# hmetaxa/MVTopicModel

Measured on AMD Instinct MI355X. Metric: gibbs_tokens_per_sec, higher is better.
Workload: dtype f64

## Files before the change

include/mvhdp.h:

```cpp
#ifndef MVHDP_H
#define MVHDP_H

#include <stddef.h>
#include <stdint.h>

#ifdef __cplusplus
extern "C" {
#endif

#define MVHDP_MAX_MODALITIES 8
#define MVHDP_MAX_TOPICS     2048
#define MVHDP_UNASSIGNED_TOPIC (-1)

typedef enum {
    MVHDP_OK = 0,
    MVHDP_ERR_INVALID_ARG   = -1,
    MVHDP_ERR_STATE         = -2,
    MVHDP_ERR_HIP           = -3,
    MVHDP_ERR_NO_DEVICE     = -4,
    MVHDP_ERR_NEGATIVE_COUNT= -5,
    MVHDP_ERR_UNSUPPORTED   = -6
} mvhdp_status;

typedef struct mvhdp_ctx* mvhdp_handle;
// ... 95 lines not shown
int mvhdp_build_counts(mvhdp_handle h);
int mvhdp_build_trees(mvhdp_handle h);
int mvhdp_build_inference_trees(mvhdp_handle h);
int mvhdp_init_assignments_from_trees(mvhdp_handle h, uint64_t seed);
int mvhdp_get_counts(mvhdp_handle h, int32_t m, int32_t* n_wk , int32_t* n_k );
int mvhdp_set_counts(mvhdp_handle h, int32_t m, const int32_t* n_wk, const int32_t* n_k);
int mvhdp_get_tree(mvhdp_handle h, int32_t m, int32_t type, double* tree );
int mvhdp_get_doc_topic_hist(mvhdp_handle h, int32_t m, int32_t* hist , int32_t hist_len,
                             int32_t* doc_len_counts , int32_t len_len);

int mvhdp_get_count_histogram(mvhdp_handle h, int32_t m, int32_t* hist, int32_t len);
int mvhdp_view_overlap_sums(mvhdp_handle h, double* sums );
int mvhdp_model_log_likelihood(mvhdp_handle h, double* log_likelihood );
int mvhdp_gamma_doc_statistics(mvhdp_handle h, int32_t m, double gamma_m, uint64_t seed, uint32_t round, double* qs, double* qw);
int mvhdp_dp_table_statistics(mvhdp_handle h, int32_t m, const int32_t* hist , int32_t hist_len, const double* conc ,
                              uint64_t seed, uint32_t round, double* mk , uint8_t* active );
int mvhdp_antoniak_draws(mvhdp_handle h, int32_t n, const int32_t* items , const double* conc , uint64_t seed, uint32_t round, int32_t* tables );
int mvhdp_doc_topic_proportions(mvhdp_handle h, const double* view_weights , int64_t d0, int64_t d1, double* out );

#define MVHDP_DIAG_MAX_TOP_WORDS 64
#define MVHDP_DIAG_PROPORTIONS   7
#define MVHDP_DIAG_TOKENS             0
#define MVHDP_DIAG_DOCUMENT_ENTROPY   1
#define MVHDP_DIAG_WORD_LENGTH        2
#define MVHDP_DIAG_COHERENCE          3
#define MVHDP_DIAG_NORM_DISCR_WEIGHT  4
#define MVHDP_DIAG_DISCR_WEIGHT       5
#define MVHDP_DIAG_UNIFORM_DIST       6
#define MVHDP_DIAG_CORPUS_DIST        7
#define MVHDP_DIAG_EFF_NUM_WORDS      8
#define MVHDP_DIAG_TOKEN_DOC_DIFF     9
#define MVHDP_DIAG_RANK_1_DOCS       10
#define MVHDP_DIAG_ALLOCATION_RATIO  11
#define MVHDP_DIAG_ALLOCATION_COUNT  12
#define MVHDP_DIAG_ROWS              13
typedef struct {
    int32_t num_top_words;
    const int32_t* word_length;
} mvhdp_diag_args;
typedef struct {
    double*  scores;
    double*  word_scores;
    int32_t* codoc;
    int32_t* top_types;
    int32_t* top_counts;
    int32_t* nonzero;
    int32_t* num_rank1_docs;
    int32_t* num_nonzero_docs;
    int32_t* num_docs_at_proportions;
    double*  sum_count_log_count;
    int32_t* word_type_counts;
    int64_t* num_tokens;
    double*  discr_weight_per_view;
} mvhdp_diag_out;
int mvhdp_top_words(mvhdp_handle h, int32_t m, int32_t n, int32_t* types , int32_t* counts , int32_t* nonzero );
int mvhdp_discr_weights(mvhdp_handle h, double* per_view , int32_t m, double* type_weight );
int mvhdp_diagnostics(mvhdp_handle h, const mvhdp_diag_args* args, mvhdp_diag_out* out);

int mvhdp_sweep(mvhdp_handle h, uint32_t sweep_idx, uint64_t seed, uint32_t flags,
                const double* p_override, const mvhdp_debug* dbg, mvhdp_sweep_stats* stats);
int mvhdp_sweep_many(mvhdp_handle h, uint32_t first_idx, int32_t n, uint64_t seed, uint32_t flags, mvhdp_sweep_stats* stats );
int mvhdp_apply_delta(mvhdp_handle h, int32_t activated_topic, int32_t activated_modality);
int mvhdp_apply_delta_begin(mvhdp_handle h);
int mvhdp_apply_delta_rows(mvhdp_handle h, int64_t row_begin, int64_t row_end);
int mvhdp_apply_delta_end(mvhdp_handle h, int32_t activated_topic, int32_t activated_modality);
int mvhdp_get_birth_keys(mvhdp_handle h, int64_t* keys );
int mvhdp_activate_births(mvhdp_handle h, const int64_t* keys );
int mvhdp_trees_current(mvhdp_handle h);
int mvhdp_get_view_weights(mvhdp_handle h, double* p );

typedef struct {
    int32_t force_primary;
    int32_t narrow;
    int32_t walk_fixed;
    int32_t single_stream;
    int32_t live16;
    int32_t single_wave;
    double  walk_theta[MVHDP_MAX_MODALITIES];
    double  primary_min_share;
    int32_t learnt_walk_step[4];
    double  tree_branch_share[MVHDP_MAX_MODALITIES];
    int32_t live_overlap;
    int32_t live_rows;
} mvhdp_tuning;
int mvhdp_get_tuning(mvhdp_handle h, mvhdp_tuning* t);
int mvhdp_set_tuning(mvhdp_handle h, const mvhdp_tuning* t);

typedef struct {
    int32_t num_topics, num_modalities;
    int64_t num_entities;
    int64_t max_entity_tokens;
    int64_t entities_longer_than[5];
    uint64_t tokens_by_list_rounds[17];
    uint64_t entities_by_class[8];
    uint32_t flags;
    int32_t debug, batch, trees_current;
    int32_t num_cus;
    int32_t kernel_registers[6][3];
    int32_t inactive_topics;
} mvhdp_plan_input;
typedef struct {
    int32_t status;
    int32_t segments, primary_class, register_resident, need_full_trees, dominant_class;
    int64_t routed_prefix;
    int32_t class_used[6], class_map[6], class_stream[6], class_grid[6], class_walk[6], class_narrow[6], class_register_resident[6];
    int64_t class_lds_bytes[6];
    double  class_theta0[6];
    int32_t delta16, live_rows;
} mvhdp_plan_output;
int mvhdp_plan_probe(const mvhdp_plan_input* in, const mvhdp_tuning* tuning , mvhdp_plan_output* out);
int mvhdp_tuner_probe(int32_t num_modalities, const double* tree_branch_share , const double* u1_hist ,
                      const double* ns_by_step , int32_t n_sweeps, int32_t group, int32_t* steps_out );

typedef struct mvhdp_group_ctx* mvhdp_group;
#define MVHDP_UNIQUE_ID_BYTES 128
typedef struct {
    int32_t local_members;
    int32_t local_devices;
    int32_t ranks, first_rank;
    int32_t rccl;
    int32_t rccl_version;
    int32_t exchange_chunks;
    int32_t exchange_packed;
    double  last_exchange_ms;
    int64_t last_exchange_bytes;
} mvhdp_group_info;
int mvhdp_group_create(int32_t n, const mvhdp_handle* members, mvhdp_group* out);
int mvhdp_group_unique_id(uint8_t* id );
int mvhdp_group_create_rank(mvhdp_handle member, const uint8_t* id , int32_t rank, int32_t nranks, mvhdp_group* out);
int mvhdp_group_destroy(mvhdp_group g);
const char* mvhdp_group_last_error(mvhdp_group g);
int mvhdp_group_get_info(mvhdp_group g, mvhdp_group_info* info);
int mvhdp_group_set_exchange_chunks(mvhdp_group g, int32_t chunks );
int mvhdp_group_build_counts(mvhdp_group g);
int mvhdp_group_sweep(mvhdp_group g, uint32_t sweep_idx, uint64_t seed, uint32_t flags, mvhdp_sweep_stats* stats);
#define MVHDP_SWEEP_ASYNC_EXCHANGE 0x100u
int mvhdp_group_drain(mvhdp_group g);
int mvhdp_group_abort(mvhdp_group g);

int mvhdp_group_set_hyper(mvhdp_group g, const mvhdp_hyper* hy);
int mvhdp_group_log_likelihood(mvhdp_group g, double* log_likelihood );
int mvhdp_group_doc_topic_hist(mvhdp_group g, int32_t m, int32_t* hist , int32_t hist_len,
                               int32_t* doc_len_counts , int32_t len_len);
int mvhdp_group_count_histogram(mvhdp_group g, int32_t m, int32_t* hist, int32_t len);
int mvhdp_group_view_overlap_sums(mvhdp_group g, double* sums );
int mvhdp_group_gamma_doc_statistics(mvhdp_group g, int32_t m, double gamma_m, uint64_t seed, uint32_t round, double* qs, double* qw);
int mvhdp_group_diagnostics(mvhdp_group g, const mvhdp_diag_args* args, mvhdp_diag_out* out);

int mvhdp_device_buffer(mvhdp_handle h, mvhdp_buffer which, void** dev_ptr, size_t* bytes);
int mvhdp_counts_written(mvhdp_handle h);
int mvhdp_set_stream(mvhdp_handle h, void* hip_stream );
int mvhdp_synchronize(mvhdp_handle h);

#ifdef __cplusplus
}
#endif
#endif
```

mvtopicmodel_amd/_lib.py:

```python
import ctypes as C
import os

_HERE = os.path.dirname(os.path.abspath(__file__))
LIB_PATH = os.path.join(_HERE, "lib", "libmvhdp.so")

MAX_M = 8

ABI_SYMBOLS = [
    "mvhdp_create", "mvhdp_destroy", "mvhdp_last_error", "mvhdp_version",
    "mvhdp_set_corpus", "mvhdp_set_assignments", "mvhdp_set_view_presence", "mvhdp_get_assignments",
    "mvhdp_set_hyper", "mvhdp_get_alpha", "mvhdp_build_counts", "mvhdp_build_trees",
    "mvhdp_build_inference_trees", "mvhdp_init_assignments_from_trees",
    "mvhdp_get_counts", "mvhdp_set_counts", "mvhdp_get_tree", "mvhdp_get_doc_topic_hist",
    "mvhdp_get_count_histogram", "mvhdp_view_overlap_sums", "mvhdp_model_log_likelihood", "mvhdp_doc_topic_proportions",
    "mvhdp_gamma_doc_statistics", "mvhdp_dp_table_statistics", "mvhdp_antoniak_draws",
    "mvhdp_top_words", "mvhdp_discr_weights", "mvhdp_diagnostics",
    "mvhdp_sweep", "mvhdp_sweep_many", "mvhdp_get_tuning", "mvhdp_set_tuning", "mvhdp_plan_probe", "mvhdp_tuner_probe",
    "mvhdp_apply_delta", "mvhdp_apply_delta_begin", "mvhdp_apply_delta_rows", "mvhdp_apply_delta_end",
    "mvhdp_get_birth_keys", "mvhdp_activate_births",
    "mvhdp_trees_current", "mvhdp_get_view_weights",
    "mvhdp_device_buffer", "mvhdp_counts_written", "mvhdp_set_stream", "mvhdp_synchronize",
    "mvhdp_group_create", "mvhdp_group_unique_id", "mvhdp_group_create_rank", "mvhdp_group_destroy", "mvhdp_group_last_error",
    "mvhdp_group_get_info", "mvhdp_group_set_exchange_chunks", "mvhdp_group_build_counts", "mvhdp_group_sweep", "mvhdp_group_abort", "mvhdp_group_drain",
    "mvhdp_group_set_hyper", "mvhdp_group_log_likelihood", "mvhdp_group_doc_topic_hist", "mvhdp_group_count_histogram",
    "mvhdp_group_view_overlap_sums", "mvhdp_group_gamma_doc_statistics", "mvhdp_group_diagnostics",
]

UNIQUE_ID_BYTES = 128


class MvhdpError(RuntimeError):
    def __init__(self, code, msg):
        super().__init__(f"mvhdp error {code}: {msg}")
        self.code = code


class Config(C.Structure):
    _fields_ = [("num_topics", C.c_int32), ("num_modalities", C.c_int32),
                ("num_types", C.c_int32 * MAX_M), ("device", C.c_int32),
                ("doc_id_base", C.c_int64), ("flags", C.c_uint32)]


class HyperC(C.Structure):
    _fields_ = [("alpha", C.c_void_p),
                ("alpha_sum", C.c_double * MAX_M), ("beta", C.c_double * MAX_M),
                ("beta_sum", C.c_double * MAX_M), ("gamma", C.c_double * MAX_M),
                ("p_a", (C.c_double * MAX_M) * MAX_M), ("p_b", (C.c_double * MAX_M) * MAX_M),
                ("inactive", C.c_void_p)]


class SweepStatsC(C.Structure):
    _fields_ = [("tokens", C.c_int64), ("changed", C.c_int64), ("new_mass_cnt", C.c_int64),
                ("topic_doc_mass_cnt", C.c_int64), ("word_ftree_mass_cnt", C.c_int64),
                ("oov_skipped", C.c_int64), ("aborted_docs", C.c_int64), ("exact_fallbacks", C.c_int64),
                ("activated_topic", C.c_int32), ("activated_modality", C.c_int32),
                ("activation_key", C.c_int64), ("sweep_kernel_ms", C.c_double), ("total_ms", C.c_double),
                ("activations", C.c_int32), ("reserved", C.c_int32)]


class DebugC(C.Structure):
    _fields_ = [("tok_dbg", C.c_void_p * MAX_M), ("n_trace", C.c_int32),
                ("trace_doc", C.c_void_p), ("trace_view", C.c_void_p), ("trace_pos", C.c_void_p),
                ("trace_out", C.c_void_p)]


class TuningC(C.Structure):
    _fields_ = [("force_primary", C.c_int32), ("narrow", C.c_int32), ("walk_fixed", C.c_int32), ("single_stream", C.c_int32),
                ("live16", C.c_int32), ("single_wave", C.c_int32),
                ("walk_theta", C.c_double * MAX_M), ("primary_min_share", C.c_double),
                ("learnt_walk_step", C.c_int32 * 4), ("tree_branch_share", C.c_double * MAX_M),
                ("live_overlap", C.c_int32), ("live_rows", C.c_int32)]


class GroupInfoC(C.Structure):
    _fields_ = [("local_members", C.c_int32), ("local_devices", C.c_int32), ("ranks", C.c_int32), ("first_rank", C.c_int32),
                ("rccl", C.c_int32), ("rccl_version", C.c_int32), ("exchange_chunks", C.c_int32), ("exchange_packed", C.c_int32),
                ("last_exchange_ms", C.c_double), ("last_exchange_bytes", C.c_int64)]


class PlanInputC(C.Structure):
    _fields_ = [("num_topics", C.c_int32), ("num_modalities", C.c_int32), ("num_entities", C.c_int64),
                ("max_entity_tokens", C.c_int64), ("entities_longer_than", C.c_int64 * 5),
                ("tokens_by_list_rounds", C.c_uint64 * 17), ("entities_by_class", C.c_uint64 * 8),
                ("flags", C.c_uint32), ("debug", C.c_int32), ("batch", C.c_int32), ("trees_current", C.c_int32),
                ("num_cus", C.c_int32), ("kernel_registers", (C.c_int32 * 3) * 6), ("inactive_topics", C.c_int32)]


class PlanOutputC(C.Structure):
    _fields_ = [("status", C.c_int32), ("segments", C.c_int32), ("primary_class", C.c_int32), ("register_resident", C.c_int32),
                ("need_full_trees", C.c_int32), ("dominant_class", C.c_int32), ("routed_prefix", C.c_int64),
                ("class_used", C.c_int32 * 6), ("class_map", C.c_int32 * 6), ("class_stream", C.c_int32 * 6),
                ("class_grid", C.c_int32 * 6), ("class_walk", C.c_int32 * 6), ("class_narrow", C.c_int32 * 6),
                ("class_register_resident", C.c_int32 * 6), ("class_lds_bytes", C.c_int64 * 6), ("class_theta0", C.c_double * 6),
                ("delta16", C.c_int32), ("live_rows", C.c_int32)]


DIAG_MAX_TOP_WORDS = 64
DIAG_PROPORTIONS = 7
DIAG_ROWS = ["tokens", "document_entropy", "word-length", "coherence", "normDiscrWeight", "discrWeight", "uniform_dist",
             "corpus_dist", "eff_num_words", "token-doc-diff", "rank_1_docs", "allocation_ratio", "allocation_count"]


class DiagArgsC(C.Structure):
    _fields_ = [("num_top_words", C.c_int32), ("word_length", C.c_void_p)]


class DiagOutC(C.Structure):
    _fields_ = [("scores", C.c_void_p), ("word_scores", C.c_void_p), ("codoc", C.c_void_p), ("top_types", C.c_void_p),
                ("top_counts", C.c_void_p), ("nonzero", C.c_void_p), ("num_rank1_docs", C.c_void_p), ("num_nonzero_docs", C.c_void_p),
                ("num_docs_at_proportions", C.c_void_p), ("sum_count_log_count", C.c_void_p), ("word_type_counts", C.c_void_p),
                ("num_tokens", C.c_void_p), ("discr_weight_per_view", C.c_void_p)]


_lib = None
_preloaded = []


def _torch_lib_dir():
    import importlib.util
    try:
        spec = importlib.util.find_spec("torch")
    except (ImportError, ValueError):
        return None
    if spec is None or not spec.submodule_search_locations:
        return None
    d = os.path.join(list(spec.submodule_search_locations)[0], "lib")
    return d if os.path.isdir(d) else None


def mapped_runtime_libraries():
    found = {"libamdhip64": set(), "libhsa-runtime64": set(), "librccl": set()}
    try:
        with open("/proc/self/maps") as f:
            for line in f:
                path = line.rsplit(None, 1)[-1] if "/" in line else ""
                base = os.path.basename(path)
                for name in found:
                    if base.startswith(name + ".so"):
                        found[name].add(os.path.realpath(path))
    except OSError:
        pass
    return {k: sorted(v) for k, v in found.items()}


def _preload_one_hip_runtime():
    d = _torch_lib_dir()
    if d is None:
        return False
    already = mapped_runtime_libraries()
    if already["libamdhip64"] or already["libhsa-runtime64"]:
        return False
    path = os.path.join(d, "libamdhip64.so")
    if not os.path.exists(path):
        return False
# ... 96 lines not shown
```

mvtopicmodel_amd/csrc/mvhdp_api.hip:

```cpp
#include "mvhdp_ctx.h"

static thread_local std::string g_create_error;

static std::mutex g_reg_mutex;
static std::set<mvhdp_ctx*>* g_live = nullptr;
static bool g_exiting = false, g_atexit_registered = false;
static void release_device_resources(mvhdp_ctx* h);

static void mvhdp_at_exit()
{
    std::lock_guard<std::mutex> lk(g_reg_mutex);
    g_exiting = true;
    if (g_live) for (mvhdp_ctx* h : *g_live) release_device_resources(h);
}

static void register_handle(mvhdp_ctx* h)
{
    std::lock_guard<std::mutex> lk(g_reg_mutex);
    if (!g_live) g_live = new std::set<mvhdp_ctx*>();
    g_live->insert(h);
    if (!g_atexit_registered) { atexit(mvhdp_at_exit); g_atexit_registered = true; }
}

bool mvhdp_is_live(mvhdp_ctx* h)
{
    std::lock_guard<std::mutex> lk(g_reg_mutex);
    return g_live && g_live->count(h) != 0;
}

static void read_environment(mvhdp_ctx* h)
{
    if (const char* f = getenv("MVHDP_FORCE_RMAX")) { const int v = atoi(f); if (v == 1 || v == 2 || v == 4 || v == 8 || v == 16 || v == 32) h->tu.force_primary = v; }
    if (const char* f = getenv("MVHDP_NARROW")) h->tu.narrow = atoi(f) != 0 ? -1 : 0;
    if (const char* f = getenv("MVHDP_SINGLE_STREAM")) h->tu.single_stream = atoi(f) != 0;
    if (const char* f = getenv("MVHDP_SIDE_PRIORITY")) h->side_priority = atoi(f);
    if (const char* f = getenv("MVHDP_LIVE16")) h->tu.live16 = atoi(f);
    if (const char* f = getenv("MVHDP_LIVE_OVERLAP")) h->tu.live_overlap = atoi(f);
    if (const char* f = getenv("MVHDP_LIVE_ROWS")) h->tu.live_rows = atoi(f);
    if (const char* f = getenv("MVHDP_LIVE_ROWS_THETA")) h->tu.live_rows_theta = atof(f);
    if (const char* f = getenv("MVHDP_COEF_LDS_KB")) h->tu.coef_lds_max_bytes = std::max(0, std::min(64, atoi(f))) * 1024;
    if (const char* f = getenv("MVHDP_LIVE_ROWS_SEGMENTS")) h->tu.live_rows_segments = std::max(1, std::min(255, atoi(f)));
    if (const char* f = getenv("MVHDP_WIDEST_ON_MAIN")) h->tu.widest_on_main = atoi(f) != 0;
    if (const char* f = getenv("MVHDP_NARROW_WIDE")) h->tu.narrow_wide = atoi(f) != 0;
    if (const char* f = getenv("MVHDP_LIVE_TREE_EVERY")) h->live_tree_every = std::max(1, atoi(f));
    if (const char* f = getenv("MVHDP_GATE_PCT")) { const int v = atoi(f); if (v >= 5 && v <= 95) h->gate_pct = v; }
    if (const char* f = getenv("MVHDP_FOUR_ROUND_ON_C")) h->tu.four_round_on_c = atoi(f);
    if (const char* f = getenv("MVHDP_DELTA16")) h->tu.delta16 = atoi(f) != 0;
    if (const char* f = getenv("MVHDP_FORK_DELAY_US")) h->tu.fork_delay_us = std::max(0, std::min(1000, atoi(f)));
    if (const char* f = getenv("MVHDP_FORCE_MODE")) { if (!strcmp(f, "serial")) h->tu.single_stream = 1; }
    if (const char* f = getenv("MVHDP_PRIMARY_MIN_SHARE")) { const double v = atof(f); if (v > 0.0 && v <= 1.0) h->tu.primary_min_share = v; }
    if (const char* t = getenv("MVHDP_WALK_THETA")) {
        int m = 0;
        for (const char* q = t; *q && m < MVHDP_MAXM; m++) {
            h->tu.walk_theta[m] = atof(q);
            while (*q && *q != ',') q++;
            if (*q == ',') q++;
        }
        for (; m < MVHDP_MAXM; m++) h->tu.walk_theta[m] = 0.0;
        h->tu.walk_fixed = 1;
    }
    h->dbg_env = getenv("MVHDP_DEBUG") != nullptr;
}

extern "C" const char* mvhdp_version(void) { return "mvhdp 0.1 (gfx950)"; }

extern "C" const char* mvhdp_last_error(mvhdp_handle h) { return (h && mvhdp_is_live(h)) ? h->err.c_str() : g_create_error.c_str(); }

extern "C" int mvhdp_create(const mvhdp_config* cfg, mvhdp_handle* out)
{
    if (!cfg || !out) { g_create_error = "null argument"; return MVHDP_ERR_INVALID_ARG; }
    *out = nullptr;
    const int K = cfg->num_topics, M = cfg->num_modalities;
    if (K < 1 || K > MVHDP_MAX_TOPICS || M < 1 || M > MVHDP_MAX_MODALITIES) {
        g_create_error = "num_topics must be in [1,2048] and num_modalities in [1,8]";
        return MVHDP_ERR_INVALID_ARG;
    }
    for (int m = 0; m < M; m++) if (cfg->num_types[m] < 1) { g_create_error = "num_types[m] must be >= 1"; return MVHDP_ERR_INVALID_ARG; }
    for (int m = 0; m < M; m++) if (cfg->num_types[m] >= (1 << 29)) { g_create_error = "num_types[m] must be below 2^29"; return MVHDP_ERR_INVALID_ARG; }
    if (cfg->doc_id_base < 0 || cfg->doc_id_base >= (1LL << 29)) { g_create_error = "doc_id_base out of range"; return MVHDP_ERR_INVALID_ARG; }
    int ndev = 0;
    if (hipGetDeviceCount(&ndev) != hipSuccess || ndev <= 0 || cfg->device < 0 || cfg->device >= ndev) {
        g_create_error = "no usable HIP device (the sweep has no CPU fallback)";
        return MVHDP_ERR_NO_DEVICE;
    }
    hipDeviceProp_t prop;
    if (hipGetDeviceProperties(&prop, cfg->device) != hipSuccess) { g_create_error = "hipGetDeviceProperties failed"; return MVHDP_ERR_HIP; }
    if (strncmp(prop.gcnArchName, "gfx950", 6) != 0) {
        g_create_error = std::string("device is ") + prop.gcnArchName + ", this library is built for gfx950 only";
        return MVHDP_ERR_NO_DEVICE;
    }
    mvhdp_ctx* h = new mvhdp_ctx();
    register_handle(h);
    h->cfg = *cfg;
    h->device = cfg->device;
    h->num_cus = prop.multiProcessorCount;
    h->max_lds = 160 * 1024;
    MvModel& mm = h->mm;
    mm.K = K; mm.M = M;
    mm.rowbase[0] = 0;
    for (int m = 0; m < M; m++) { mm.V[m] = cfg->num_types[m]; mm.rowbase[m + 1] = mm.rowbase[m] + cfg->num_types[m]; }
    mm.doc_id_base = cfg->doc_id_base;
    mm.first_inactive = -1;
    mm.D = -1;
#define CREATE_HIP(call) do { hipError_t e_ = (call); if (e_ != hipSuccess) { \
    g_create_error = std::string(#call) + ": " + hipGetErrorString(e_); mvhdp_destroy(h); return MVHDP_ERR_HIP; } } while (0)
    CREATE_HIP(hipSetDevice(h->device));
    CREATE_HIP(hipStreamCreateWithFlags(&h->stream, hipStreamNonBlocking));
    h->own_stream = true;
    for (auto& e : h->ev) CREATE_HIP(hipEventCreate(&e));
    const int64_t nrows = mm.rowbase[M];
    const size_t cbytes = (size_t)(nrows * K + (int64_t)M * K + MVHDP_TAIL_WORDS) * sizeof(int32_t);
    CREATE_HIP(hipMalloc(&mm.counts, cbytes));
    CREATE_HIP(hipMalloc(&mm.delta, cbytes));
    CREATE_HIP(hipMemset(mm.counts, 0, cbytes));
    CREATE_HIP(hipMalloc(&mm.counts16, (size_t)nrows * K * sizeof(uint16_t) + 64));
    CREATE_HIP(hipMemset(mm.counts16, 0, (size_t)nrows * K * sizeof(uint16_t)));
    CREATE_HIP(hipMalloc(&mm.delta16, (size_t)(nrows * K + 2) * sizeof(uint16_t)));
    CREATE_HIP(hipMemsetD16(mm.delta16, (unsigned short)0x8000, (size_t)(nrows * K + 2)));
    CREATE_HIP(hipMalloc(&mm.heavy, (size_t)nrows));
    CREATE_HIP(hipMemset(mm.heavy, 1, (size_t)nrows));
    CREATE_HIP(hipMemset(mm.delta, 0, cbytes));
    CREATE_HIP(hipMalloc(&mm.trees, (size_t)nrows * 2 * K * sizeof(double)));
    CREATE_HIP(hipMalloc(&mm.root, (size_t)nrows * sizeof(double)));
    CREATE_HIP(hipMalloc(&mm.mass0, (size_t)nrows * sizeof(float)));
    CREATE_HIP(hipMemset(mm.mass0, 0, (size_t)nrows * sizeof(float)));
    CREATE_HIP(hipMalloc(&mm.coef, (size_t)M * (((K + 7) & ~7) + K + 8) * sizeof(float)));
    {
        const int nlev = (K > 1) ? (32 - __builtin_clz((unsigned)(K - 1))) : 0;
        mm.dt_f = nlev ? ((nlev - 1) % 3) + 1 : 0;
        mm.dt_nbd = 1; mm.dt_base[0] = 0; mm.dt_depth[0] = 0;
        int nblk = 1;
        for (int dep = mm.dt_f; nlev && dep < nlev; dep += 3) {
            mm.dt_base[mm.dt_nbd] = nblk; mm.dt_depth[mm.dt_nbd] = dep; mm.dt_nbd++;
            nblk += 1 << dep;
        }
        mm.dt_nblk = nblk;
        CREATE_HIP(hipMalloc(&mm.dtab, (size_t)nrows * nblk * 8 * sizeof(double)));
    }
    CREATE_HIP(hipMalloc(&h->d_alpha, (size_t)M * (K + 1) * sizeof(double)));
    CREATE_HIP(hipMalloc(&h->d_inactive, (size_t)K));
    CREATE_HIP(hipMemset(h->d_inactive, 0, (size_t)K));
    CREATE_HIP(hipMalloc(&h->d_births, (size_t)(2 + 2 * K) * sizeof(int32_t)));
    CREATE_HIP(hipMemset(h->d_births, 0, (size_t)(2 + 2 * K) * sizeof(int32_t)));
    CREATE_HIP(hipMalloc(&h->d_birth_keys, (size_t)K * sizeof(long long)));
    CREATE_HIP(hipMalloc(&h->d_birth_table, (size_t)K * sizeof(long long)));
    {
        const std::vector<long long> none((size_t)K, LLONG_MAX);
        CREATE_HIP(hipMemcpy(h->d_birth_table, none.data(), (size_t)K * sizeof(long long), hipMemcpyHostToDevice));
    }
    CREATE_HIP(hipMalloc(&h->d_ctl, CTL_WORDS * sizeof(unsigned long long)));
    CREATE_HIP(hipMemset(h->d_ctl, 0, CTL_WORDS * sizeof(unsigned long long)));
    h->d_stats = h->d_ctl;
    h->d_act_key = (long long*)(h->d_ctl + ST_COUNT);
    h->d_ovf_meta = (unsigned int*)(h->d_ctl + ST_COUNT + 1);
    h->d_doc_counter = h->d_ctl + ST_COUNT + 1 + META_WORDS64;
    CREATE_HIP(hipHostMalloc((void**)&h->h_ctl, CTL_WORDS * sizeof(unsigned long long), hipHostMallocDefault));
    for (int c = 0; c < MVHDP_N_CLASSES; c++)
        for (int f = 0; f < 3; f++) h->regs.regs[c][f] = mvhdp_sweep_kernel_regs(c, f);
    read_environment(h);
    mm.alpha = h->d_alpha;
    mm.inactive = h->d_inactive;
    h->h_alpha.assign((size_t)M * (K + 1), 0.0);
    h->h_inactive.assign((size_t)K, 0);
    h->wt.init_defaults(K);
    *out = h;
    return MVHDP_OK;
}

static void release_device_resources(mvhdp_ctx* h)
{
    if (h->device_released) return;
    h->device_released = true;
    hipSetDevice(h->device);
    if (h->stream) hipStreamSynchronize(h->stream);
    auto fr = [](auto*& p) { if (p) { hipFree((void*)p); p = nullptr; } };
    for (int m = 0; m < MVHDP_MAXM; m++) { fr(h->d_doc_off[m]); fr(h->d_tok[m]); fr(h->d_z[m]); fr(h->d_carry[m]); fr(h->d_present[m]); }
    fr(h->mm.counts); fr(h->mm.delta16); fr(h->mm.counts16); fr(h->mm.heavy); fr(h->mm.delta); fr(h->mm.trees); fr(h->mm.root); fr(h->mm.coef); fr(h->mm.mass0); fr(h->d_births); fr(h->d_birth_keys); fr(h->d_birth_table); fr(h->mm.dtab); fr(h->mm.p);
    fr(h->d_alpha); fr(h->d_inactive); fr(h->d_ctl);
    if (h->h_ctl) { hipHostFree(h->h_ctl); h->h_ctl = nullptr; }
    h->d_stats = nullptr; h->d_act_key = nullptr; h->d_doc_counter = nullptr; h->d_ovf_meta = nullptr;
    fr(h->d_doc_order); fr(h->d_lists); fr(h->d_nslots); fr(h->d_stats_many); fr(h->d_heavy_list); fr(h->d_heavy_ctl);
    if (h->ev_rf_go) { hipEventDestroy(h->ev_rf_go); h->ev_rf_go = nullptr; }
    if (h->ev_rf_done) { hipEventDestroy(h->ev_rf_done); h->ev_rf_done = nullptr; }
    if (h->rf_stream) { hipStreamDestroy(h->rf_stream); h->rf_stream = nullptr; }
    fr(h->ov.counts2); fr(h->ov.counts16_2); fr(h->ov.dtab2); fr(h->ov.root2); fr(h->ov.trees2); fr(h->ov.delta2); fr(h->ov.delta3); fr(h->ov.ctl2); fr(h->ov.lists2);
    for (auto& e : h->ov.ev_seg) if (e) { hipEventDestroy(e); e = nullptr; }
    if (h->ov.ev_start) { hipEventDestroy(h->ov.ev_start); h->ov.ev_start = nullptr; }
    if (h->ov.x1) { hipStreamDestroy(h->ov.x1); h->ov.x1 = nullptr; }
    if (h->ov.xa) { hipStreamDestroy(h->ov.xa); h->ov.xa = nullptr; }
    for (auto& e : h->ev_many) if (e) { hipEventDestroy(e); e = nullptr; }
    for (auto& e : h->ev) if (e) { hipEventDestroy(e); e = nullptr; }
    if (h->ev_fork) { hipEventDestroy(h->ev_fork); h->ev_fork = nullptr; }
    for (auto& e : h->ev_join) if (e) { hipEventDestroy(e); e = nullptr; }
    for (auto& st : h->side) if (st) { hipStreamDestroy(st); st = nullptr; }
    if (h->own_stream && h->stream) hipStreamDestroy(h->stream);
    h->stream = nullptr;
}

extern "C" int mvhdp_destroy(mvhdp_handle h)
{
    if (!h) return MVHDP_OK;
    bool exiting;
    {
        std::lock_guard<std::mutex> lk(g_reg_mutex);
        if (!g_live || g_live->erase(h) == 0) return MVHDP_ERR_INVALID_ARG;
        exiting = g_exiting;
    }
    if (!exiting) release_device_resources(h);
    delete h;
    return MVHDP_OK;
}

extern "C" int mvhdp_set_stream(mvhdp_handle h, void* hip_stream)
{
    CHECK_H(h);
    HIPC(h, hipSetDevice(h->device));
    HIPC(h, hipStreamSynchronize(h->stream));
    if (h->own_stream) { hipStreamDestroy(h->stream); h->own_stream = false; }
    if (hip_stream) h->stream = (hipStream_t)hip_stream;
    else { HIPC(h, hipStreamCreateWithFlags(&h->stream, hipStreamNonBlocking)); h->own_stream = true; }
    return MVHDP_OK;
}

extern "C" int mvhdp_synchronize(mvhdp_handle h)
{
    CHECK_H(h);
    HIPC(h, hipSetDevice(h->device));
    HIPC(h, hipStreamSynchronize(h->stream));
    return MVHDP_OK;
}

extern "C" int mvhdp_set_corpus(mvhdp_handle h, int32_t m, int64_t D, const int64_t* doc_off, const int32_t* tokens)
{
    CHECK_H(h);
    MvModel& mm = h->mm;
    if (m < 0 || m >= mm.M || D < 0 || !doc_off) FAIL(h, MVHDP_ERR_INVALID_ARG, "set_corpus: bad view, num_docs or doc_off");
    if (mm.D >= 0 && D != mm.D) {
        bool any_other = false;
        for (int j = 0; j < mm.M; j++) if (j != m && h->have_corpus[j]) any_other = true;
        if (any_other) FAIL(h, MVHDP_ERR_INVALID_ARG, "set_corpus: every view must list the same entities (empty span = view absent)");
    }
    if (mm.doc_id_base + D >= (1LL << 29)) FAIL(h, MVHDP_ERR_INVALID_ARG, "set_corpus: too many entities");
    if (doc_off[0] != 0) FAIL(h, MVHDP_ERR_INVALID_ARG, "set_corpus: doc_off[0] must be 0");
    for (int64_t d = 0; d < D; d++) {
        int64_t len = doc_off[d + 1] - doc_off[d];
        if (len < 0) FAIL(h, MVHDP_ERR_INVALID_ARG, "set_corpus: doc_off must be non-decreasing");
        if (len >= (1 << 20)) FAIL(h, MVHDP_ERR_INVALID_ARG, "set_corpus: a view of one entity is limited to 2^20-1 tokens");
    }
    const int64_t N = doc_off[D];
    if (N > 0 && !tokens) FAIL(h, MVHDP_ERR_INVALID_ARG, "set_corpus: tokens is null");
    HIPC(h, hipSetDevice(h->device));
    HIPC(h, hipStreamSynchronize(h->stream));
    if (h->d_doc_off[m]) { hipFree(h->d_doc_off[m]); h->d_doc_off[m] = nullptr; }
    if (h->d_tok[m]) { hipFree(h->d_tok[m]); h->d_tok[m] = nullptr; }
    if (h->d_z[m]) { hipFree(h->d_z[m]); h->d_z[m] = nullptr; }
    if (h->d_present[m]) { hipFree(h->d_present[m]); h->d_present[m] = nullptr; }
    h->h_present[m].clear(); mm.present[m] = nullptr;
    HIPC(h, hipMalloc(&h->d_doc_off[m], (size_t)(D + 1) * sizeof(int64_t)));
    HIPC(h, hipMemcpy(h->d_doc_off[m], doc_off, (size_t)(D + 1) * sizeof(int64_t), hipMemcpyHostToDevice));
    const size_t nb = (size_t)std::max<int64_t>(N, 1) * sizeof(int32_t);
// ... 746 lines not shown
        MvModel mk;
        if (p.seg_apply) {
            mk = B[seg == 0 ? 0 : (seg - 1) & 1];
            mk.delta = D3[seg % 3];
        } else {
            mk = mm;
            mk.delta = mm.counts;
            mk.dtab = B[seg & 1].dtab; mk.root = B[seg & 1].root; mk.trees = B[seg & 1].trees;
            if (seg >= 1 && !(flags & MVHDP_SWEEP_REUSE_TREES)) {
                step(hipStreamWaitEvent(xs, ev_reset(seg - 1), 0));
                const int64_t n_prev = share_of(seg - 1, mm.D), H_prev = p.route ? share_of(seg - 1, p.H) : 0;
                const unsigned long long thr = (unsigned long long)((n_prev - H_prev) * h->gate_pct / 100);
                step(mvhdp_launch_gate(ctl[(seg - 1) & 1].qheads + p.pc, thr, xs));
                MvModel tm = mm;
                tm.dtab = mk.dtab; tm.root = mk.root; tm.trees = mk.trees;
                if (p.live16) step(mvhdp_launch_build_trees_from_mirror(tm, p.need_full, xs, true));
                else step(mvhdp_launch_build_trees(tm, false, p.need_full, xs, true));
            } else if (seg >= 1) {
                mk.dtab = mm.dtab; mk.root = mm.root; mk.trees = mm.trees;
            }
        }
        step(mvhdp_launch_ctl_reset(nullptr, 0, nullptr, nullptr, 0, cs.class_counts, cs.qheads, xs));
        step(hipEventRecord(ev_reset(seg), xs));
        step(launch_segment_kernels(h, p, mk, sl, seg, xs, cs, d_stats));
        step(hipEventRecord(ev_done(seg), xs));
        if (p.seg_apply) {
            if (seg >= 1) step(hipStreamWaitEvent(xs, ev_applied(seg - 1), 0));
            const MvModel& dst = B[(seg + 1) & 1];
            step(mvhdp_launch_apply2_counts(dst, D3[seg % 3], seg >= 1 ? D3[(seg - 1) % 3] : nullptr, use_mirror, d_stats + ST_NEGATIVE, xs));
            step(hipEventRecord(ev_applied(seg), xs));
        }
    }
    if (mm.D > 0 && e == hipSuccess) {
        if (p.seg_apply) {
            step(hipStreamWaitEvent(X[0], ev_applied(nseg - 1), 0));
            if (nseg >= 2) step(hipStreamWaitEvent(X[0], ev_done(nseg - 2), 0));
            const MvModel& last = B[(nseg + 1) & 1];
            step(mvhdp_launch_apply_sparse(last, D3[(nseg - 1) % 3], use_mirror, X[0]));
            h->have_trees = false;
        } else {
            step(hipStreamWaitEvent(X[0], ev_done(nseg - 1), 0));
            if (nseg >= 2) step(hipStreamWaitEvent(X[0], ev_done(nseg - 2), 0));
        }
    }
    if (p.live) {
        if (p.live16 && mm.D > 0) { step(mvhdp_launch_widen_mirror(mm, X[0])); h->have_trees = false; }
        if (flags & MVHDP_SWEEP_NO_APPLY) {
            step(mvhdp_launch_live_helper(mm, 1, d_stats, X[0]));
            if (!(flags & MVHDP_SWEEP_REUSE_TREES)) h->have_trees = false;
        } else step(mvhdp_launch_live_helper(mm, 2, d_stats, X[0]));
        if (!(flags & MVHDP_SWEEP_REUSE_TREES)) h->have_trees = false;
    }
    step(hipEventRecord(ev_k1, X[0]));
    if (e != hipSuccess) HIPC(h, e);
    return MVHDP_OK;
}

static int enqueue_sweep(mvhdp_ctx* h, const SweepPlan& p, uint32_t sweep_idx, uint64_t seed, const double* p_override,
                         const DebugBufs* db, unsigned long long* d_stats, hipEvent_t ev_k0, hipEvent_t ev_k1, SweepOutcome& oc)
{
    if (p.overlap) return enqueue_overlapped(h, p, sweep_idx, seed, p_override, d_stats, ev_k0, ev_k1);
    MvModel& mm = h->mm;
    const int M = mm.M;
    const uint32_t flags = p.flags;
    const int nseg = p.nseg;
    hipStream_t s = h->stream;
    hipError_t e = hipSuccess;
    auto step = [&](hipError_t r) { if (e == hipSuccess) e = r; };

    SweepLaunch sl{};
    sl.sweep_idx = sweep_idx; sl.seed_lo = (uint32_t)seed; sl.seed_hi = (uint32_t)(seed >> 32);
    sl.flags = flags & 0x7fffu; sl.S_cap = p.S_cap;
    if (h->tu.single_wave && p.live) sl.flags |= MVHDP_SL_STRICT_LIVE;
    if (p.live_rows && getenv("MVHDP_NO_ROW_SAMPLE")) sl.flags |= 0x2000u;
#ifdef MVHDP_PROBE
    if (const char* f = getenv("MVHDP_ATOMIC_PROBE")) sl.flags |= ((unsigned)atoi(f) & 7u) << 16;
#endif
    sl.q_order_stride = 1;
    sl.nk_global = p.nk_global; sl.block_shared_bytes = p.block_shared_bytes;
    sl.live16 = p.live16 ? 1 : 0;
    sl.live_rows = p.live_rows ? 1 : 0;
    sl.coef_lds = p.coef_lds ? 1 : 0;
    sl.delta16 = p.delta16 ? 1 : 0;
    sl.stats = d_stats;
    sl.act_key = h->d_act_key;
    const bool births = sweep_births(p, flags, mm);
    if (births) { sl.births = h->d_births; sl.birth_keys = h->d_birth_keys; }
    sl.slot_hist = (unsigned long long*)h->d_ovf_meta + META_HIST;
    if (db) {
        for (int m = 0; m < M; m++) sl.tok_dbg[m] = db->tok_dbg[m];
        sl.n_trace = db->n_trace; sl.trace_doc = db->trace_doc; sl.trace_view = db->trace_view; sl.trace_pos = db->trace_pos; sl.trace_out = db->trace_out;
    }
    unsigned int* class_counts = h->d_ovf_meta + META_CLASS_COUNTS;

    if (M > 1) {
        if (!mm.p && mm.D > 0) step(hipMalloc(&mm.p, (size_t)mm.D * M * M * sizeof(double)));
        if (e == hipSuccess) {
            if (p_override) step(hipMemcpyAsync(mm.p, p_override, (size_t)mm.D * M * M * sizeof(double), hipMemcpyHostToDevice, s));
            else step(mvhdp_launch_draw_p(mm, sweep_idx, sl.seed_lo, sl.seed_hi, s));
        }
    }
    h->last_need_full = p.need_full;
    const bool dummy_poll = getenv("MVHDP_DUMMY_POLL") != nullptr;
    const bool refresher = ((p.live_rows && p.live16) || dummy_poll) && !h->tu.single_wave && !getenv("MVHDP_NO_HEAVY_REFRESH");
    auto live_rows_prepare = [&](bool from_mirror) -> hipError_t {
        if ((p.live16 || dummy_poll) && !h->d_heavy_list) {
            hipError_t e1 = hipMalloc(&h->d_heavy_list, (size_t)MVHDP_HEAVY_CAP * sizeof(int32_t));
            if (e1 == hipSuccess) e1 = hipMalloc(&h->d_heavy_ctl, 2 * sizeof(unsigned int));
            if (e1 != hipSuccess) return e1;
        }
        if (refresher && !h->rf_stream) {
            int least = 0, greatest = 0;
            if (hipDeviceGetStreamPriorityRange(&least, &greatest) != hipSuccess || greatest >= least ||
                hipStreamCreateWithPriority(&h->rf_stream, hipStreamNonBlocking, greatest) != hipSuccess) {
                (void)hipGetLastError(); h->rf_stream = nullptr;
                hipError_t e1 = hipStreamCreateWithFlags(&h->rf_stream, hipStreamNonBlocking); if (e1 != hipSuccess) return e1;
            }
            hipError_t e1 = hipEventCreateWithFlags(&h->ev_rf_go, hipEventDisableTiming);
            if (e1 == hipSuccess) e1 = hipEventCreateWithFlags(&h->ev_rf_done, hipEventDisableTiming);
            if (e1 != hipSuccess) return e1;
        }
        return mvhdp_launch_live_rows_prepare(mm, from_mirror, p.live16, p.live16 ? h->d_heavy_list : nullptr, p.live16 ? h->d_heavy_ctl : nullptr, MVHDP_HEAVY_CAP,
                                              p.live16 ? 512 : 256 , s);
    };
    auto rebuild_trees = [&]() {
        step(mvhdp_launch_build_trees(mm, false, p.need_full, s));
        h->have_trees = true; h->full_trees = p.need_full; h->trees_inference = false;
    };
    if (p.live_rows) {
        step(live_rows_prepare(false));
        h->have_trees = false; h->full_trees = false;
    } else if (!(flags & MVHDP_SWEEP_REUSE_TREES)) rebuild_trees();
    if (dummy_poll && !p.live_rows) {
        if (!h->d_heavy_list) { step(hipMalloc(&h->d_heavy_list, (size_t)MVHDP_HEAVY_CAP * sizeof(int32_t))); step(hipMalloc(&h->d_heavy_ctl, 2 * sizeof(unsigned int))); }
        if (!h->rf_stream) { step(hipStreamCreateWithFlags(&h->rf_stream, hipStreamNonBlocking)); step(hipEventCreateWithFlags(&h->ev_rf_go, hipEventDisableTiming)); step(hipEventCreateWithFlags(&h->ev_rf_done, hipEventDisableTiming)); }
        step(hipMemsetAsync(h->d_heavy_ctl, 0, 2 * sizeof(unsigned int), s));
    }
    else if (p.need_full && !h->full_trees) {
        step(mvhdp_launch_build_trees(mm, h->trees_inference, true, s));
        h->full_trees = true;
    }
    MvModel mk = mm;
    if (p.live) {
        mk.delta = mm.counts;
        if (flags & MVHDP_SWEEP_NO_APPLY) { step(mvhdp_launch_live_helper(mm, 0, d_stats, s)); h->delta_clean = false; }
    } else if (!p.frozen) {
        if (!h->delta_clean) {
            step(hipMemsetAsync(mm.delta, 0, (size_t)counts_len(h) * sizeof(int32_t), s));
            if (h->delta16_used) step(hipMemsetD16Async(mm.delta16, (unsigned short)0x8000, (size_t)(mm.rowbase[M] * mm.K), s));
            h->delta16_used = false;
        }
        h->delta_clean = false;
        if (p.delta16) h->delta16_used = true;
    }
    step(mvhdp_launch_ctl_reset(d_stats, ST_COUNT, h->d_act_key, (unsigned long long*)h->d_ovf_meta, META_WORDS64, nullptr, h->d_doc_counter, s));
    if (births) step(births_begin(h, s));
    step(hipEventRecord(ev_k0, s));

    const int seg_lo = p.only_seg >= 0 ? p.only_seg : 0, seg_hi = p.only_seg >= 0 ? p.only_seg + 1 : nseg;
    for (int seg = seg_lo; seg < seg_hi && e == hipSuccess && mm.D > 0; seg++) {
        if (seg > seg_lo) {
            if (births && !(flags & MVHDP_SWEEP_NO_APPLY) && e == hipSuccess) {
                const int rc = births_end(h, s, oc);
                if (rc != MVHDP_OK) return rc;
                mk.first_inactive = mm.first_inactive;
                step(births_begin(h, s));
// ... 261 lines not shown
    CHECK_H(h);
    if (n < 0) FAIL(h, MVHDP_ERR_INVALID_ARG, "sweep_many: n < 0");
    if (n == 0) return MVHDP_OK;
    MvModel& mm = h->mm;
    const bool frozen = (flags & MVHDP_SWEEP_FROZEN) != 0;
    if (n == 1 || mm.first_inactive >= 0 || ((flags & MVHDP_SWEEP_NO_APPLY) && !frozen) || ((flags & MVHDP_SWEEP_REUSE_TREES) && !frozen) || n > 4096) {
        for (int i = 0; i < n; i++) {
            const int rc = mvhdp_sweep(h, first_idx + (uint32_t)i, seed, flags, nullptr, nullptr, stats ? stats + i : nullptr);
            if (rc) return rc;
        }
        return MVHDP_OK;
    }
    int rc = sweep_preconditions(h, flags); if (rc) return rc;
    HIPC(h, hipSetDevice(h->device));
    hipStream_t s = h->stream;
    rc = ensure_slot_counts(h); if (rc) return rc;
    PlanIn in; fill_plan_in(h, flags, false, true, in);
    SweepPlan p;
    plan_sweep(in, h->tu, h->wt, p);
    if (p.err) FAIL(h, p.err, p.msg);
    rc = set_generic_lds(h, p); if (rc) return rc;
    if (h->dbg_env) debug_print_plan(h, p, first_idx);
    if (h->stats_many_cap < n) {
        if (h->d_stats_many) { hipFree(h->d_stats_many); h->d_stats_many = nullptr; h->stats_many_cap = 0; }
        HIPC(h, hipMalloc(&h->d_stats_many, (size_t)n * ST_COUNT * sizeof(unsigned long long)));
        h->stats_many_cap = n;
    }
    while ((int)h->ev_many.size() < 2 * n) { hipEvent_t ev; HIPC(h, hipEventCreate(&ev)); h->ev_many.push_back(ev); }
    HIPC(h, hipEventRecord(h->ev[0], s));
    for (int i = 0; i < n; i++) {
        SweepOutcome oc;
        unsigned long long* d_st = h->d_stats_many + (size_t)i * ST_COUNT;
        rc = enqueue_sweep(h, p, first_idx + (uint32_t)i, seed, nullptr, nullptr, d_st, h->ev_many[2 * i], h->ev_many[2 * i + 1], oc);
        if (rc) return rc;
        if (!p.frozen && !p.live && !p.seg_apply) {
            HIPC(h, mvhdp_launch_apply_delta(mm, d_st, s, h->delta16_used));
            h->delta16_used = false;
            h->have_trees = false; h->delta_clean = true;
        } else if (p.live || p.seg_apply) {
            h->have_trees = false;
            if (p.seg_apply) h->delta_clean = true;
        }
    }
    HIPC(h, hipEventRecord(h->ev[3], s));
    std::vector<unsigned long long> hs((size_t)n * ST_COUNT);
    unsigned long long meta[META_WORDS64] = {0};
    HIPC(h, hipMemcpyAsync(hs.data(), h->d_stats_many, hs.size() * sizeof(unsigned long long), hipMemcpyDeviceToHost, s));
    HIPC(h, hipMemcpyAsync(meta, h->d_ovf_meta, sizeof meta, hipMemcpyDeviceToHost, s));
    HIPC(h, hipStreamSynchronize(s));
    if (p.seg_apply && p.overlap) h->ov.deltas_dirty = false;
    float ms_t = 0;
    hipEventElapsedTime(&ms_t, h->ev[0], h->ev[3]);
    int ret = MVHDP_OK;
    double ms_sum = 0;
    for (int i = 0; i < n; i++) {
        const unsigned long long* hi = hs.data() + (size_t)i * ST_COUNT;
        mvhdp_sweep_stats st;
        stats_from_counters(hi, LLONG_MAX, st);
        float ms_k = 0;
        hipEventElapsedTime(&ms_k, h->ev_many[2 * i], h->ev_many[2 * i + 1]);
        st.sweep_kernel_ms = ms_k; st.total_ms = ms_t / n;
        ms_sum += ms_k;
        if (stats) stats[i] = st;
        if (hi[ST_MISCLASS]) { h->nslots_valid = false; FAIL(h, MVHDP_ERR_HIP, "internal: an entity reached a sweep kernel variant that cannot hold its topic list"); }
        if (hi[ST_NEGATIVE] && ret == MVHDP_OK) { h->err = "a topic count went below zero (UPD:202-215)"; ret = MVHDP_ERR_NEGATIVE_COUNT; }
    }
    if (meta[META_MISROUTED]) { h->nslots_valid = false; FAIL(h, MVHDP_ERR_HIP, "internal: an entity could not be routed to a sweep kernel"); }
    std::vector<unsigned long long> acc(ST_COUNT, 0);
    for (int i = 0; i < n; i++) for (int k = 0; k < ST_COUNT; k++) acc[k] += hs[(size_t)i * ST_COUNT + k];
    const bool comparable = p.fast && !h->tu.walk_fixed && !(flags & (MVHDP_SWEEP_FROZEN | MVHDP_SWEEP_EXACT_CHAIN));
    learn_from_sweep(h, p, acc.data(), meta + META_HIST, ms_sum, comparable);
    if (!p.frozen && acc[ST_ABORT] == 0) for (int m = 0; m < mm.M; m++) h->unassigned[m] = false;
    return ret;
}

extern "C" int mvhdp_get_tuning(mvhdp_handle h, mvhdp_tuning* t)
{
    CHECK_H(h);
    if (!t) FAIL(h, MVHDP_ERR_INVALID_ARG, "get_tuning: null");
    memset(t, 0, sizeof *t);
    t->force_primary = h->tu.force_primary; t->narrow = h->tu.narrow; t->walk_fixed = h->tu.walk_fixed;
    t->single_stream = h->tu.single_stream; t->primary_min_share = h->tu.primary_min_share; t->live16 = h->tu.live16;
    t->single_wave = h->tu.single_wave; t->live_overlap = h->tu.live_overlap; t->live_rows = h->tu.live_rows;
    for (int m = 0; m < MVHDP_MAX_MODALITIES; m++) { t->walk_theta[m] = h->tu.walk_theta[m]; t->tree_branch_share[m] = h->wt.walk_f[m]; }
    for (int g = 0; g < WALK_GROUPS; g++) t->learnt_walk_step[g] = g == h->wt.walk_cls ? h->wt.walk_i : h->wt.walk_i_by[g];
    t->learnt_walk_step[3] = -1;
    return MVHDP_OK;
}

extern "C" int mvhdp_set_tuning(mvhdp_handle h, const mvhdp_tuning* t)
{
    CHECK_H(h);
    if (!t) FAIL(h, MVHDP_ERR_INVALID_ARG, "set_tuning: null");
    const int fp = t->force_primary;
    if (!(fp == 0 || fp == 1 || fp == 2 || fp == 4 || fp == 8 || fp == 16 || fp == 32)) FAIL(h, MVHDP_ERR_INVALID_ARG, "set_tuning: force_primary must be 0, 1, 2, 4, 8, 16 or 32");
    if (t->primary_min_share < 0.0 || t->primary_min_share > 1.0) FAIL(h, MVHDP_ERR_INVALID_ARG, "set_tuning: primary_min_share outside [0, 1]");
    for (int g = 0; g < WALK_GROUPS; g++) if (t->learnt_walk_step[g] < -1 || t->learnt_walk_step[g] > MVHDP_WALK_BINS) FAIL(h, MVHDP_ERR_INVALID_ARG, "set_tuning: learnt_walk_step outside [-1, 20]");
    h->tu.force_primary = fp; h->tu.narrow = t->narrow; h->tu.walk_fixed = t->walk_fixed ? 1 : 0;
    h->tu.single_stream = t->single_stream ? 1 : 0;
    h->tu.live16 = t->live16 < 0 ? -1 : (t->live16 ? 1 : 0);
    h->tu.single_wave = t->single_wave ? 1 : 0;
    h->tu.live_overlap = t->live_overlap < 0 ? -1 : (t->live_overlap ? 1 : 0);
    h->tu.live_rows = t->live_rows < 0 ? -1 : (t->live_rows ? 1 : 0);
    h->tu.primary_min_share = t->primary_min_share > 0.0 ? t->primary_min_share : 0.10;
    for (int m = 0; m < MVHDP_MAX_MODALITIES; m++) h->tu.walk_theta[m] = t->walk_theta[m];
    if (t->learnt_walk_step[0] >= 0 || t->learnt_walk_step[1] >= 0 || t->learnt_walk_step[2] >= 0) h->wt.restore(t->learnt_walk_step, t->tree_branch_share, h->mm.M);
    return MVHDP_OK;
}

extern "C" int mvhdp_plan_probe(const mvhdp_plan_input* pi, const mvhdp_tuning* t, mvhdp_plan_output* po)
{
    if (!pi || !po) return MVHDP_ERR_INVALID_ARG;
    PlanIn in;
    in.K = pi->num_topics; in.M = pi->num_modalities; in.D = pi->num_entities; in.mdt = pi->max_entity_tokens;
    if (in.K < 1 || in.K > MVHDP_MAX_TOPICS || in.M < 1 || in.M > MVHDP_MAX_MODALITIES || in.D < 0) return MVHDP_ERR_INVALID_ARG;
    in.have_order = true;
    for (int c = 0; c < 5; c++) in.n_longer[c] = pi->entities_longer_than[c];
    for (int b = 0; b < MVHDP_HIST_BINS; b++) in.tok_hist[b] = pi->tokens_by_list_rounds[b];
    for (int b = 0; b < MVHDP_ENT_BINS; b++) in.ent_hist[b] = pi->entities_by_class[b];
    in.flags = pi->flags; in.debug = pi->debug != 0; in.batch = pi->batch != 0; in.trees_current = pi->trees_current != 0;
    in.first_inactive = pi->inactive_topics ? 0 : -1;
    in.num_cus = pi->num_cus > 0 ? pi->num_cus : 256;
    for (int c = 0; c < MVHDP_N_CLASSES; c++) for (int f = 0; f < 3; f++) in.regs.regs[c][f] = pi->kernel_registers[c][f];
    PlanTuning tu;
    WalkTuner wt;
    wt.init_defaults(in.K);
    if (t) {
        tu.force_primary = t->force_primary; tu.narrow = t->narrow; tu.walk_fixed = t->walk_fixed; tu.single_stream = t->single_stream;
        tu.live16 = t->live16; tu.single_wave = t->single_wave ? 1 : 0; tu.live_overlap = t->live_overlap; tu.live_rows = t->live_rows;
        if (t->primary_min_share > 0) tu.primary_min_share = t->primary_min_share;
        for (int m = 0; m < MVHDP_MAX_MODALITIES; m++) tu.walk_theta[m] = t->walk_theta[m];
        if (t->learnt_walk_step[0] >= 0 || t->learnt_walk_step[1] >= 0 || t->learnt_walk_step[2] >= 0) wt.restore(t->learnt_walk_step, t->tree_branch_share, in.M);
    }
    SweepPlan p;
    plan_sweep(in, tu, wt, p);
    memset(po, 0, sizeof *po);
    po->status = p.err;
    if (p.err) return MVHDP_OK;
    po->segments = p.nseg; po->primary_class = p.pc; po->routed_prefix = p.H; po->register_resident = p.fast ? 1 : 0;
    po->need_full_trees = p.need_full ? 1 : 0; po->dominant_class = p.dominant;
    for (int c = 0; c < MVHDP_N_CLASSES; c++) {
        po->class_used[c] = p.cls[c].used ? 1 : 0; po->class_map[c] = p.class_map[c];
        po->class_stream[c] = p.cls[c].stream; po->class_grid[c] = p.cls[c].grid; po->class_lds_bytes[c] = (int64_t)p.cls[c].lds;
        po->class_walk[c] = p.cls[c].walk; po->class_narrow[c] = p.cls[c].narrow; po->class_register_resident[c] = p.cls[c].fast ? 1 : 0;
        po->class_theta0[c] = p.cls[c].theta[0];
    }
    po->delta16 = p.delta16 ? 1 : 0;
    po->live_rows = p.live_rows ? 1 : 0;
    return MVHDP_OK;
}

extern "C" int mvhdp_tuner_probe(int32_t num_modalities, const double* tree_branch_share, const double* u1_hist, const double* ns_by_step ,
                                 int32_t n_sweeps, int32_t group, int32_t* steps_out )
{
    if (!tree_branch_share || !ns_by_step || !steps_out || num_modalities < 1 || num_modalities > MVHDP_MAX_MODALITIES || n_sweeps < 0) return MVHDP_ERR_INVALID_ARG;
    WalkTuner wt;
    if (group < 0 || group >= WALK_GROUPS) return MVHDP_ERR_INVALID_ARG;
    for (int m = 0; m < num_modalities; m++) wt.walk_f[m] = tree_branch_share[m];
    for (int b = 0; b < MVHDP_WALK_BINS; b++) wt.walk_hist[b] = u1_hist ? u1_hist[b] : 0.0;
    for (int i = 0; i < n_sweeps; i++) {
        double theta[WALK_GROUPS][MVHDP_MAXM]; bool measure;
        wt.propose(group, num_modalities, theta, &measure);
        steps_out[i] = wt.walk_probe_i;
        wt.observe(true, 1, num_modalities, ns_by_step[std::max(0, std::min(MVHDP_WALK_BINS, wt.walk_probe_i))]);
    }
    return MVHDP_OK;
}

extern "C" int mvhdp_get_view_weights(mvhdp_handle h, double* p)
{
    CHECK_H(h);
    MvModel& mm = h->mm;
    if (!p) FAIL(h, MVHDP_ERR_INVALID_ARG, "get_view_weights: null");
    if (mm.M == 1) { for (int64_t d = 0; d < mm.D; d++) p[d] = 1.0; return MVHDP_OK; }
    if (!mm.p) FAIL(h, MVHDP_ERR_STATE, "get_view_weights before the first sweep");
    HIPC(h, hipSetDevice(h->device));
    HIPC(h, hipStreamSynchronize(h->stream));
    HIPC(h, hipMemcpy(p, mm.p, (size_t)mm.D * mm.M * mm.M * sizeof(double), hipMemcpyDeviceToHost));
    return MVHDP_OK;
}

extern "C" int mvhdp_device_buffer(mvhdp_handle h, mvhdp_buffer which, void** dev_ptr, size_t* bytes)
{
    CHECK_H(h);
    if (!dev_ptr || !bytes) FAIL(h, MVHDP_ERR_INVALID_ARG, "device_buffer: null");
    size_t b = (size_t)counts_len(h) * sizeof(int32_t);
    if (which == MVHDP_BUF_COUNTS) { *dev_ptr = h->mm.counts; *bytes = b; return MVHDP_OK; }
    if (which == MVHDP_BUF_DELTA) { *dev_ptr = h->mm.delta; *bytes = b; return MVHDP_OK; }
    if (which == MVHDP_BUF_BIRTH_KEYS) { *dev_ptr = h->d_birth_table; *bytes = (size_t)h->mm.K * sizeof(long long); return MVHDP_OK; }
    FAIL(h, MVHDP_ERR_INVALID_ARG, "device_buffer: unknown buffer");
}

extern "C" int mvhdp_counts_written(mvhdp_handle h)
{
    CHECK_H(h);
    h->have_counts = true; h->have_trees = false; h->counts_stale = false;
    return MVHDP_OK;
}

static double log_gamma_stirling_host(double z)
{
    const double HALF_LOG_TWO_PI = std::log(6.283185307179586) / 2.0;
    int shift = 0;
    while (z < 2.0) { z = z + 1; shift++; }
    double result = HALF_LOG_TWO_PI + (z - 0.5) * std::log(z) - z + 1 / (12.0 * z) - 1 / (360.0 * z * z * z)
                    + 1 / (1260.0 * z * z * z * z * z);
    while (shift > 0) { shift--; z = z - 1; result = result - std::log(z); }
    return result;
}

extern "C" int mvhdp_get_count_histogram(mvhdp_handle h, int32_t m, int32_t* hist, int32_t len)
{
// ... 237 lines not shown
```

mvtopicmodel_amd/csrc/mvhdp_device.h:

```cpp
#pragma once
#include <hip/hip_runtime.h>
#include <stdint.h>

#define MVHDP_MAXM 8
#define MVHDP_WALK_BINS 20
#define MVHDP_VIEW_STATS (2 + MVHDP_WALK_BINS)

struct MvModel {
    int32_t K, M;
    int32_t V[MVHDP_MAXM];
    int64_t rowbase[MVHDP_MAXM + 1];
    int64_t D;
    int64_t doc_id_base;
    const int64_t* doc_off[MVHDP_MAXM];
    const int32_t* tok[MVHDP_MAXM];
    int32_t* z[MVHDP_MAXM];
    const uint8_t* present[MVHDP_MAXM];
    uint16_t* nslots;
    int32_t* counts;
    uint16_t* delta16;
    uint16_t* counts16;
    uint8_t* heavy;
    int32_t* delta;
    double* trees;
    double* root;
    float* coef;
    float* mass0;
    double* dtab;
    int32_t dt_nblk, dt_nbd, dt_f;
    int32_t dt_base[6], dt_depth[6];
    const double* alpha;
    const uint8_t* inactive;
    double alpha_sum[MVHDP_MAXM], beta[MVHDP_MAXM], beta_sum[MVHDP_MAXM], gamma[MVHDP_MAXM];
    double p_a[MVHDP_MAXM][MVHDP_MAXM], p_b[MVHDP_MAXM][MVHDP_MAXM];
    double* p;
    int32_t first_inactive;
};

#define MVHDP_SL_STRICT_LIVE 0x8000u
#define MVHDP_ROW_HEAVY 1
#define MVHDP_ROW_BIG 2

struct SweepLaunch {
    uint32_t sweep_idx;
    uint32_t seed_lo, seed_hi;
    uint32_t flags;
    int32_t  S_cap;
    int32_t  waves_per_block;
    uint32_t block_shared_bytes;
    int32_t  nk_global;
    uint32_t wave_bytes;
    unsigned long long* stats;
    long long* act_key;
    int32_t* births;
    long long* birth_keys;
    unsigned long long* doc_counter;
    const int32_t* q_list;
    const unsigned int* q_list_count;
    const int32_t* q_order;
    int64_t q_order_start, q_order_count, q_order_stride;
    double walk_theta[MVHDP_MAXM];
    int32_t walk;
    int32_t narrow;
    int32_t delta16;
    int32_t live16;
    int32_t live_rows;
    int32_t coef_lds;
    unsigned long long* slot_hist;
    double* tok_dbg[MVHDP_MAXM];
    int32_t n_trace;
    const int64_t* trace_doc; const int32_t* trace_view; const int32_t* trace_pos;
    double* trace_out;
};

enum {
    ST_TOKENS = 0, ST_CHANGED, ST_NEW, ST_DOC, ST_TREE, ST_OOV, ST_ABORT, ST_FALLBACK, ST_NEGATIVE, ST_MISCLASS, ST_ONDEMAND,
    ST_VIEW_BASE, ST_VIEW_LAST = ST_VIEW_BASE + MVHDP_VIEW_STATS * MVHDP_MAXM - 1,
    ST_T_QUEUE, ST_T_PROLOGUE, ST_T_VIEW, ST_T_CHUNK_HEAD, ST_T_TOKENS, ST_T_CHUNK_END, ST_T_TOTAL,
    ST_T_ENT0, ST_T_ENT1, ST_T_ENT2, ST_N_ENT0, ST_N_ENT1, ST_N_ENT2, ST_T_INIT, ST_T_FLUSH, ST_N_WAVES, ST_T_ROWS, ST_T_ROWS_WAIT,
    ST_COUNT
};

size_t mvhdp_sweep_wave_bytes(int M, int S_cap);

hipError_t mvhdp_launch_build_counts(const MvModel& mm, const int64_t* n_tokens_per_view, hipStream_t s);
hipError_t mvhdp_launch_build_trees(const MvModel& mm, bool inference_leaves, bool write_full, hipStream_t s, bool beside_samplers = false);
hipError_t mvhdp_launch_build_trees_rows(const MvModel& mm, bool inference_leaves, bool write_full, int64_t row_begin, int64_t row_end,
                                         bool apply_first, unsigned long long* negatives, hipStream_t s);
hipError_t mvhdp_launch_build_trees_from_mirror(const MvModel& mm, bool write_full, hipStream_t s, bool beside_samplers = false);
hipError_t mvhdp_launch_widen_mirror(const MvModel& mm, hipStream_t s);
hipError_t mvhdp_launch_live_rows_prepare(const MvModel& mm, bool from_mirror, bool with_heavy_trees, int32_t* heavy_list, unsigned int* heavy_ctl, int heavy_cap, int batch_cells, hipStream_t s);
hipError_t mvhdp_launch_heavy_refresh(const MvModel& mm, const int32_t* heavy_list, const unsigned int* ctl, int heavy_cap, int blocks, hipStream_t s);
hipError_t mvhdp_launch_set_u32(unsigned int* p, unsigned int v, hipStream_t s);
hipError_t mvhdp_launch_apply_nk(const MvModel& mm, unsigned long long* negatives, hipStream_t s);
hipError_t mvhdp_launch_apply2_counts(const MvModel& dst, const int32_t* dA, int32_t* dB, bool use_mirror, unsigned long long* negatives, hipStream_t s);
hipError_t mvhdp_launch_apply_sparse(const MvModel& dst, int32_t* d, bool use_mirror, hipStream_t s);
hipError_t mvhdp_launch_gate(const unsigned long long* qhead, unsigned long long threshold, hipStream_t s);
hipError_t mvhdp_launch_init_from_trees(const MvModel& mm, uint32_t seed_lo, uint32_t seed_hi, hipStream_t s);
hipError_t mvhdp_launch_draw_p(const MvModel& mm, uint32_t sweep_idx, uint32_t seed_lo, uint32_t seed_hi, hipStream_t s);
hipError_t mvhdp_launch_sweep(const MvModel& mm, const SweepLaunch& sl, int grid_blocks, bool debug, hipStream_t s);
hipError_t mvhdp_launch_apply_delta(const MvModel& mm, unsigned long long* stats, hipStream_t s, bool with_delta16 = false);
hipError_t mvhdp_launch_delay(int microseconds, hipStream_t s);
hipError_t mvhdp_launch_ctl_reset(unsigned long long* stats, int n_stats, long long* act_key, unsigned long long* meta, int n_meta,
                                  unsigned int* class_counts, unsigned long long* qheads, hipStream_t s);
hipError_t mvhdp_launch_birth_table(const int32_t* births, const long long* birth_keys, const long long* act_key, int K, long long* keys, hipStream_t s);
hipError_t mvhdp_launch_live_helper(const MvModel& mm, int which, unsigned long long* stats, hipStream_t s);
hipError_t mvhdp_launch_doc_topic_hist(const MvModel& mm, int m, int32_t* hist, int32_t hist_len,
                                       int32_t* doc_len_counts, int32_t len_len, hipStream_t s);
hipError_t mvhdp_sweep_set_max_lds(size_t bytes);
hipError_t mvhdp_launch_count_hist(const MvModel& mm, int m, int32_t* hist, int32_t len, hipStream_t s);
hipError_t mvhdp_launch_view_overlap(const MvModel& mm, double* out, hipStream_t s);
hipError_t mvhdp_launch_loglik_doc(const MvModel& mm, int m, double* doc_out, hipStream_t s);
hipError_t mvhdp_launch_loglik_topic(const MvModel& mm, int m, double* partial, int n_partial, unsigned long long* nonzero, hipStream_t s);
hipError_t mvhdp_launch_gamma_doc_stats(const MvModel& mm, int m, double gamma_m, uint32_t seed_lo, uint32_t seed_hi, uint32_t round,
                                        double* partial, int n_blocks, hipStream_t s);
hipError_t mvhdp_launch_dp_tables(const int32_t* hist, int hist_len, int K, int m, const double* conc, uint32_t seed_lo, uint32_t seed_hi, uint32_t round,
                                  double* mk, uint8_t* active, hipStream_t s);
hipError_t mvhdp_launch_antoniak_draws(int n, const int32_t* items, const double* conc, uint32_t seed_lo, uint32_t seed_hi, uint32_t round, int32_t* tables, hipStream_t s);
hipError_t mvhdp_launch_slot_hist(const MvModel& mm, unsigned long long* hist, hipStream_t s);
struct DocTopicCarry { const int64_t* src[MVHDP_MAXM]; };
hipError_t mvhdp_launch_doc_topic_prop(const MvModel& mm, const DocTopicCarry& carry, const double* w_dev, int64_t d0, int64_t d1, double* out_dev, hipStream_t s);
#define MVHDP_N_CLASSES 6
struct ClassifyArgs {
    const int32_t* order;
    int64_t n, start, stride;
    int32_t class_map[MVHDP_N_CLASSES];
    int32_t check_views;
    int32_t* lists[MVHDP_N_CLASSES];
    unsigned int* counts;
    unsigned long long* misrouted;
};
hipError_t mvhdp_launch_classify(const MvModel& mm, const ClassifyArgs& ca, hipStream_t s);
size_t mvhdp_sweep_fast_wave_bytes(int M, int S_cap, int rmax);
hipError_t mvhdp_launch_sweep_fast(const MvModel& mm, const SweepLaunch& sl, int rmax, int grid_blocks, bool debug, hipStream_t s);
int mvhdp_sweep_fast_occupancy(int rmax, bool debug, bool walk, int block_threads, size_t lds_bytes);
int mvhdp_sweep_generic_occupancy(bool debug, int block_threads, size_t lds_bytes);
int mvhdp_sweep_kernel_regs(int cls, int flavour);
int mvhdp_sweep_generic_regs(bool debug);

#define MVHDP_DOC_BATCH 2
#define MVHDP_HIST_BINS 17
#define MVHDP_ENT_BINS 8
#define MVHDP_NSLOTS_UNKNOWN 0xFFFFu

__host__ __device__ __forceinline__ int mvhdp_class_of(int n, bool view_beyond_16_bits)
{
    int c = (n <= 64) ? 0 : (n <= 128) ? 1 : (n <= 256) ? 2 : (n <= 512) ? 3 : (n <= 1024) ? 4 : 5;
// ... 66 lines not shown
```

mvtopicmodel_amd/csrc/mvhdp_group.hip:

```cpp
#include "mvhdp_ctx.h"

#include <dlfcn.h>
#include <rccl/rccl.h>

#include <map>

namespace {

struct Rccl {
    void* lib = nullptr;
    std::string path, why;
    ncclResult_t (*GetVersion)(int*) = nullptr;
    ncclResult_t (*GetUniqueId)(ncclUniqueId*) = nullptr;
    ncclResult_t (*CommInitRank)(ncclComm_t*, int, ncclUniqueId, int) = nullptr;
    ncclResult_t (*CommInitAll)(ncclComm_t*, int, const int*) = nullptr;
    ncclResult_t (*CommDestroy)(ncclComm_t) = nullptr;
    ncclResult_t (*AllReduce)(const void*, void*, size_t, ncclDataType_t, ncclRedOp_t, ncclComm_t, hipStream_t) = nullptr;
    ncclResult_t (*GroupStart)() = nullptr;
    ncclResult_t (*GroupEnd)() = nullptr;
    const char* (*GetErrorString)(ncclResult_t) = nullptr;
};

std::mutex g_rccl_mutex;
Rccl g_rccl;
// ... 363 lines not shown
    info->exchange_packed = g->pack_on ? 1 : 0;
    return MVHDP_OK;
}

extern "C" int mvhdp_group_set_exchange_chunks(mvhdp_group g, int32_t chunks)
{
    CHECK_G(g);
    if (chunks < 1 || chunks > 64) GFAIL(g, MVHDP_ERR_INVALID_ARG, "group_set_exchange_chunks: 1..64");
    g->chunks = chunks;
    return MVHDP_OK;
}

struct XErr {
    mvhdp_group_ctx* g;
    int rc = MVHDP_OK;
    void hip(hipError_t e, const char* what) { if (e != hipSuccess && rc == MVHDP_OK) { rc = MVHDP_ERR_HIP; g->err = std::string(what) + ": " + hipGetErrorString(e); } }
    void nccl(ncclResult_t r, const char* what) { if (r != ncclSuccess && rc == MVHDP_OK) { rc = MVHDP_ERR_HIP; g->err = std::string(what) + ": " + (g_rccl.GetErrorString ? g_rccl.GetErrorString(r) : "RCCL error"); } }
};

static int reduce_local(mvhdp_group_ctx* g, bool counts)
{
    XErr x{g};
    const int n = (int)g->members.size();
    for (int i = 0; i < n; i++) {
        const int li = g->leader_of[i];
        if (li == i) continue;
        mvhdp_ctx *h = g->members[i], *L = g->members[li];
        x.hip(hipSetDevice(L->device), "hipSetDevice");
        x.hip(hipStreamWaitEvent(L->stream, g->ev_swept[i], 0), "hipStreamWaitEvent");
        x.hip(launch_add_into(counts ? L->mm.counts : L->mm.delta, counts ? h->mm.counts : h->mm.delta, counts_len_of(L), L->stream), "add_into_kernel");
    }
    return x.rc;
}

static int allreduce_range(mvhdp_group_ctx* g, bool counts, int64_t e0, int64_t e1)
{
    if (e1 <= e0 || g->comms.empty()) return MVHDP_OK;
    Rccl* r = &g_rccl;
    XErr x{g};
    if (g->comms.size() > 1) x.nccl(r->GroupStart(), "ncclGroupStart");
    for (size_t l = 0; l < g->leaders.size(); l++) {
        mvhdp_ctx* L = g->members[g->leaders[l]];
        x.hip(hipSetDevice(L->device), "hipSetDevice");
        int32_t* buf = (counts ? L->mm.counts : L->mm.delta) + e0;
        x.nccl(r->AllReduce(buf, buf, (size_t)(e1 - e0), ncclInt32, ncclSum, g->comms[l], L->stream), "ncclAllReduce");
    }
    if (g->comms.size() > 1) x.nccl(r->GroupEnd(), "ncclGroupEnd");
    return x.rc;
}

static int fan_out_range(mvhdp_group_ctx* g, bool counts, int64_t e0, int64_t e1)
{
    if (e1 <= e0 || g->members.size() == g->leaders.size()) return MVHDP_OK;
    XErr x{g};
    for (size_t l = 0; l < g->leaders.size(); l++) {
        mvhdp_ctx* L = g->members[g->leaders[l]];
        x.hip(hipSetDevice(L->device), "hipSetDevice");
        x.hip(hipEventRecord(g->ev_reduced[l], L->stream), "hipEventRecord");
        for (size_t i = 0; i < g->members.size(); i++) {
            if (g->leader_of[i] != g->leaders[l] || (int)i == g->leaders[l]) continue;
            mvhdp_ctx* h = g->members[i];
            x.hip(hipStreamWaitEvent(h->stream, g->ev_reduced[l], 0), "hipStreamWaitEvent");
            const int32_t* src = (counts ? L->mm.counts : L->mm.delta) + e0;
            int32_t* dst = (counts ? h->mm.counts : h->mm.delta) + e0;
            x.hip(hipMemcpyAsync(dst, src, (size_t)(e1 - e0) * sizeof(int32_t), hipMemcpyDeviceToDevice, h->stream), "hipMemcpyAsync");
            x.hip(hipEventRecord(g->ev_swept[i], h->stream), "hipEventRecord");
            x.hip(hipStreamWaitEvent(L->stream, g->ev_swept[i], 0), "hipStreamWaitEvent");
        }
    }
    return x.rc;
}

static int pack_prepare(mvhdp_group_ctx* g)
{
    if (g->pack_ready || !g->pack_allowed) return MVHDP_OK;
    for (mvhdp_ctx* h : g->members) for (int m = 0; m < h->mm.M; m++) if (h->unassigned[m]) return MVHDP_OK;
    mvhdp_ctx* L0 = g->members[g->leaders[0]];
    const int64_t rows = L0->mm.rowbase[L0->mm.M];
    const int K = L0->mm.K;
    if (rows <= 0) return MVHDP_OK;
    std::vector<uint8_t> cls((size_t)rows);
    GHIP(g, hipSetDevice(L0->device));
    GHIP(g, hipMemcpy(cls.data(), L0->mm.heavy, (size_t)rows, hipMemcpyDeviceToHost));
    g->woff.assign((size_t)rows + 1, 0);
    for (int64_t r = 0; r < rows; r++) g->woff[(size_t)r + 1] = g->woff[(size_t)r] + (cls[(size_t)r] == 0 ? (K + 1) / 2 : K);
    if (g->d_woff.empty()) { g->d_woff.assign(g->leaders.size(), nullptr); g->d_cls.assign(g->leaders.size(), nullptr); g->xpack.assign(g->leaders.size(), nullptr); }
    for (size_t l = 0; l < g->leaders.size(); l++) {
        mvhdp_ctx* L = g->members[g->leaders[l]];
        GHIP(g, hipSetDevice(L->device));
        if (!g->d_woff[l]) GHIP(g, hipMalloc(&g->d_woff[l], (size_t)(rows + 1) * sizeof(int64_t)));
        if (!g->d_cls[l]) GHIP(g, hipMalloc(&g->d_cls[l], (size_t)rows));
        if (!g->xpack[l]) GHIP(g, hipMalloc(&g->xpack[l], (size_t)rows * K * sizeof(int32_t)));
        GHIP(g, hipMemcpy(g->d_woff[l], g->woff.data(), (size_t)(rows + 1) * sizeof(int64_t), hipMemcpyHostToDevice));
        GHIP(g, hipMemcpy(g->d_cls[l], cls.data(), (size_t)rows, hipMemcpyHostToDevice));
    }
    g->pack_hash = (int32_t)(g->woff[(size_t)rows] % 4091) + 1;
    g->pack_ready = true;
    return MVHDP_OK;
}

static void pack_reset(mvhdp_group_ctx* g) { g->pack_on = false; g->pack_ready = false; g->pack_hash = 0; g->sweeps_since_counts = 0; }

static int allreduce_rows_packed(mvhdp_group_ctx* g, int64_t r0, int64_t r1)
{
    XErr x{g};
    Rccl* r = &g_rccl;
    const int64_t w0 = g->woff[(size_t)r0], w1 = g->woff[(size_t)r1];
    const int K = g->members[0]->mm.K;
    const int grid = (int)std::min<int64_t>((r1 - r0 + 3) / 4, 8192);
    for (size_t l = 0; l < g->leaders.size(); l++) {
        mvhdp_ctx* L = g->members[g->leaders[l]];
        x.hip(hipSetDevice(L->device), "hipSetDevice");
        hipLaunchKernelGGL(pack_rows_kernel, dim3(std::max(grid, 1)), dim3(256), 0, L->stream, L->mm.delta, g->d_cls[l], g->d_woff[l], g->xpack[l], r0, r1, K);
        x.hip(hipGetLastError(), "pack_rows_kernel");
    }
    if (!g->comms.empty() && w1 > w0) {
        if (g->comms.size() > 1) x.nccl(r->GroupStart(), "ncclGroupStart");
        for (size_t l = 0; l < g->leaders.size(); l++) {
            mvhdp_ctx* L = g->members[g->leaders[l]];
            x.hip(hipSetDevice(L->device), "hipSetDevice");
            x.nccl(r->AllReduce(g->xpack[l] + w0, g->xpack[l] + w0, (size_t)(w1 - w0), ncclInt32, ncclSum, g->comms[l], L->stream), "ncclAllReduce");
        }
        if (g->comms.size() > 1) x.nccl(r->GroupEnd(), "ncclGroupEnd");
    }
    for (size_t l = 0; l < g->leaders.size(); l++) {
        mvhdp_ctx* L = g->members[g->leaders[l]];
        x.hip(hipSetDevice(L->device), "hipSetDevice");
        hipLaunchKernelGGL(unpack_rows_kernel, dim3(std::max(grid, 1)), dim3(256), 0, L->stream, L->mm.delta, g->d_cls[l], g->d_woff[l], g->xpack[l], r0, r1, K);
        x.hip(hipGetLastError(), "unpack_rows_kernel");
    }
    g->last_exchange_bytes += (w1 - w0) * (long long)sizeof(int32_t);
    return x.rc;
}

extern "C" int mvhdp_group_build_counts(mvhdp_group g)
{
    CHECK_G(g);
    DeviceGuard dg;
    if (g->async_pending) {
        for (size_t l = 0; l < g->leaders.size(); l++) { hipSetDevice(g->members[g->leaders[l]]->device); hipStreamSynchronize(g->comm[l]); }
        g->async_pending = false;
    }
    const int n = (int)g->members.size();
    const int64_t len = counts_len_of(g->members[0]);
    int local_err = MVHDP_OK;
    auto note = [&](int rc, const std::string& what) { if (rc != MVHDP_OK && local_err == MVHDP_OK) { local_err = rc; g->err = what; } };
    XErr x{g};
    pack_reset(g);
    for (int i = 0; i < n; i++) {
        mvhdp_ctx* h = g->members[i];
        const int rc = mvhdp_build_counts(h);
        if (rc != MVHDP_OK) note(rc, "member " + std::to_string(i) + ": " + h->err);
        if (!h->delta_clean) { x.hip(hipSetDevice(h->device), "hipSetDevice"); x.hip(hipMemsetAsync(h->mm.delta, 0, (size_t)(len + MVHDP_TAIL_WORDS) * sizeof(int32_t), h->stream), "hipMemsetAsync"); h->delta_clean = true; h->delta_pending = false; }
    }
    if (local_err != MVHDP_OK)
        for (int i = 0; i < n; i++) { mvhdp_ctx* h = g->members[i]; x.hip(hipSetDevice(h->device), "hipSetDevice"); x.hip(hipMemsetAsync(h->mm.counts, 0, (size_t)len * sizeof(int32_t), h->stream), "hipMemsetAsync"); }
    for (int i = 0; i < n; i++) { x.hip(hipSetDevice(g->members[i]->device), "hipSetDevice"); x.hip(hipEventRecord(g->ev_swept[i], g->members[i]->stream), "hipEventRecord"); }
    note(reduce_local(g, true), g->err);
    note(x.rc, g->err);
    for (size_t l = 0; l < g->leaders.size(); l++) {
        mvhdp_ctx* L = g->members[g->leaders[l]];
        x.hip(hipSetDevice(L->device), "hipSetDevice");
        hipLaunchKernelGGL(set_word_kernel, dim3(1), dim3(1), 0, L->stream, L->mm.counts + len, local_err != MVHDP_OK ? 1 : 0);
    }
    note(allreduce_range(g, true, 0, len + 1), g->err);
    note(fan_out_range(g, true, 0, len + 1), g->err);
// ... 661 lines not shown
```

mvtopicmodel_amd/csrc/mvhdp_kernels.hip:

```cpp
#include "mvhdp_device.h"
#include "../../include/mvhdp.h"

#include "mvhdp_wave.h"
#include <algorithm>

__global__ __launch_bounds__(256) void build_counts_kernel(MvModel mm, int m, int64_t n_tokens)
{
    extern __shared__ int nk_local[];
    const int K = mm.K;
    for (int i = threadIdx.x; i < K; i += blockDim.x) nk_local[i] = 0;
    __syncthreads();
    int32_t* nwk = mm.counts;
    const int64_t stride = (int64_t)gridDim.x * blockDim.x;
    for (int64_t i = (int64_t)blockIdx.x * blockDim.x + threadIdx.x; i < n_tokens; i += stride) {
        int topic = mm.z[m][i];
        if (topic == MVHDP_UNASSIGNED_TOPIC) continue;
        int type = mm.tok[m][i];
        if (type < 0 || type >= mm.V[m] || topic < 0 || topic >= K) continue;
        atomicAdd(&nk_local[topic], 1);
        atomicAdd(&nwk[(mm.rowbase[m] + type) * K + topic], 1);
    }
    __syncthreads();
    int32_t* nk = mm.counts + mm.rowbase[mm.M] * K + (int64_t)m * K;
    for (int i = threadIdx.x; i < K; i += blockDim.x)
        if (nk_local[i]) atomicAdd(&nk[i], nk_local[i]);
}

hipError_t mvhdp_launch_build_counts(const MvModel& mm, const int64_t* n_tokens, hipStream_t s)
{
    const int K = mm.K;
    size_t total = (size_t)(mm.rowbase[mm.M] * K + (int64_t)mm.M * K) * sizeof(int32_t);
    hipError_t e = hipMemsetAsync(mm.counts, 0, total, s);
    if (e != hipSuccess) return e;
    for (int m = 0; m < mm.M; m++) {
        if (n_tokens[m] <= 0) continue;
        int64_t blocks = (n_tokens[m] + 255) / 256;
        int grid = (int)(blocks < 2048 ? blocks : 2048);
        hipLaunchKernelGGL(build_counts_kernel, dim3(grid), dim3(256), (size_t)K * sizeof(int), s, mm, m, n_tokens[m]);
        e = hipGetLastError();
        if (e != hipSuccess) return e;
    }
    return hipSuccess;
}

template <bool COHERENT = false>
__device__ __forceinline__ void tree_from_leaves(const MvModel& mm, int64_t row, double* t, int lane, bool write_full)
{
    const int K = mm.K;
    if (lane == 0) t[0] = 0.0;
    __syncthreads();
    if (K > 1) {
        int dmax = 31 - __clz(K - 1);
        for (int d = dmax; d >= 0; d--) {
            int lo = 1 << d, hi = min(2 << d, K);
            for (int i = lo + lane; i < hi; i += WAVE) t[i] = t[2 * i] + t[2 * i + 1];
            __syncthreads();
        }
    }
    if (write_full) {
        double* out = mm.trees + row * 2 * K;
        for (int i = lane; i < 2 * K; i += WAVE) out[i] = t[i];
    }
    if (lane == 0) { if (COHERENT) __hip_atomic_store(&mm.root[row], t[1], __ATOMIC_RELAXED, __HIP_MEMORY_SCOPE_AGENT); else mm.root[row] = t[1]; }
    double* dt = mm.dtab + row * (int64_t)mm.dt_nblk * 8;
    double2* o = (double2*)dt;
    for (int u = lane; u < mm.dt_nblk * 4; u += WAVE) {
        const int x = u >> 2, j = u & 3;
        int base = 0, dep = 0;
        if (x >= 1) {
            base = 1; dep = mm.dt_f;
            while (x >= base + (1 << dep)) { base += 1 << dep; dep += 3; }
        }
        const int b = (1 << dep) + (x - base);
        double v2[2];
#pragma unroll
        for (int h = 0; h < 2; h++) {
            const int q = 2 * j + h;
            const int node = (q == 0) ? b : (q < 3) ? 2 * b + (q - 1) : 4 * b + (q - 3);
            v2[h] = (q == 7) ? ((x == 0) ? t[1] : 0.0) : ((node < K) ? t[2 * node] : 0.0);
        }
        if (COHERENT) {
            __hip_atomic_store(&dt[2 * u], v2[0], __ATOMIC_RELAXED, __HIP_MEMORY_SCOPE_AGENT);
            __hip_atomic_store(&dt[2 * u + 1], v2[1], __ATOMIC_RELAXED, __HIP_MEMORY_SCOPE_AGENT);
        } else o[u] = make_double2(v2[0], v2[1]);
    }
    __syncthreads();
}

template <int TB>
__global__ __launch_bounds__(64) void build_trees_kernel(MvModel mm, bool inference_leaves, bool write_full, int64_t row_begin, int64_t row_end,
                                                         bool apply_first, unsigned long long* negatives, bool from_mirror, bool only_heavy = false)
{
    extern __shared__ double t[];
    const int K = mm.K, lane = threadIdx.x;
    const int64_t nrows = mm.rowbase[mm.M];
    const int32_t* nk_all = mm.counts + nrows * K;
    int neg = 0;
    __builtin_amdgcn_s_setprio(3);
    for (int64_t row = row_begin + blockIdx.x; row < row_end; row += gridDim.x) {
        if (only_heavy && mm.heavy[row] != MVHDP_ROW_HEAVY) continue;
        int m = 0;
        while (m + 1 < mm.M && row >= mm.rowbase[m + 1]) m++;
        int32_t* cnt = mm.counts + row * K;
        int32_t* dl = mm.delta + row * K;
        const int32_t* nk = nk_all + (int64_t)m * K;
        const double* al = mm.alpha + (int64_t)m * (K + 1);
        const double beta = mm.beta[m], beta_sum = mm.beta_sum[m], gamma = mm.gamma[m];
        uint16_t* c16 = mm.counts16 + row * K;
        const bool light_src = from_mirror && mm.heavy[row] != MVHDP_ROW_HEAVY;
        bool hv = false;
        if (!from_mirror) {
            long long sum = 0;
            for (int k0 = 0; k0 < K; k0 += WAVE * TB) {
                int cv[TB], dv[TB];
#pragma unroll
                for (int u = 0; u < TB; u++) {
                    const int k = k0 + u * WAVE + lane;
                    cv[u] = (k < K) ? cnt[k] : 0;
                    dv[u] = (apply_first && k < K) ? dl[k] : 0;
                }
#pragma unroll
                for (int u = 0; u < TB; u++) {
                    const int k = k0 + u * WAVE + lane;
                    if (k < K) {
                        int c = cv[u];
                        if (apply_first) {
                            const int d = dv[u];
                            if (d) { c += d; cnt[k] = c; dl[k] = 0; neg += c < 0; }
                        }
                        sum += c < 0 ? 70000 : c;
                    }
                }
            }
#pragma unroll
            for (int sft = 32; sft >= 1; sft >>= 1) sum += __shfl_xor(sum, sft, WAVE);
            hv = sum > 65534;
            if (lane == 0) mm.heavy[row] = hv ? MVHDP_ROW_HEAVY : (sum > 32767 ? MVHDP_ROW_BIG : 0);
        }
        for (int k0 = 0; k0 < K; k0 += WAVE * TB) {
            int cv[TB], nkv[TB];
            double alv[TB];
            bool inact[TB];
#pragma unroll
            for (int u = 0; u < TB; u++) {
                const int k = k0 + u * WAVE + lane;
                const bool in = k < K;
                cv[u] = in ? (light_src ? (int)c16[k] : cnt[k]) : 0;
                nkv[u] = in ? nk[k] : 0;
                alv[u] = (in && !inference_leaves) ? al[k] : 0.0;
                inact[u] = in && !inference_leaves && mm.inactive[k];
            }
#pragma unroll
            for (int u = 0; u < TB; u++) {
                const int k = k0 + u * WAVE + lane;
                if (k < K) {
                    const int c = cv[u];
                    if (light_src) cnt[k] = c;
                    else if (!from_mirror) c16[k] = hv ? (uint16_t)65535 : (uint16_t)c;
                    double leaf;
                    if (inference_leaves) {
                        leaf = ((double)c + beta) / ((double)nkv[u] + beta_sum);
                    } else if (inact[u]) {
                        leaf = 0.0;
                    } else {
                        double p_wt = ((double)c + beta) / ((double)nkv[u] + beta_sum);
                        leaf = gamma * alv[u] * p_wt;
                    }
                    t[K + k] = leaf;
                }
            }
        }
        tree_from_leaves(mm, row, t, lane, write_full);
    }
    if (apply_first && negatives) {
#pragma unroll
        for (int sft = 32; sft >= 1; sft >>= 1) neg += __shfl_xor(neg, sft, WAVE);
        if (lane == 0 && neg) atomicAdd(negatives, (unsigned long long)neg);
    }
}

hipError_t mvhdp_launch_build_trees(const MvModel& mm, bool inference_leaves, bool write_full, hipStream_t s, bool beside_samplers)
{
    if (!beside_samplers) return mvhdp_launch_build_trees_rows(mm, inference_leaves, write_full, 0, mm.rowbase[mm.M], false, nullptr, s);
    const int64_t nrows = mm.rowbase[mm.M];
    if (nrows <= 0) return hipSuccess;
    int grid = (int)(nrows < 65536 ? nrows : 65536);
    hipLaunchKernelGGL(build_trees_kernel<1>, dim3(grid), dim3(64), (size_t)2 * mm.K * sizeof(double), s, mm, inference_leaves, write_full,
                       (int64_t)0, nrows, false, (unsigned long long*)nullptr, false);
    return hipGetLastError();
}

hipError_t mvhdp_launch_build_trees_rows(const MvModel& mm, bool inference_leaves, bool write_full, int64_t row_begin, int64_t row_end,
                                         bool apply_first, unsigned long long* negatives, hipStream_t s)
{
    int64_t nrows = row_end - row_begin;
    if (nrows <= 0) return hipSuccess;
    int grid = (int)(nrows < 65536 ? nrows : 65536);
    if (mm.K > 512)
        hipLaunchKernelGGL(build_trees_kernel<8>, dim3(grid), dim3(64), (size_t)2 * mm.K * sizeof(double), s, mm, inference_leaves, write_full,
                           row_begin, row_end, apply_first, negatives, false);
    else
        hipLaunchKernelGGL(build_trees_kernel<4>, dim3(grid), dim3(64), (size_t)2 * mm.K * sizeof(double), s, mm, inference_leaves, write_full,
                           row_begin, row_end, apply_first, negatives, false);
    return hipGetLastError();
}

hipError_t mvhdp_launch_build_trees_from_mirror(const MvModel& mm, bool write_full, hipStream_t s, bool beside_samplers)
{
    const int64_t nrows = mm.rowbase[mm.M];
    if (nrows <= 0) return hipSuccess;
    int grid = (int)(nrows < 65536 ? nrows : 65536);
    if (beside_samplers)
        hipLaunchKernelGGL(build_trees_kernel<1>, dim3(grid), dim3(64), (size_t)2 * mm.K * sizeof(double), s, mm, false, write_full,
                           (int64_t)0, nrows, false, (unsigned long long*)nullptr, true);
    else if (mm.K > 512)
        hipLaunchKernelGGL(build_trees_kernel<8>, dim3(grid), dim3(64), (size_t)2 * mm.K * sizeof(double), s, mm, false, write_full,
                           (int64_t)0, nrows, false, (unsigned long long*)nullptr, true);
    else
        hipLaunchKernelGGL(build_trees_kernel<4>, dim3(grid), dim3(64), (size_t)2 * mm.K * sizeof(double), s, mm, false, write_full,
                           (int64_t)0, nrows, false, (unsigned long long*)nullptr, true);
    return hipGetLastError();
}

__global__ __launch_bounds__(256) void apply2_nk_kernel(int32_t* nk_dst, const int32_t* __restrict__ dA, int32_t* __restrict__ dB, int n, unsigned long long* negatives)
{
    const int i = blockIdx.x * blockDim.x + threadIdx.x;
    if (i >= n) return;
    int d = dA[i];
    if (dB) { const int d2 = dB[i]; if (d2) { d += d2; dB[i] = 0; } }
    if (d) { const int c = nk_dst[i] + d; nk_dst[i] = c; if (c < 0 && negatives) atomicAdd(negatives, 1ull); }
}

__global__ __launch_bounds__(256) void apply2_counts_kernel(MvModel mm, const int32_t* __restrict__ dA, int32_t* __restrict__ dB, bool use_mirror,
                                                           int64_t n_cells, int64_t n_all, unsigned long long* negatives)
{
    const int64_t stride = (int64_t)gridDim.x * blockDim.x;
    unsigned int* m32 = (unsigned int*)mm.counts16;
    const int K = mm.K;
    int neg = 0;
    __builtin_amdgcn_s_setprio(3);
    for (int64_t i = (int64_t)blockIdx.x * blockDim.x + threadIdx.x; i < n_all; i += stride) {
        int d = dA[i];
        if (dB) { const int d2 = dB[i]; if (d2) { d += d2; dB[i] = 0; } }
        if (!d) continue;
        const int old = __hip_atomic_fetch_add(&mm.counts[i], d, __ATOMIC_RELAXED, __HIP_MEMORY_SCOPE_AGENT);
        neg += old + d < 0;
        if (use_mirror && i < n_cells && mm.heavy[i / K] != MVHDP_ROW_HEAVY) __hip_atomic_fetch_add(&m32[i >> 1], (unsigned int)d << ((i & 1) * 16), __ATOMIC_RELAXED, __HIP_MEMORY_SCOPE_AGENT);
    }
    if (neg && negatives) atomicAdd(negatives, (unsigned long long)neg);
}

hipError_t mvhdp_launch_apply2_counts(const MvModel& dst, const int32_t* dA, int32_t* dB, bool use_mirror, unsigned long long* negatives, hipStream_t s)
{
    const int64_t cells = dst.rowbase[dst.M] * dst.K, all = cells + (int64_t)dst.M * dst.K;
    int grid = (int)std::min<int64_t>((all + 255) / 256, 4096);
    if (grid < 1) grid = 1;
    hipLaunchKernelGGL(apply2_counts_kernel, dim3(grid), dim3(256), 0, s, dst, dA, dB, use_mirror, cells, all, negatives);
    return hipGetLastError();
}

__global__ __launch_bounds__(256) void apply_sparse_kernel(MvModel mm, int32_t* __restrict__ d, bool use_mirror, int64_t n_cells, int64_t n_all)
{
    const int64_t stride = (int64_t)gridDim.x * blockDim.x;
    unsigned int* m32 = (unsigned int*)mm.counts16;
    const int K = mm.K;
    for (int64_t i = (int64_t)blockIdx.x * blockDim.x + threadIdx.x; i < n_all; i += stride) {
        const int dl = d[i];
        if (!dl) continue;
        mm.counts[i] += dl;
        d[i] = 0;
        if (use_mirror && i < n_cells && mm.heavy[i / K] != MVHDP_ROW_HEAVY) __hip_atomic_fetch_add(&m32[i >> 1], (unsigned int)dl << ((i & 1) * 16), __ATOMIC_RELAXED, __HIP_MEMORY_SCOPE_AGENT);
    }
}

hipError_t mvhdp_launch_apply_sparse(const MvModel& dst, int32_t* d, bool use_mirror, hipStream_t s)
{
    const int64_t cells = dst.rowbase[dst.M] * dst.K, all = cells + (int64_t)dst.M * dst.K;
    int grid = (int)std::min<int64_t>((all + 255) / 256, 8192);
    if (grid < 1) grid = 1;
    hipLaunchKernelGGL(apply_sparse_kernel, dim3(grid), dim3(256), 0, s, dst, d, use_mirror, cells, all);
    return hipGetLastError();
}

__global__ __launch_bounds__(64) void gate_kernel(const unsigned long long* qhead, unsigned long long threshold)
{
    const unsigned long long t0 = __builtin_amdgcn_s_memrealtime();
    for (int i = 0; i < 4000000; i++) {
        const unsigned long long v = __hip_atomic_load(qhead, __ATOMIC_RELAXED, __HIP_MEMORY_SCOPE_AGENT);
        if (v >= threshold) break;
        if (__builtin_amdgcn_s_memrealtime() - t0 > 200000000ull) break;
        __builtin_amdgcn_s_sleep(32);
    }
}

hipError_t mvhdp_launch_gate(const unsigned long long* qhead, unsigned long long threshold, hipStream_t s)
{
    hipLaunchKernelGGL(gate_kernel, dim3(1), dim3(64), 0, s, qhead, threshold);
    return hipGetLastError();
}

__global__ __launch_bounds__(256) void widen_mirror_kernel(MvModel mm)
{
    const int K = mm.K;
    const int64_t nrows = mm.rowbase[mm.M];
    const int lane = threadIdx.x & 63;
    const int64_t wstride = (int64_t)gridDim.x * (blockDim.x >> 6);
    for (int64_t row = (int64_t)blockIdx.x * (blockDim.x >> 6) + (threadIdx.x >> 6); row < nrows; row += wstride) {
        if (mm.heavy[row] == MVHDP_ROW_HEAVY) continue;
        const uint16_t* c16 = mm.counts16 + row * K;
        int32_t* cnt = mm.counts + row * K;
        for (int k = lane; k < K; k += WAVE) cnt[k] = (int)c16[k];
    }
}

hipError_t mvhdp_launch_widen_mirror(const MvModel& mm, hipStream_t s)
{
    const int64_t nrows = mm.rowbase[mm.M];
    if (nrows <= 0) return hipSuccess;
    int64_t blocks = (nrows + 3) / 4;
    hipLaunchKernelGGL(widen_mirror_kernel, dim3((unsigned int)(blocks < 16384 ? blocks : 16384)), dim3(256), 0, s, mm);
    return hipGetLastError();
}

__global__ __launch_bounds__(64) void live_coef_kernel(MvModel mm)
{
    const int K = mm.K, Kp = (K + 7) & ~7, m = blockIdx.x;
    const int32_t* nk = mm.counts + mm.rowbase[mm.M] * K + (int64_t)m * K;
    float* cf = mm.coef + (int64_t)m * Kp;
    float* smp = mm.coef + (int64_t)mm.M * Kp + (int64_t)m * K;
    for (int k = threadIdx.x; k < Kp; k += blockDim.x)
        cf[k] = (k >= K || mm.inactive[k]) ? 0.0f : (float)(mm.gamma[m] * mm.alpha[(int64_t)m * (K + 1) + k] / ((double)nk[k] + mm.beta_sum[m]));
    __syncthreads();
    if (threadIdx.x == 0) {
        const float beta32 = (float)mm.beta[m];
        float run = 0.0f;
        for (int k = 0; k < K; k++) { run += cf[k] * beta32; smp[k] = run; }
    }
}

template <int TB>
__global__ __launch_bounds__(64) void live_rows_prepare_kernel(MvModel mm, bool from_mirror, int32_t* heavy_list, unsigned int* heavy_n, int heavy_cap, int batch_cells)
{
    const int K = mm.K, lane = threadIdx.x;
    const int64_t nrows = mm.rowbase[mm.M];
    for (int64_t row = blockIdx.x; row < nrows; row += gridDim.x) {
        int m = 0;
        while (m + 1 < mm.M && row >= mm.rowbase[m + 1]) m++;
        const int32_t* cnt = mm.counts + row * K;
        uint16_t* c16 = mm.counts16 + row * K;
        const int Kp = (K + 7) & ~7;
        const float* cf = mm.coef + (int64_t)m * Kp;
        const float smp_total = mm.coef[(int64_t)mm.M * Kp + (int64_t)m * K + K - 1];
        const bool light_src = from_mirror && mm.heavy[row] != MVHDP_ROW_HEAVY;
        bool hv = false;
        if (!from_mirror) {
            long long sum = 0;
            for (int k0 = 0; k0 < K; k0 += WAVE * TB) {
                int cv[TB];
#pragma unroll
                for (int u = 0; u < TB; u++) { const int k = k0 + u * WAVE + lane; cv[u] = (k < K) ? cnt[k] : 0; }
#pragma unroll
                for (int u = 0; u < TB; u++) sum += cv[u] < 0 ? 70000 : cv[u];
            }
#pragma unroll
            for (int sft = 32; sft >= 1; sft >>= 1) sum += __shfl_xor(sum, sft, WAVE);
            hv = sum > 65534;
            if (lane == 0) mm.heavy[row] = hv ? MVHDP_ROW_HEAVY : (sum > 32767 ? MVHDP_ROW_BIG : 0);
        }
        double acc = 0.0, acc0 = 0.0;
        for (int k0 = 0; k0 < K; k0 += WAVE * TB) {
            int cv[TB];
            float fv[TB];
#pragma unroll
            for (int u = 0; u < TB; u++) {
                const int k = k0 + u * WAVE + lane;
                const bool in = k < K;
                cv[u] = in ? (light_src ? (int)c16[k] : cnt[k]) : 0;
                fv[u] = in ? cf[k] : 0.0f;
            }
#pragma unroll
            for (int u = 0; u < TB; u++) {
                const int k = k0 + u * WAVE + lane;
                if (k < K) {
                    if (!from_mirror) c16[k] = hv ? (uint16_t)65535 : (uint16_t)cv[u];
                    const double t = (double)fv[u] * (double)cv[u];
                    acc += t;
                    if (k < batch_cells) acc0 += t;
                }
            }
        }
#pragma unroll
        for (int sft = 32; sft >= 1; sft >>= 1) { acc += __shfl_xor(acc, sft, WAVE); acc0 += __shfl_xor(acc0, sft, WAVE); }
        if (lane == 0) { mm.root[row] = (double)smp_total + acc; mm.mass0[row] = (float)acc0; }
        if (lane == 0 && heavy_list && mm.heavy[row] == MVHDP_ROW_HEAVY) {
            const unsigned int i = atomicAdd(heavy_n, 1u);
            if ((int)i < heavy_cap) heavy_list[i] = (int32_t)row;
        }
    }
}

__global__ __launch_bounds__(64) void heavy_refresh_kernel(MvModel mm, const int32_t* heavy_list, const unsigned int* ctl , int heavy_cap, bool write_full)
{
    extern __shared__ double t[];
    const int K = mm.K, lane = threadIdx.x;
    const int64_t nrows = mm.rowbase[mm.M];
    const int32_t* nk_all = mm.counts + nrows * K;
    const unsigned long long t0 = __builtin_amdgcn_s_memrealtime();
    const int n = min((int)__hip_atomic_load(&ctl[0], __ATOMIC_RELAXED, __HIP_MEMORY_SCOPE_AGENT), heavy_cap);
#ifdef MVHDP_REFRESH_PRINT
    if (blockIdx.x == 0 && lane == 0) printf("[refresher] %d heavy rows\n", n);
#endif
    for (int pass = 0; pass < 1000000; pass++) {
        for (int i = blockIdx.x; i < n; i += gridDim.x) {
            const int64_t row = heavy_list[i];
            int m = 0;
            while (m + 1 < mm.M && row >= mm.rowbase[m + 1]) m++;
            const int32_t* cnt = mm.counts + row * K;
            const int32_t* nk = nk_all + (int64_t)m * K;
            const double* al = mm.alpha + (int64_t)m * (K + 1);
            const double beta = mm.beta[m], beta_sum = mm.beta_sum[m], gamma = mm.gamma[m];
            for (int k = lane; k < K; k += WAVE) {
                const int c = __hip_atomic_load(&cnt[k], __ATOMIC_RELAXED, __HIP_MEMORY_SCOPE_AGENT);
                t[K + k] = mm.inactive[k] ? 0.0 : gamma * al[k] * (((double)c + beta) / ((double)nk[k] + beta_sum));
            }
            tree_from_leaves<true>(mm, row, t, lane, write_full);
        }
#ifdef MVHDP_REFRESH_SLEEP_ONLY
        if (__builtin_amdgcn_s_memrealtime() - t0 > 300000ull) break;
        __builtin_amdgcn_s_sleep(127);
        continue;
#endif
        if (n <= (int)blockIdx.x) break;
        if (__hip_atomic_load(&ctl[1], __ATOMIC_RELAXED, __HIP_MEMORY_SCOPE_AGENT) != 0u) break;
        if (__builtin_amdgcn_s_memrealtime() - t0 > 200000000ull) break;
    }
}

hipError_t mvhdp_launch_heavy_refresh(const MvModel& mm, const int32_t* heavy_list, const unsigned int* ctl, int heavy_cap, int blocks, hipStream_t s)
{
    hipLaunchKernelGGL(heavy_refresh_kernel, dim3(blocks), dim3(64), (size_t)2 * mm.K * sizeof(double), s, mm, heavy_list, ctl, heavy_cap, getenv("MVHDP_REFRESH_FULL") != nullptr);
    return hipGetLastError();
}

__global__ void set_u32_kernel(unsigned int* p, unsigned int v) { __hip_atomic_store(p, v, __ATOMIC_RELAXED, __HIP_MEMORY_SCOPE_AGENT); }
hipError_t mvhdp_launch_set_u32(unsigned int* p, unsigned int v, hipStream_t s)
{
    hipLaunchKernelGGL(set_u32_kernel, dim3(1), dim3(1), 0, s, p, v);
    return hipGetLastError();
}

hipError_t mvhdp_launch_live_rows_prepare(const MvModel& mm, bool from_mirror, bool with_heavy_trees, int32_t* heavy_list, unsigned int* heavy_ctl, int heavy_cap, int batch_cells, hipStream_t s)
{
    const int64_t nrows = mm.rowbase[mm.M];
    hipLaunchKernelGGL(live_coef_kernel, dim3(mm.M), dim3(64), 0, s, mm);
    if (nrows <= 0) return hipGetLastError();
    const int grid = (int)(nrows < 65536 ? nrows : 65536);
    if (heavy_ctl) { hipError_t e = hipMemsetAsync(heavy_ctl, 0, 2 * sizeof(unsigned int), s); if (e != hipSuccess) return e; }
    if (mm.K > 512) hipLaunchKernelGGL(live_rows_prepare_kernel<8>, dim3(grid), dim3(64), 0, s, mm, from_mirror, heavy_list, heavy_ctl, heavy_cap, batch_cells);
    else hipLaunchKernelGGL(live_rows_prepare_kernel<4>, dim3(grid), dim3(64), 0, s, mm, from_mirror, heavy_list, heavy_ctl, heavy_cap, batch_cells);
    if (with_heavy_trees)
        hipLaunchKernelGGL(build_trees_kernel<4>, dim3(grid), dim3(64), (size_t)2 * mm.K * sizeof(double), s, mm, false, false, (int64_t)0, nrows, false,
                           (unsigned long long*)nullptr, true, true);
    return hipGetLastError();
}

__global__ __launch_bounds__(256) void apply_nk_kernel(int32_t* counts_nk, int32_t* delta_nk, int n, unsigned long long* negatives)
{
    const int i = blockIdx.x * blockDim.x + threadIdx.x;
    if (i >= n) return;
    const int d = delta_nk[i];
    if (d) { const int c = counts_nk[i] + d; counts_nk[i] = c; delta_nk[i] = 0; if (c < 0 && negatives) atomicAdd(negatives, 1ull); }
}

hipError_t mvhdp_launch_apply_nk(const MvModel& mm, unsigned long long* negatives, hipStream_t s)
{
    const int n = mm.M * mm.K;
    const int64_t off = mm.rowbase[mm.M] * mm.K;
// ... 833 lines not shown
```

mvtopicmodel_amd/csrc/mvhdp_plan.h:

```cpp
#pragma once
#include <stdint.h>
#include <stddef.h>
#include <algorithm>
#include <cmath>
#include <cstring>

#include "mvhdp_device.h"
#include "../../include/mvhdp.h"

enum { PLAN_STREAM_MAIN = 0, PLAN_STREAM_A = 1, PLAN_STREAM_B = 2, PLAN_STREAM_C = 3, PLAN_STREAM_D = 4, PLAN_N_STREAMS = 5 };

struct PlanRegs { int regs[MVHDP_N_CLASSES][3]; };

struct PlanIn {
    int K = 0, M = 0;
    int64_t D = 0;
    int64_t mdt = 0;
    int64_t n_longer[5] = {0, 0, 0, 0, 0};
    bool have_order = false;
    unsigned long long tok_hist[MVHDP_HIST_BINS] = {0};
    unsigned long long ent_hist[MVHDP_ENT_BINS] = {0};
    uint32_t flags = 0;
    bool debug = false;
    bool batch = false;
    bool trees_current = false;
    bool unassigned = false;
    int first_inactive = -1;
    int num_cus = 256;
    size_t max_lds = 160 * 1024;
    PlanRegs regs{};
};

struct ClassLaunch {
    bool used = false;
    bool fast = false;
    int r = 0;
    int S_cap = 0;
    uint32_t wave_bytes = 0;
    int wpb = 0;
    size_t lds = 0;
    int grid = 0;
    int stream = PLAN_STREAM_MAIN;
    int walk = 0, narrow = 0;
    double theta[MVHDP_MAXM] = {0};
};

struct SweepPlan {
    int err = 0;
    const char* msg = "";
    uint32_t flags = 0;
    bool live = false, seg_apply = false, frozen = false, debug = false;
    bool overlap = false;
    int nseg = 1;
    int only_seg = -1;
    int S_cap = 0;
    bool fast = false;
    int pc = 0;
    bool route = false;
    int64_t H = 0;
    ClassLaunch cls[MVHDP_N_CLASSES];
    int class_map[MVHDP_N_CLASSES] = {0, 1, 2, 3, 4, 5};
    bool need_full = false;
    int nk_global = 0;
    uint32_t block_shared_bytes = 0;
    bool delta16 = false;
    bool live16 = false;
    bool live_rows = false;
    bool coef_lds = false;
    int dominant = 0;
    int walk_cfg = 0;
};

static inline double plan_class_tokens(const unsigned long long* tok_hist, int c)
{
    double t = 0;
    for (int b = 0; b < MVHDP_HIST_BINS; b++) {
        const int rounds = b + 1;
        int cb = 0;
        while (cb < 5 && rounds > (1 << cb)) cb++;
        if (b == MVHDP_HIST_BINS - 1) cb = 5;
        if (cb == c) t += (double)tok_hist[b];
    }
    return t;
}

static inline int plan_blocks_per_cu(int regs, int threads, size_t lds)
{
    int r = (regs + 7) / 8 * 8;
    int waves_simd = r > 0 ? 512 / r : 8;
    waves_simd = std::max(1, std::min(8, waves_simd));
    const int wpb = threads / 64;
    int b = waves_simd * 4 / wpb;
    b = std::min(b, (int)((160 * 1024) / (lds > 0 ? lds : 1)));
    b = std::min(b, 32 / wpb);
    return std::max(1, b);
}

size_t mvhdp_sweep_wave_bytes(int M, int S_cap);
size_t mvhdp_sweep_fast_wave_bytes(int M, int S_cap, int rmax);

struct PlanTuning {
    int force_primary = 0;
    int narrow = -1;
    int walk_fixed = 0;
    double walk_theta[MVHDP_MAXM] = {0};
    double primary_min_share = 0.10;
    int single_stream = 0;
    int four_round_on_c = -1;
    int delta16 = 1;
    int narrow_wide = 1;
    int fork_delay_us = 0;
    int widest_on_main = 0;
    int live_overlap = -1;
    int single_wave = 0;
    int live16 = -1;
    int live_rows = -1;
    int live_rows_segments = 1;
    int coef_lds_max_bytes = 12 * 1024;
    double live_rows_theta = 0.3;
};

enum { WALK_GROUPS = 3 };
struct WalkTuner {
    int walk_i = 0, walk_probe_i = 0, walk_b_i = 0, walk_phase = 0, walk_dir = 1, walk_fails = 0, walk_wait = 4, walk_cfg = -1, walk_maxj = 6;
    bool walk_far = false;
    double walk_ns_a1 = 0.0, walk_ns_b = 0.0;
    int walk_cls = 2, walk_i_by[WALK_GROUPS] = {-1, -1, -1};
    int walk_default[WALK_GROUPS] = {0, 0, 0};

    void init_defaults(int K)
    {
        if (K >= 256) { walk_default[0] = 6; walk_default[1] = MVHDP_WALK_BINS; walk_default[2] = 9; }
        walk_i = walk_default[walk_cls];
    }
    int stored(int g) const { return walk_i_by[g] >= 0 ? walk_i_by[g] : walk_default[g]; }
    double walk_cap = 0.004;
    long long walk_idle_until = 0, walk_refresh_at = 0, sweeps_done = 0;
    double walk_f[MVHDP_MAXM] = {-1, -1, -1, -1, -1, -1, -1, -1};
    double walk_hist[MVHDP_WALK_BINS] = {0};

    bool controlled(int m) const { return walk_f[m] >= 0.0 && walk_f[m] < 0.35; }
    bool any_controlled(int M) const { for (int m = 0; m < M; m++) if (controlled(m)) return true; return false; }
    bool any_unknown(int M) const { for (int m = 0; m < M; m++) if (walk_f[m] < 0.0) return true; return false; }

    void propose(int grp, int M, double theta[WALK_GROUPS][MVHDP_MAXM], bool* measure)
    {
        if (grp != walk_cls) {
            walk_i_by[walk_cls] = walk_i;
            walk_i = stored(grp);
            walk_cls = grp;
            walk_phase = 0; walk_far = false;
        }
        const bool any = any_controlled(M);
        const int top = MVHDP_WALK_BINS;
        walk_probe_i = walk_i;
        if (walk_phase == 1 && any) {
            if (walk_far && walk_i < 4) walk_far = false;
            if (walk_far) walk_dir = -1;
            if (walk_dir > 0 && walk_i >= top) walk_dir = -1;
            if (walk_dir < 0 && walk_i <= 0) walk_dir = 1;
            if (walk_dir > 0) {
                int j = 1;
                double extra = walk_hist[walk_i];
                while (walk_i + j < top && j < walk_maxj && extra + walk_hist[walk_i + j] <= walk_cap) { extra += walk_hist[walk_i + j]; j++; }
                walk_probe_i = walk_i + j;
            } else walk_probe_i = walk_far ? walk_i / 2 : walk_i - 1;
        }
        for (int m = 0; m < MVHDP_MAXM; m++) {
            const bool c = m < M && controlled(m);
            for (int g = 0; g < WALK_GROUPS; g++) theta[g][m] = c ? (double)(g == grp ? walk_probe_i : stored(g)) / MVHDP_WALK_BINS : 0.0;
        }
        *measure = false;
        if (!any && sweeps_done >= walk_refresh_at) { *measure = true; walk_refresh_at = sweeps_done + 16; }
        if (any_unknown(M)) *measure = true;
    }

    void measured(int M, int nseg, const unsigned long long* view_stats )
    {
        double all = 0.0;
        for (int m = 0; m < M; m++) {
            const double n = (double)view_stats[m * MVHDP_VIEW_STATS];
            all += n;
            if (n >= 64) walk_f[m] = (double)view_stats[m * MVHDP_VIEW_STATS + 1] / n;
            else if (nseg == 1) walk_f[m] = 1.0;
        }
        for (int b = 0; b < MVHDP_WALK_BINS; b++) {
            double c = 0.0;
            for (int m = 0; m < M; m++)
                if (controlled(m)) c += (double)view_stats[m * MVHDP_VIEW_STATS + 2 + b];
            walk_hist[b] = all > 0 ? c / all : 0.0;
        }
    }
// ... 143 lines not shown
    auto geometry = [&](bool is_fast, int c, int walk, ClassLaunch& g) -> bool {
        const int r = 1 << c;
        g.fast = is_fast; g.r = is_fast ? r : 0;
        g.S_cap = is_fast ? std::min(S_cap, 64 * r) : S_cap;
        g.wave_bytes = (uint32_t)(is_fast ? mvhdp_sweep_fast_wave_bytes(M, g.S_cap, r) : mvhdp_sweep_wave_bytes(M, S_cap));
        g.wpb = 4;
        while (g.wpb > 1 && p.block_shared_bytes + (size_t)g.wpb * g.wave_bytes > in.max_lds) g.wpb >>= 1;
        g.lds = p.block_shared_bytes + (size_t)g.wpb * g.wave_bytes;
        if (g.lds > in.max_lds) return false;
        const int regs = is_fast ? in.regs.regs[c][in.debug ? 2 : (walk ? 1 : 0)] : in.regs.regs[5][in.debug ? 2 : 0];
        const int bpc = plan_blocks_per_cu(regs, 64 * g.wpb, g.lds);
        const int64_t need = (in.D + (int64_t)g.wpb * MVHDP_DOC_BATCH - 1) / ((int64_t)g.wpb * MVHDP_DOC_BATCH);
        g.grid = (int)std::max<int64_t>(1, std::min<int64_t>(need, (int64_t)in.num_cus * ((p.overlap && bpc > 1) ? bpc - 1 : bpc)));
        if (tu.single_wave) { g.wpb = 1; g.lds = p.block_shared_bytes + g.wave_bytes; g.grid = 1; }
        return true;
    };

    const bool mirror_ok = fast && !in.debug && tu.narrow != 0 && (!(flags & MVHDP_SWEEP_REUSE_TREES) || in.trees_current) &&
                           !((flags & MVHDP_SWEEP_SEGMENT_OVERLAP) && in.unassigned);
    const bool want_live16 = mirror_ok && p.live && !p.frozen && !in.unassigned && (tu.live16 > 0 || (tu.live16 < 0 && K >= 256));
    auto group_of = [&](int c) { return c != 0 ? 2 : ((mirror_ok && (!p.live || want_live16)) ? 0 : 1); };
    double theta[WALK_GROUPS][MVHDP_MAXM] = {{0}};
    bool measure = false;
    if (tu.walk_fixed) {
        for (int g = 0; g < WALK_GROUPS; g++) for (int m = 0; m < MVHDP_MAXM; m++) theta[g][m] = tu.walk_theta[m];
        measure = true;
    } else wt.propose(fast ? group_of(p.dominant) : 2, M, theta, &measure);
    const bool mirror_pays = mirror_ok && !p.live && K >= 256;
    auto walk_of = [&](int c) { const int g = group_of(c); bool w = measure || in.debug || mirror_pays; for (int m = 0; m < M; m++) w = w || theta[g][m] > 0.0; return w ? 1 : 0; };

    ClassLaunch gen;
    if (!geometry(false, 5, 0, gen)) return fail(MVHDP_ERR_UNSUPPORTED, "per-entity LDS state exceeds 160 KiB (K * modalities too large)");
    gen.used = false;
    if (fast) {
        ClassLaunch pg;
        if (!geometry(true, pc, walk_of(pc), pg)) fast = false;
    }
    p.fast = fast;
    p.pc = fast ? pc : 5;
    const bool four_on_c = tu.four_round_on_c > 0 || (tu.four_round_on_c < 0 && !unknown && tok[2] < 0.03 * tot);
    const int stream_of[MVHDP_N_CLASSES] = {PLAN_STREAM_C, PLAN_STREAM_C, four_on_c ? PLAN_STREAM_C : PLAN_STREAM_D, PLAN_STREAM_B, PLAN_STREAM_A, PLAN_STREAM_A};
    if (!fast) {
        p.cls[5] = gen; p.cls[5].used = true; p.cls[5].stream = PLAN_STREAM_MAIN;
        for (int c = 0; c < MVHDP_N_CLASSES; c++) p.class_map[c] = 5;
        p.route = false; p.H = 0;
        p.need_full = true;
    } else {
        p.H = (S_cap > (64 << pc)) ? (in.have_order ? in.n_longer[pc] : in.D) : 0;
        if (view_16 && pc >= 3) p.H = in.have_order ? std::max<int64_t>(p.H, in.n_longer[4]) : in.D;
        p.route = p.H > 0;
        for (int c = pc; c < MVHDP_N_CLASSES; c++) {
            const bool reachable = c == pc || (p.route && (c <= c_max || (c == 5 && view_16)));
            const bool populated = c == pc || unknown || in.ent_hist[c] != 0 || (c == 5 && view_16);
            if (!(reachable && populated)) continue;
            ClassLaunch g;
            const int w = walk_of(c);
            if (c < 5 && geometry(true, c, w, g)) { g.walk = w; }
            else { g = gen; g.walk = 0; }
            g.used = true;
            g.stream = (c == pc || tu.single_stream || tu.single_wave) ? PLAN_STREAM_MAIN : stream_of[c];
            for (int m = 0; m < MVHDP_MAXM; m++) g.theta[m] = theta[group_of(c)][m];
            p.cls[c] = g;
        }
        if (!tu.single_stream && !tu.single_wave && tu.widest_on_main) {
            int next = PLAN_STREAM_MAIN;
            for (int c = MVHDP_N_CLASSES - 1; c >= pc; c--) if (p.cls[c].used) { p.cls[c].stream = next; next = std::min(next + 1, (int)PLAN_STREAM_D); }
        }
        for (int c = 0; c < MVHDP_N_CLASSES; c++) {
            int t = std::max(c, pc);
            while (t < MVHDP_N_CLASSES && !p.cls[t].used) t++;
            p.class_map[c] = t < MVHDP_N_CLASSES ? t : -1;
        }
        p.need_full = in.debug;
        for (int c = pc; c < MVHDP_N_CLASSES; c++) if (p.cls[c].used && !p.cls[c].fast) p.need_full = true;
        if (p.route && p.class_map[5] < 0 && (c_max == 5 || view_16)) {
            p.cls[5] = gen; p.cls[5].used = true; p.cls[5].stream = tu.single_stream ? PLAN_STREAM_MAIN : PLAN_STREAM_A; p.class_map[5] = 5; p.need_full = true;
        }
    }
    if (mirror_ok && !p.live && p.cls[0].used && p.cls[0].fast && p.cls[0].walk) p.cls[0].narrow = 1;
    if (mirror_ok && !p.live && tu.narrow_wide && tu.narrow != 1)
        for (int c = 1; c < 5; c++) if (p.cls[c].used && p.cls[c].fast && p.cls[c].walk) p.cls[c].narrow = 1;
    p.delta16 = tu.delta16 != 0 && mirror_ok && !p.live && !p.frozen && !p.seg_apply && nseg == 1 && p.only_seg < 0 &&
                !(flags & MVHDP_SWEEP_NO_APPLY) && !in.unassigned;
    if (want_live16) {
        bool all_fast = true;
        for (int c = 0; c < MVHDP_N_CLASSES; c++) if (p.cls[c].used && !p.cls[c].fast) all_fast = false;
        if (all_fast) {
            p.live16 = true;
            for (int c = 0; c < MVHDP_N_CLASSES; c++) if (p.cls[c].used) { p.cls[c].walk = 1; p.cls[c].narrow = 1; }
        }
    }
    if (want_rows) {
        bool all_fast = p.fast;
        for (int c = 0; c < MVHDP_N_CLASSES; c++) if (p.cls[c].used && !p.cls[c].fast) all_fast = false;
        if (all_fast) {
            p.live_rows = true;
            p.need_full = false;
            for (int c = 0; c < MVHDP_N_CLASSES; c++)
                if (p.cls[c].used) {
                    p.cls[c].walk = 1;
                    for (int m = 0; m < MVHDP_MAXM; m++) p.cls[c].theta[m] = (m < M && wt.controlled(m)) ? tu.live_rows_theta : 0.0;
                }
        } else p.coef_lds = false;
    } else p.coef_lds = false;
    p.walk_cfg = (p.live_rows ? 1 << 20 : 0) + (p.fast ? (1 << p.dominant) : 32) * 2 + (p.route ? 1 : 0) + 64 * nseg + (p.live ? 1 << 16 : 0) + (p.seg_apply ? 1 << 17 : 0) + (p.live16 ? 1 << 18 : 0) + (p.overlap ? 1 << 19 : 0);
}
```

mvtopicmodel_amd/csrc/mvhdp_sweep_fast.hip:

```cpp
#include "mvhdp_device.h"
#include "../../include/mvhdp.h"
#include "mvhdp_wave.h"

size_t mvhdp_sweep_fast_wave_bytes(int M, int S_cap, int rmax)
{
    size_t counts = (size_t)M * S_cap * (rmax >= 8 ? 2 : 4);
    size_t b = (size_t)(64 + 64 + 64 + 16 + S_cap) * 4 + counts;
    b += (size_t)M * M * 12;
    return (b + 15) & ~(size_t)15;
}

#ifndef MVHDP_LB1
#define MVHDP_LB1 1
#endif
#ifndef MVHDP_LB1W
#define MVHDP_LB1W 7
#endif
#ifndef MVHDP_LB2
#define MVHDP_LB2 7
#endif
#ifndef MVHDP_LB2_ROOMY
#define MVHDP_LB2_ROOMY 6
#endif
#ifndef MVHDP_LB4
#define MVHDP_LB4 4
#endif
#ifndef MVHDP_NB2_FROM
#define MVHDP_NB2_FROM 4
#endif
#ifndef MVHDP_LB16
#define MVHDP_LB16 1
#endif
#ifndef MVHDP_LB_ROWS
#define MVHDP_LB_ROWS 7
#endif
#ifndef MVHDP_LB8
#define MVHDP_LB8 1
#endif
#ifndef MVHDP_GATHER_SC
#define MVHDP_GATHER_SC 0
#endif
template <typename T>
__device__ __forceinline__ int gather_cell(gptr_t p)
{
    const __attribute__((address_space(1))) T* q = (const __attribute__((address_space(1))) T*)p;
#if MVHDP_GATHER_SC == 1
    return (int)__hip_atomic_load(q, __ATOMIC_RELAXED, __HIP_MEMORY_SCOPE_AGENT);
#elif MVHDP_GATHER_SC == 3
    return (int)__hip_atomic_load(q, __ATOMIC_RELAXED, __HIP_MEMORY_SCOPE_SYSTEM);
#elif MVHDP_GATHER_SC == 4
    return (int)__builtin_nontemporal_load(q);
#else
    return (int)*q;
#endif
}
#define W_HEAVY 0x40000000
#define W_BIG   0x20000000
#define W_ROW(w) ((w) & 0x1fffffff)
typedef unsigned int rowq_t __attribute__((ext_vector_type(4), aligned(4)));
typedef float coefq_t __attribute__((ext_vector_type(4)));

__device__ __forceinline__ int smoothing_sample_live(const float* __restrict__ smp, int K, float t, int lane)
{
    for (int k0 = 0; k0 < K; k0 += WAVE) {
        const int k = k0 + lane;
        const float p = (k < K) ? smp[k] : 3.0e38f;
        const unsigned long long hit = __builtin_amdgcn_ballot_w64(p > t && k < K);
        if (hit) return k0 + (int)__builtin_ctzll(hit);
    }
    return K - 1;
}

template <bool CELL16>
__device__ __forceinline__ rowq_t row_batch_load(gptr_t rowp, int K, int b, int lane)
{
    constexpr int CPL = CELL16 ? 8 : 4;
    const int k = (b * WAVE + lane) * CPL;
    rowq_t q = {0u, 0u, 0u, 0u};
    if (k < K) q = *(const __attribute__((address_space(1))) rowq_t*)(rowp + (unsigned int)k * (CELL16 ? 2u : 4u));
    return q;
}

typedef float f2_t __attribute__((ext_vector_type(2)));
template <bool CELL16>
__device__ __forceinline__ int row_batch_pick(rowq_t q, coefq_t c0, coefq_t c1, int kb, float base, float target, bool force, float& tot, bool& any)
{
    constexpr int CPL = CELL16 ? 8 : 4, NS = CPL / 2;
    f2_t n2[NS], k2[NS], A[NS];
    if (CELL16) {
        n2[0] = f2_t{(float)(q.x & 0xffffu), (float)(q.x >> 16)}; n2[1] = f2_t{(float)(q.y & 0xffffu), (float)(q.y >> 16)};
        n2[NS - 2] = f2_t{(float)(q.z & 0xffffu), (float)(q.z >> 16)}; n2[NS - 1] = f2_t{(float)(q.w & 0xffffu), (float)(q.w >> 16)};
        k2[0] = f2_t{c0.x, c0.y}; k2[1] = f2_t{c0.z, c0.w}; k2[NS - 2] = f2_t{c1.x, c1.y}; k2[NS - 1] = f2_t{c1.z, c1.w};
    } else {
        n2[0] = f2_t{(float)(int)q.x, (float)(int)q.y}; n2[NS - 1] = f2_t{(float)(int)q.z, (float)(int)q.w};
        k2[0] = f2_t{c0.x, c0.y}; k2[NS - 1] = f2_t{c0.z, c0.w};
    }
    A[0] = n2[0] * k2[0];
#pragma unroll
    for (int s = 1; s < NS; s++) A[s] = __builtin_elementwise_fma(n2[s], k2[s], A[s - 1]);
    const float ev = A[NS - 1].x;
    const float acc = ev + A[NS - 1].y;
    const float incl = wave_incl_scan_f_dpp(acc);
    tot = bcast_f(incl, 63);
    const unsigned long long pos = __builtin_amdgcn_ballot_w64(acc > 0.0f);
    any = pos != 0;
    if (!pos || !(force || base + tot > target)) return -1;
    const unsigned long long hit = force ? 0ull : (__builtin_amdgcn_ballot_w64(base + incl > target) & pos);
    const int hl = hit ? (int)__builtin_ctzll(hit) : 63 - (int)__builtin_clzll(pos);
    const float thr = target - (base + (hl > 0 ? bcast_f(incl, hl - 1) : 0.0f));
    int cnt = 0;
#pragma unroll
    for (int s = 0; s < NS; s++) cnt += (A[s].x <= thr) ? 1 : 0;
#pragma unroll
    for (int s = 0; s < NS; s++) cnt += (ev + A[s].y <= thr) ? 1 : 0;
    int p = force ? CPL : bcast_i(cnt, hl);
    if (p >= CPL) {
        int lp = 0;
#pragma unroll
        for (int s = 0; s < NS; s++) if (n2[s].x > 0.0f && k2[s].x > 0.0f) lp = s;
#pragma unroll
        for (int s = 0; s < NS; s++) if (n2[s].y > 0.0f && k2[s].y > 0.0f) lp = NS + s;
        p = bcast_i(lp, hl);
    }
    return kb + hl * CPL + (p < NS ? 2 * p : 2 * (p - NS) + 1);
}

template <bool CELL16, bool TWOB>
__device__ __forceinline__ int row_sample_live(rowq_t q0, bool have_q0, bool in_lds, const __attribute__((address_space(3))) float* cf_lds, const float* __restrict__ cf_g, const float* __restrict__ smp, float S,
                                                gptr_t rowp, int K, float u2f, float rootf, int bq, float mass0, int lane, unsigned long long* t_after_wait)
{
    constexpr int CPL = CELL16 ? 8 : 4;
    (void)t_after_wait;
    float target = u2f * rootf;
    if (target < S) return smoothing_sample_live(smp, K, target, lane);
    target -= S;
    float base = 0.0f;
    int lastb = -1;
    const int nb = (K + WAVE * CPL - 1) / (WAVE * CPL);
    if (!TWOB || nb != 2) bq = 0;
    const float bbase = bq ? mass0 : 0.0f;
    if (have_q0 && in_lds) {
// ... 226 lines not shown
            const double pmj = pd ? pd[lane] : 1.0;
            qsh[lane] = pmj * (mm.gamma[pj] * mm.alpha[(int64_t)pj * (K + 1) + K]) / dd;
            wsh[lane] = (pj != pm && wlen[pj] != 0) ? (float)(pmj / dd) : 0.0f;
        }
        LDS_FENCE();
        MVHDP_TMAIN(tp, tt, te);
        bool aborted = false;

        for (int m = 0; m < M && !aborted; m++) {
            const int lenm = uniform_i(wlen[m]);
            if (lenm == 0) continue;
            const double beta_m = mm.beta[m];
            const double scale_m = (double)lenm + mm.gamma[m] * mm.alpha_sum[m];
            const double p_mm = pd ? pd[m * M + m] : 1.0;
            const int32_t* nk = nk_all + (int64_t)m * K;

            int cn[RMAX];
            double oth[RMAX], den[RMAX];
            unsigned int onz = 0;
            auto slot_consts = [&](int r, double& o, double& dn) {
                o = 0.0; dn = 1.0;
                const int i = lane * R_eff + r;
                if (r < R_eff && i < S_used) {
                    const int k = koff[r] >> 2;
                    double acc = 0.0;
                    for (int j = 0; j < M; j++) {
                        if (j == m) continue;
                        const int cj = sn_get(j * S + i);
                        const int lj = wlen[j];
                        if (lj != 0)
                            acc += pd[m * M + j] * ((double)cj + mm.gamma[j] * mm.alpha[(int64_t)j * (K + 1) + k])
                                   / ((double)lj + mm.gamma[j] * mm.alpha_sum[j]);
                    }
                    o = acc * scale_m;
                    dn = (double)nk[k] + mm.beta_sum[m];
                }
            };
            float rden32[RMAX], brden32[RMAX], oth32[RMAX];
            const float beta32 = (float)beta_m, scale32 = (float)scale_m;
            const float* const smp_m = mm.coef + (int64_t)M * Kp + (int64_t)m * K;
            const float smS = LIVEROWS ? uniform_f(smp_m[K - 1]) : 0.0f;
#pragma unroll
            for (int r = 0; r < RMAX; r++) {
                cn[r] = 0;
                const int i = lane * R_eff + r;
                const bool used = r < R_eff && i < S_used;
                if (SCREEN) {
                    float acc = 0.0f;
                    double dn = 1.0;
                    if (used) {
                        const int k = koff[r] >> 2;
                        cn[r] = sn_get(m * S + i);
                        for (int j = 0; j < M; j++) {
                            if (j == m) continue;
                            const int cj = sn_get(j * S + i);
                            if (cj != 0) onz |= 1u << r;
                            acc = __builtin_fmaf(wsh[m * M + j], (float)cj + (float)(mm.gamma[j] * mm.alpha[(int64_t)j * (K + 1) + k]), acc);
                        }
                        dn = (double)nk[k] + mm.beta_sum[m];
                    }
                    oth[r] = 0.0; den[r] = 1.0;
                    rden32[r] = __builtin_amdgcn_rcpf((float)dn);
                    brden32[r] = beta32 * rden32[r];
                    oth32[r] = acc * scale32;
                } else {
                    if (used) {
                        cn[r] = sn_get(m * S + i);
                        for (int j = 0; j < M; j++) if (j != m && sn_get(j * S + i) != 0) onz |= 1u << r;
                    }
                    slot_consts(r, oth[r], den[r]);
                    rden32[r] = 0.0f; brden32[r] = 0.0f; oth32[r] = 0.0f;
                }
            }
            double newAll = 0.0;
            for (int j = 0; j < M; j++) newAll += qsh[m * M + j];
            newAll = newAll * scale_m;
            const double newMass = (mm.first_inactive < 0) ? 0.0 : newAll / (double)K;
            const float pmm32 = uniform_f((float)p_mm), newMass32 = uniform_f((float)newMass);

            const int64_t base = mm.doc_off[m][d];
            const int64_t row0 = mm.rowbase[m];
            const char* nwk_v = (const char*)(nwk + row0 * K);
            const char* nwk16_v = (const char*)(nwk16 + row0 * K);
            int koffh[RMAX];
#pragma unroll
            for (int r = 0; r < RMAX; r++) koffh[r] = koff[r] >> 1;
            const int Vm = mm.V[m];
            const double walk_theta = sl.walk_theta[m];
            const unsigned int v_tok0 = n_tok, v_tree0 = c_tree;
            unsigned int whist_l = 0;

            MVHDP_TMAIN(tv, te, te);
            for (int c0 = 0; c0 < lenm && !aborted; c0 += WAVE) {
                const int ti = c0 + lane;
                const bool tvalid = ti < lenm;
                int w_l = tvalid ? mm.tok[m][base + ti] : -1;
                int z_l = tvalid ? mm.z[m][base + ti] : -1;
                int so_l = -1;
                if (z_l >= 0) {
                    uint32_t w = bitmap[z_l >> 5];
                    so_l = prefix[z_l >> 5] + __popc(w & ((1u << (z_l & 31)) - 1u));
                }
                double u1_l, u2_l;
                {
                    uint32_t x[4];
                    philox4x32_10((uint32_t)ti, (uint32_t)m, (uint32_t)dg, sl.sweep_idx,
                                  sl.seed_lo, sl.seed_hi ^ (uint32_t)((unsigned long long)dg >> 32), x);
                    u1_l = bits_to_unit(x[0], x[1]);
                    u2_l = bits_to_unit(x[2], x[3]);
                }
                MVHDP_TSUB2(tp);
                if (w_l >= Vm) w_l = -1;
                if (NARROW && w_l >= 0) {
                    const int hv = mm.heavy[row0 + w_l];
                    if (hv) w_l |= (hv == MVHDP_ROW_HEAVY) ? (W_HEAVY | W_BIG) : W_BIG;
                }
                const float u1f_l = (float)u1_l;
                int znew_l = z_l;

                double root_l = 0.0;
                int zt_l = -1, st_l = -1;
                const bool heavy_l = NARROW && w_l >= 0 && (w_l & W_HEAVY);
                const bool walk_l = tvalid && w_l >= 0 && (!WALK || u1_l >= walk_theta) && (!LIVEROWS || heavy_l);
                const unsigned long long walked = WALK ? __ballot(walk_l) : ~0ull;
                const unsigned long long specm = LIVEROWS ? __ballot(tvalid && w_l >= 0 && !heavy_l && u1_l >= walk_theta) : 0ull;
                rowq_t rowq = {0u, 0u, 0u, 0u};
                if (WALK && tvalid && w_l >= 0 && !walk_l) root_l = mm.root[row0 + W_ROW(w_l)];
                {
                    const bool act = walk_l;
                    const double* __restrict__ dt = mm.dtab + (row0 + W_ROW(max(w_l, 0))) * (int64_t)mm.dt_nblk * 8;
                    double u = 0.0;
                    int i = 1;
                    for (int bd = 0; bd < mm.dt_nbd; bd++) {
                        if (act && (bd == 0 || i < K)) {
                            const double2* __restrict__ blk = (const double2*)(dt + (int64_t)(mm.dt_base[bd] + (i - (1 << mm.dt_depth[bd]))) * 8);
                            double2 q0, q1, q2, q3;
                            if (LIVEROWS) {
                                const double* bp = (const double*)blk;
                                q0.x = __hip_atomic_load(bp + 0, __ATOMIC_RELAXED, __HIP_MEMORY_SCOPE_AGENT); q0.y = __hip_atomic_load(bp + 1, __ATOMIC_RELAXED, __HIP_MEMORY_SCOPE_AGENT);
                                q1.x = __hip_atomic_load(bp + 2, __ATOMIC_RELAXED, __HIP_MEMORY_SCOPE_AGENT); q1.y = __hip_atomic_load(bp + 3, __ATOMIC_RELAXED, __HIP_MEMORY_SCOPE_AGENT);
                                q2.x = __hip_atomic_load(bp + 4, __ATOMIC_RELAXED, __HIP_MEMORY_SCOPE_AGENT); q2.y = __hip_atomic_load(bp + 5, __ATOMIC_RELAXED, __HIP_MEMORY_SCOPE_AGENT);
                                q3.x = __hip_atomic_load(bp + 6, __ATOMIC_RELAXED, __HIP_MEMORY_SCOPE_AGENT); q3.y = __hip_atomic_load(bp + 7, __ATOMIC_RELAXED, __HIP_MEMORY_SCOPE_AGENT);
                            } else { q0 = blk[0]; q1 = blk[1]; q2 = blk[2]; q3 = blk[3]; }
                            const int levels = (bd == 0) ? mm.dt_f : 3;
                            if (bd == 0) { root_l = q3.y; u = u2_l * root_l; }
                            int path = 0;
                            if (i < K && levels > 0) {
                                const double l = q0.x;
                                if (u < l) { i = 2 * i; } else { u = u - l; i = 2 * i + 1; path = 1; }
                            }
                            if (i < K && levels > 1) {
                                const double l = path ? q1.x : q0.y;
                                if (u < l) { i = 2 * i; path = 2 * path; } else { u = u - l; i = 2 * i + 1; path = 2 * path + 1; }
                                if (i < K && levels > 2) {
                                    const double l3 = (path == 0) ? q1.y : (path == 1) ? q2.x : (path == 2) ? q2.y : q3.x;
                                    if (u < l3) { i = 2 * i; } else { u = u - l3; i = 2 * i + 1; }
                                }
                            }
                        }
                    }
                    if (act) {
                        zt_l = i - K;
                        const uint32_t wbit = bitmap[zt_l >> 5];
                        if ((wbit >> (zt_l & 31)) & 1u) st_l = (int)(prefix[zt_l >> 5] + __popc(wbit & ((1u << (zt_l & 31)) - 1u)));
                    }
                }

                MVHDP_TSUB2(tv);
                const float root32_l = (float)root_l;
                const float u2f_l = LIVEROWS ? (float)u2_l : 0.0f;
                unsigned long long bselm = 0ull;
                if (LIVEROWS == 2) {
                    constexpr int BCELLS = WAVE * (NARROW ? 8 : 4);
                    if (K > BCELLS && K <= 2 * BCELLS) {
                        float mass0_l = 0.0f;
                        if (tvalid && w_l >= 0 && !heavy_l) mass0_l = mm.mass0[row0 + W_ROW(w_l)];
                        bselm = __ballot(tvalid && w_l >= 0 && !heavy_l && (u2f_l * root32_l) - smS >= mass0_l);
                    }
                }
                MVHDP_TMAIN(th, te, tt);
                constexpr int NB = (RMAX >= MVHDP_NB2_FROM) ? 2 : 1;
                int gn[RMAX], gn2[RMAX];
                unsigned long long rem = __ballot(tvalid && w_l >= 0);
                n_oov += (unsigned int)__popcll(__ballot(tvalid && w_l < 0));
                n_tok += (unsigned int)__popcll(rem);
                const int t_first = rem ? (int)__builtin_ctzll(rem) : 0;
#pragma unroll
                for (int a = 0; a < NB; a++) {
                    const unsigned long long ra = (a == 0) ? rem : (rem & (rem - 1));
                    const int w0 = bcast_i(w_l, ra ? (int)__builtin_ctzll(ra) : t_first);
                    const unsigned int r0 = (unsigned int)W_ROW(max(w0, 0));
                    const bool h0 = w0 >= 0 && (w0 & W_HEAVY);
                    if (NARROW && !h0) {
                        const gptr_t c0q = scalar_row(nwk16_v, r0, (unsigned int)K * 2u);
#pragma unroll
                        for (int r = 0; r < RMAX; r++) { const int v = gather_cell<uint16_t>(c0q + (unsigned int)koffh[r]); if (a == 0) gn[r] = v; else gn2[r] = v; }
                    } else {
                        const gptr_t c0p = scalar_row(nwk_v, r0, (unsigned int)K * 4u);
#pragma unroll
                        for (int r = 0; r < RMAX; r++) { const int v = gather_cell<int32_t>(c0p + (unsigned int)koff[r]); if (a == 0) gn[r] = v; else gn2[r] = v; }
                    }
                }

                while (rem) {
                    const int t = (int)__builtin_ctzll(rem);
                    rem &= ~(1ull << t);
#define TOK_T t
#define TOK_G gn
#include "mvhdp_sweep_fast_token.inc"
#undef TOK_T
#undef TOK_G
                    if (NB == 2 && rem) {
                        const int t1 = (int)__builtin_ctzll(rem);
                        rem &= ~(1ull << t1);
#define TOK_T t1
#define TOK_G gn2
#include "mvhdp_sweep_fast_token.inc"
#undef TOK_T
#undef TOK_G
                    }
                }

                MVHDP_TMAIN(tt, te, te);
                {
                    const bool chg = tvalid && (w_l >= 0) && (znew_l != z_l) && !(sl.flags & MVHDP_SWEEP_FROZEN);
                    n_chg += (unsigned int)__popcll(__ballot(chg));
                    if (chg) {
                        const int64_t rowK = (row0 + W_ROW(w_l)) * K;
                        if (NARROW && sl.live16 && !(w_l & W_HEAVY)) {
                            unsigned int* m32 = (unsigned int*)mm.counts16;
                            if (z_l >= 0) { const int64_t c = rowK + z_l; __hip_atomic_fetch_add(&m32[c >> 1], 0u - (1u << ((c & 1) * 16)), __ATOMIC_RELAXED, __HIP_MEMORY_SCOPE_AGENT); }
                            { const int64_t c = rowK + znew_l; __hip_atomic_fetch_add(&m32[c >> 1], 1u << ((c & 1) * 16), __ATOMIC_RELAXED, __HIP_MEMORY_SCOPE_AGENT); }
                        } else if (NARROW && sl.delta16 && !(w_l & W_BIG)) {
                            unsigned int* d32 = (unsigned int*)mm.delta16;
                            if (z_l >= 0) { const int64_t c = rowK + z_l; __hip_atomic_fetch_add(&d32[c >> 1], 0u - (1u << ((c & 1) * 16)), __ATOMIC_RELAXED, __HIP_MEMORY_SCOPE_AGENT); }
                            { const int64_t c = rowK + znew_l; __hip_atomic_fetch_add(&d32[c >> 1], 1u << ((c & 1) * 16), __ATOMIC_RELAXED, __HIP_MEMORY_SCOPE_AGENT); }
                        } else {
#ifdef MVHDP_PROBE
                            const int probe = (int)((sl.flags >> 16) & 7u);
                            int64_t c_old = rowK + z_l, c_new = rowK + znew_l;
                            if (probe == 1) { c_old &= 0xffff; c_new &= 0xffff; }
                            if (probe == 7) { c_old &= 0xfffff; c_new &= 0xfffff; }
                            if (probe == 5) { c_old &= 0x7fffff; c_new &= 0x7fffff; }
                            if (probe == 6) { c_old &= 0xffffff; c_new &= 0xffffff; }
                            if (probe == 3) { if (z_l >= 0) dnwk[c_old] = -1; dnwk[c_new] = 1; }
                            else if (probe == 4) { if (z_l >= 0) __hip_atomic_fetch_add(&dnwk[c_old], -1, __ATOMIC_RELAXED, __HIP_MEMORY_SCOPE_WORKGROUP); __hip_atomic_fetch_add(&dnwk[c_new], 1, __ATOMIC_RELAXED, __HIP_MEMORY_SCOPE_WORKGROUP); }
                            else {
                                if (z_l >= 0) __hip_atomic_fetch_add(&dnwk[c_old], -1, __ATOMIC_RELAXED, __HIP_MEMORY_SCOPE_AGENT);
                                if (probe != 2) __hip_atomic_fetch_add(&dnwk[c_new], 1, __ATOMIC_RELAXED, __HIP_MEMORY_SCOPE_AGENT);
                            }
#else
                            if (z_l >= 0) __hip_atomic_fetch_add(&dnwk[rowK + z_l], -1, __ATOMIC_RELAXED, __HIP_MEMORY_SCOPE_AGENT);
                            __hip_atomic_fetch_add(&dnwk[rowK + znew_l], 1, __ATOMIC_RELAXED, __HIP_MEMORY_SCOPE_AGENT);
#endif
                        }
                        if (z_l >= 0) {
                            if (sl.nk_global) __hip_atomic_fetch_add(&dnk_g[m * K + z_l], -1, __ATOMIC_RELAXED, __HIP_MEMORY_SCOPE_AGENT);
                            else __hip_atomic_fetch_add(&nkd[m * K + z_l], -1, __ATOMIC_RELAXED, __HIP_MEMORY_SCOPE_WORKGROUP);
                        }
                        if (sl.nk_global) __hip_atomic_fetch_add(&dnk_g[m * K + znew_l], 1, __ATOMIC_RELAXED, __HIP_MEMORY_SCOPE_AGENT);
                        else __hip_atomic_fetch_add(&nkd[m * K + znew_l], 1, __ATOMIC_RELAXED, __HIP_MEMORY_SCOPE_WORKGROUP);
                        if (mm.first_inactive >= 0 && mm.inactive[znew_l]) {
                            long long key = (long long)MVHDP_ACT_KEY(dg, m, ti, znew_l);
                            atomicMin(sl.act_key, key);
                            if (sl.births) {
                                const int r_ = sl.births[2 + K + znew_l];
                                if (r_ >= 0) { atomicMin(&sl.birth_keys[r_], key); atomicMax(&sl.births[0], r_ + 1); }
                            }
                        }
                    }
                }
                if (tvalid) mm.z[m][base + ti] = znew_l;
                if (tvalid && znew_l >= 0) atomicOr(&bitmap2[znew_l >> 5], 1u << (znew_l & 31));
                if (sl.flags & MVHDP_SL_STRICT_LIVE) {
                    asm volatile("s_waitcnt vmcnt(0)" ::: "memory");
                    __builtin_amdgcn_fence(__ATOMIC_ACQUIRE, "agent");
// ... 188 lines not shown
```

mvtopicmodel_amd/csrc/mvhdp_sweep_fast_token.inc:

```
{
                    int g[RMAX];
#pragma unroll
                    for (int r = 0; r < RMAX; r++) g[r] = TOK_G[r];
                    const int wfull_t = LIVEROWS ? bcast_i(w_l, TOK_T) : 0;
                    const gptr_t rowp_t = !LIVEROWS ? (gptr_t)0 : NARROW ? scalar_row(nwk16_v, (unsigned int)W_ROW(wfull_t), (unsigned int)K * 2u)
                                                                         : scalar_row(nwk_v, (unsigned int)W_ROW(wfull_t), (unsigned int)K * 4u);
                    const bool spec_t = LIVEROWS && ((specm >> TOK_T) & 1ull);
                    const int bsel_t = (LIVEROWS == 2) ? (int)((bselm >> TOK_T) & 1ull) : 0;
                    if (LIVEROWS) {
#pragma unroll
                        for (int r = 0; r < RMAX; r++) asm volatile("" : "+v"(g[r]));
                        if (spec_t) rowq = row_batch_load<NARROW>(rowp_t, K, bsel_t, lane);
                    }
                    const unsigned long long rem_n = (NB == 2) ? (rem & (rem - 1)) : rem;
#pragma unroll
                    for (int r = 0; r < RMAX; r++) { touch_lane_off(koff[r]); if (NARROW) touch_lane_off(koffh[r]); }
                    if (NB == 2 || LIVEROWS || rem_n) {
                        const int wn = bcast_i(w_l, rem_n ? (int)__builtin_ctzll(rem_n) : TOK_T);
                        if (NARROW && !(wn & W_HEAVY)) {
                            const gptr_t cnq = scalar_row(nwk16_v, (unsigned int)W_ROW(wn), (unsigned int)K * 2u);
#pragma unroll
                            for (int r = 0; r < RMAX; r++) TOK_G[r] = gather_cell<uint16_t>(cnq + (unsigned int)koffh[r]);
                        } else {
                            const gptr_t cnp = scalar_row(nwk_v, (unsigned int)W_ROW(wn), (unsigned int)K * 4u);
#pragma unroll
                            for (int r = 0; r < RMAX; r++) TOK_G[r] = gather_cell<int32_t>(cnp + (unsigned int)koff[r]);
                        }
                    }
                    const int w = W_ROW(bcast_i(w_l, TOK_T));
                    const int so = bcast_i(so_l, TOK_T);
                    const int64_t row = row0 + w;

                    if (so >= 0) {
                        const int rs = so & (R_eff - 1), ls = so >> lg;
#pragma unroll
                        for (int r = 0; r < RMAX; r++) {
                            if (rs == r) {
                                const int c = bcast_i(cn[r], ls) - 1;
                                cn[r] = wave_writelane(cn[r], c, ls);
                                if (c == 0 && !((bcast_i((int)onz, ls) >> r) & 1)) live_m[r] &= ~(1ull << ls);
                            }
                        }
                    }

                    double mass = 0.0, s0 = 0.0, s1 = 0.0, total = 0.0;
                    int branch = 2, slot_new = -1;
                    bool unsafe = false;
                    double term[RMAX] = {};
                    bool need64 = DEBUG || exact_only || !SCREEN;
                    if (SCREEN && !need64) {
                        const float u1f = bcast_f(u1f_l, TOK_T), rootf = bcast_f(root32_l, TOK_T);
                        float t32[RMAX], c32v[RMAX];
#pragma unroll
                        for (int r = 0; r < RMAX; r++) {
                            const float pw = __builtin_fmaf((float)g[r], rden32[r], brden32[r]);
                            const float a32 = __builtin_fmaf(pmm32, (float)cn[r], oth32[r]);
                            t32[r] = __builtin_amdgcn_inverse_ballot_w64(live_m[r]) ? a32 * pw : 0.0f;
                        }
                        float ls = t32[0];
                        c32v[0] = ls;
#pragma unroll
                        for (int r = 1; r < RMAX; r++) { ls += t32[r]; c32v[r] = ls; }
                        const float incl = wave_incl_scan_f_dpp(ls);
                        const float excl = incl - ls;
#pragma unroll
                        for (int r = 0; r < RMAX; r++) c32v[r] = (r == RMAX - 1) ? incl : excl + c32v[r];
                        const float massf = bcast_f(incl, 63);
                        const float totalf = (newMass32 + massf) + rootf;
                        const float s0f = u1f * totalf;
                        const float tolf = totalf * 0x1.0p-17f;
                        bool close;
                        if (s0f < newMass32) {
                            branch = 0;
                            close = fabsf(s0f - newMass32) <= tolf;
                        } else {
                            const float s1f = s0f - newMass32;
                            close = (fabsf(s1f) <= tolf) || (fabsf(s1f - massf) <= tolf);
                            if (s1f < massf) {
                                branch = 1;
                                unsigned long long anyhit = 0, near = 0, hitr[RMAX];
#pragma unroll
                                for (int r = 0; r < RMAX; r++) {
                                    const float diff = c32v[r] - s1f;
                                    near |= __builtin_amdgcn_ballot_w64(fabsf(diff) <= tolf) & live_m[r];
                                    hitr[r] = __builtin_amdgcn_ballot_w64(diff >= 0.0f) & live_m[r];
                                    anyhit |= hitr[r];
                                }
                                close = close || near != 0;
                                if (anyhit) {
                                    if (RMAX <= 4) {
                                        unsigned int best = ~0u;
#pragma unroll
                                        for (int r = 0; r < RMAX; r++) {
                                            const unsigned int fl = hitr[r] ? (unsigned int)__builtin_ctzll(hitr[r]) : 0x0fffffffu;
                                            best = min(best, fl * (unsigned int)R_eff + (unsigned int)r);
                                        }
                                        slot_new = (int)best;
                                    } else {
                                        const int hl = (int)__builtin_ctzll(anyhit);
                                        int rr = 0;
#pragma unroll
                                        for (int r = RMAX - 1; r >= 0; r--) if ((hitr[r] >> hl) & 1ull) rr = r;
// ... 195 lines not shown
```

mvtopicmodel_amd/java/mvhdp_jni.cpp:

```cpp
#include <jni.h>

#include <condition_variable>
#include <cstdio>
#include <cstring>
#include <mutex>
#include <set>
#include <vector>

#include "mvhdp.h"

namespace {

struct Shard {
    mvhdp_handle h = nullptr;
    int K = 0, M = 0;
    int V[MVHDP_MAX_MODALITIES] = {};
    jlong D = -1;
    jlong N[MVHDP_MAX_MODALITIES] = {};
    int pins = 0;
};

std::mutex g_reg_mutex;
std::condition_variable g_reg_cv;
std::set<void*> g_shards, g_groups;
// ... 268 lines not shown
        std::vector<double> pcopy;
        if (pOverride) { pcopy.resize(static_cast<size_t>(env->GetArrayLength(pOverride))); env->GetDoubleArrayRegion(pOverride, 0, (jsize)pcopy.size(), pcopy.data()); }
        rc = mvhdp_sweep(s->h, static_cast<uint32_t>(sweepIdx), static_cast<uint64_t>(seed), static_cast<uint32_t>(flags),
                         pOverride ? pcopy.data() : nullptr, nullptr, &st);
    }
    if (rc) { throw_rt(env, s->h, rc, "mvhdp_sweep"); return; }
    jclass c = env->GetObjectClass(out);
    auto setL = [&](const char* f, jlong v) { env->SetLongField(out, env->GetFieldID(c, f, "J"), v); };
    auto setI = [&](const char* f, jint v) { env->SetIntField(out, env->GetFieldID(c, f, "I"), v); };
    auto setD = [&](const char* f, jdouble v) { env->SetDoubleField(out, env->GetFieldID(c, f, "D"), v); };
    setL("tokens", st.tokens); setL("changed", st.changed); setL("newMassCnt", st.new_mass_cnt);
    setL("topicDocMassCnt", st.topic_doc_mass_cnt); setL("wordFTreeMassCnt", st.word_ftree_mass_cnt);
    setL("oovSkipped", st.oov_skipped); setL("abortedDocs", st.aborted_docs); setL("exactFallbacks", st.exact_fallbacks);
    setI("activatedTopic", st.activated_topic); setI("activatedModality", st.activated_modality);
    setL("activationKey", st.activation_key); setD("sweepKernelMs", st.sweep_kernel_ms); setD("totalMs", st.total_ms);
    setI("activations", st.activations);
}

JNIEXPORT void JNICALL Java_org_madgik_MVTopicModel_NativeSampler_nApplyDelta(JNIEnv* env, jclass, jlong p, jint topic, jint modality)
{ ShardPin pin_(p); Shard* s = pin_.s; if (!s) { throw_msg(env, "java/lang/IllegalStateException", "NativeSampler is closed"); return; }
  int rc = mvhdp_apply_delta(s->h, topic, modality); if (rc) throw_rt(env, s->h, rc, "mvhdp_apply_delta"); }

JNIEXPORT void JNICALL Java_org_madgik_MVTopicModel_NativeSampler_nModelLogLikelihood(JNIEnv* env, jclass, jlong p, jdoubleArray out)
{
    ShardPin pin_(p); Shard* s = pin_.s;
    if (!s) { throw_msg(env, "java/lang/IllegalStateException", "NativeSampler is closed"); return; }
    if (bad_len(env, out, s->M, "modelLogLikelihood")) return;
    double ll[MVHDP_MAX_MODALITIES];
    int rc = mvhdp_model_log_likelihood(s->h, ll);
    if (rc) { throw_rt(env, s->h, rc, "mvhdp_model_log_likelihood"); return; }
    env->SetDoubleArrayRegion(out, 0, s->M, ll);
}

static void stats_to_longs(const mvhdp_sweep_stats& st, jlong* o)
{
    o[0] = st.tokens; o[1] = st.changed; o[2] = st.new_mass_cnt; o[3] = st.topic_doc_mass_cnt;
    o[4] = st.word_ftree_mass_cnt; o[5] = st.oov_skipped; o[6] = st.aborted_docs; o[7] = st.exact_fallbacks;
}

JNIEXPORT void JNICALL Java_org_madgik_MVTopicModel_NativeSampler_nSweepMany(JNIEnv* env, jclass, jlong p, jint firstIdx, jint n, jlong seed, jint flags, jlongArray statsFlat)
{
    ShardPin pin_(p); Shard* s = pin_.s;
    if (!s) { throw_msg(env, "java/lang/IllegalStateException", "NativeSampler is closed"); return; }
    if (n < 0 || (statsFlat && bad_len(env, statsFlat, (jlong)n * 8, "sweepMany stats [n][8]"))) return;
    std::vector<mvhdp_sweep_stats> st(static_cast<size_t>(n > 0 ? n : 1));
    int rc = mvhdp_sweep_many(s->h, static_cast<uint32_t>(firstIdx), n, static_cast<uint64_t>(seed), static_cast<uint32_t>(flags), st.data());
    if (rc) { throw_rt(env, s->h, rc, "mvhdp_sweep_many"); return; }
    if (statsFlat) {
        std::vector<jlong> flat(static_cast<size_t>(n) * 8);
        for (int i = 0; i < n; i++) stats_to_longs(st[i], flat.data() + (size_t)i * 8);
        env->SetLongArrayRegion(statsFlat, 0, (jsize)flat.size(), flat.data());
    }
}

JNIEXPORT void JNICALL Java_org_madgik_MVTopicModel_NativeSampler_nGetTuning(JNIEnv* env, jclass, jlong p, jintArray ints, jdoubleArray doubles)
{
    ShardPin pin_(p); Shard* s = pin_.s;
    if (!s) { throw_msg(env, "java/lang/IllegalStateException", "NativeSampler is closed"); return; }
    if (bad_len(env, ints, 8, "getTuning ints") || bad_len(env, doubles, 17, "getTuning doubles")) return;
    mvhdp_tuning t;
    int rc = mvhdp_get_tuning(s->h, &t);
    if (rc) { throw_rt(env, s->h, rc, "mvhdp_get_tuning"); return; }
    const jint iv[8] = {t.force_primary, t.narrow, t.walk_fixed, t.single_stream, t.live16, t.learnt_walk_step[0], t.learnt_walk_step[1], t.learnt_walk_step[2]};
    jdouble dv[17];
    dv[0] = t.primary_min_share;
    for (int m = 0; m < 8; m++) { dv[1 + m] = t.walk_theta[m]; dv[9 + m] = t.tree_branch_share[m]; }
    env->SetIntArrayRegion(ints, 0, 8, iv);
    env->SetDoubleArrayRegion(doubles, 0, 17, dv);
}

JNIEXPORT void JNICALL Java_org_madgik_MVTopicModel_NativeSampler_nSetTuning(JNIEnv* env, jclass, jlong p, jintArray ints, jdoubleArray doubles)
{
    ShardPin pin_(p); Shard* s = pin_.s;
    if (!s) { throw_msg(env, "java/lang/IllegalStateException", "NativeSampler is closed"); return; }
    if (bad_len(env, ints, 8, "setTuning ints") || bad_len(env, doubles, 17, "setTuning doubles")) return;
    jint iv[8]; jdouble dv[17];
    env->GetIntArrayRegion(ints, 0, 8, iv);
    env->GetDoubleArrayRegion(doubles, 0, 17, dv);
    mvhdp_tuning t;
    std::memset(&t, 0, sizeof t);
    t.force_primary = iv[0]; t.narrow = iv[1]; t.walk_fixed = iv[2]; t.single_stream = iv[3]; t.live16 = iv[4];
    t.learnt_walk_step[0] = iv[5]; t.learnt_walk_step[1] = iv[6]; t.learnt_walk_step[2] = iv[7]; t.learnt_walk_step[3] = -1;
    t.live_overlap = -1;
    t.primary_min_share = dv[0];
    for (int m = 0; m < 8; m++) { t.walk_theta[m] = dv[1 + m]; t.tree_branch_share[m] = dv[9 + m]; }
    int rc = mvhdp_set_tuning(s->h, &t);
    if (rc) throw_rt(env, s->h, rc, "mvhdp_set_tuning");
}

static void throw_group(JNIEnv* env, mvhdp_group g, int rc, const char* what)
{
    char msg[640];
    snprintf(msg, sizeof msg, "%s failed (%d): %s", what, rc, mvhdp_group_last_error(g));
    throw_msg(env, "java/lang/RuntimeException", msg);
}

JNIEXPORT jlong JNICALL Java_org_madgik_MVTopicModel_NativeSampler_nGroupCreate(JNIEnv* env, jclass, jlongArray handles)
{
    const jsize n = handles ? env->GetArrayLength(handles) : 0;
    if (n < 1) { throw_msg(env, "java/lang/IllegalArgumentException", "groupCreate: no members"); return 0; }
    std::vector<jlong> hp(static_cast<size_t>(n));
    env->GetLongArrayRegion(handles, 0, n, hp.data());
    std::vector<mvhdp_handle> hs;
    Group* gr = new Group();
    auto unpin_all = [&]() { std::lock_guard<std::mutex> lk(g_reg_mutex); for (Shard* s : gr->shards) if (--s->pins == 0) g_reg_cv.notify_all(); gr->shards.clear(); };
    for (jsize i = 0; i < n; i++) {
        Shard* s = nullptr;
        { std::lock_guard<std::mutex> lk(g_reg_mutex); if (g_shards.count(reinterpret_cast<void*>(hp[i]))) { s = reinterpret_cast<Shard*>(hp[i]); s->pins++; } }
        if (!s) { unpin_all(); delete gr; throw_msg(env, "java/lang/IllegalStateException", "groupCreate: a member is closed"); return 0; }
        gr->shards.push_back(s);
        hs.push_back(s->h);
    }
    int rc = mvhdp_group_create(n, hs.data(), &gr->g);
    if (rc != MVHDP_OK) { unpin_all(); delete gr; throw_group(env, nullptr, rc, "mvhdp_group_create"); return 0; }
    gr->members = n; gr->K = gr->shards[0]->K; gr->M = gr->shards[0]->M;
    { std::lock_guard<std::mutex> lk(g_reg_mutex); g_groups.insert(gr); }
    return reinterpret_cast<jlong>(gr);
}

JNIEXPORT void JNICALL Java_org_madgik_MVTopicModel_NativeSampler_nGroupUniqueId(JNIEnv* env, jclass, jbyteArray id)
{
    if (bad_len(env, id, MVHDP_UNIQUE_ID_BYTES, "groupUniqueId")) return;
    uint8_t buf[MVHDP_UNIQUE_ID_BYTES];
    int rc = mvhdp_group_unique_id(buf);
    if (rc) { throw_group(env, nullptr, rc, "mvhdp_group_unique_id"); return; }
    env->SetByteArrayRegion(id, 0, MVHDP_UNIQUE_ID_BYTES, reinterpret_cast<const jbyte*>(buf));
}

JNIEXPORT jlong JNICALL Java_org_madgik_MVTopicModel_NativeSampler_nGroupCreateRank(JNIEnv* env, jclass, jlong p, jbyteArray id, jint rank, jint nranks)
{
    Shard* s = nullptr;
    { std::lock_guard<std::mutex> lk(g_reg_mutex); if (g_shards.count(reinterpret_cast<void*>(p))) { s = reinterpret_cast<Shard*>(p); s->pins++; } }
    if (!s) { throw_msg(env, "java/lang/IllegalStateException", "NativeSampler is closed"); return 0; }
    auto unpin = [&]() { std::lock_guard<std::mutex> lk(g_reg_mutex); if (--s->pins == 0) g_reg_cv.notify_all(); };
    if (bad_len(env, id, MVHDP_UNIQUE_ID_BYTES, "groupCreateRank id")) { unpin(); return 0; }
    uint8_t buf[MVHDP_UNIQUE_ID_BYTES];
    env->GetByteArrayRegion(id, 0, MVHDP_UNIQUE_ID_BYTES, reinterpret_cast<jbyte*>(buf));
    Group* gr = new Group();
    int rc = mvhdp_group_create_rank(s->h, buf, rank, nranks, &gr->g);
    if (rc != MVHDP_OK) { unpin(); delete gr; throw_group(env, nullptr, rc, "mvhdp_group_create_rank"); return 0; }
    gr->members = 1; gr->K = s->K; gr->M = s->M; gr->shards.push_back(s);
    { std::lock_guard<std::mutex> lk(g_reg_mutex); g_groups.insert(gr); }
    return reinterpret_cast<jlong>(gr);
}

JNIEXPORT void JNICALL Java_org_madgik_MVTopicModel_NativeSampler_nGroupDestroy(JNIEnv*, jclass, jlong p)
{
    Group* gr = unregister_and_drain<Group>(g_groups, p);
    if (!gr) return;
    mvhdp_group_destroy(gr->g);
    { std::lock_guard<std::mutex> lk(g_reg_mutex); for (Shard* s : gr->shards) if (--s->pins == 0) g_reg_cv.notify_all(); }
    delete gr;
}

JNIEXPORT void JNICALL Java_org_madgik_MVTopicModel_NativeSampler_nGroupBuildCounts(JNIEnv* env, jclass, jlong p)
{
    GroupPin gpin_(p); Group* gr = gpin_.s;
    if (!gr) { throw_msg(env, "java/lang/IllegalStateException", "group is closed"); return; }
    int rc = mvhdp_group_build_counts(gr->g);
    if (rc) throw_group(env, gr->g, rc, "mvhdp_group_build_counts");
}

JNIEXPORT jdouble JNICALL Java_org_madgik_MVTopicModel_NativeSampler_nGroupSweep(JNIEnv* env, jclass, jlong p, jint sweepIdx, jlong seed, jint flags, jlongArray statsFlat, jintArray act)
{
    GroupPin gpin_(p); Group* gr = gpin_.s;
    if (!gr) { throw_msg(env, "java/lang/IllegalStateException", "group is closed"); return 0.0; }
// ... 227 lines not shown
```

Before: 6.765 billion.

## Add uint8 count mirror for rows whose maximum count fits a byte

Adds an 8-bit mirror of the word-topic count table, written when the tree build finds a light row whose largest count is at most 255, and marked with a new BYTE row-class bit. The narrow sweep paths gather counts from the byte mirror for such rows, cutting gather traffic relative to the 16-bit mirror. Any delta apply or mirror refresh clears the byte bit so stale byte data is never read. This costs extra memory, a lower vocabulary limit (row index loses a bit), and extra flag-handling branches in the apply kernels.

```diff
diff --git a/include/mvhdp.h b/include/mvhdp.h
--- a/include/mvhdp.h
+++ b/include/mvhdp.h
@@ -201,6 +201,7 @@
     double  tree_branch_share[MVHDP_MAX_MODALITIES];
     int32_t live_overlap;
     int32_t live_rows;
+    int32_t byte_rows;
 } mvhdp_tuning;
 int mvhdp_get_tuning(mvhdp_handle h, mvhdp_tuning* t);
 int mvhdp_set_tuning(mvhdp_handle h, const mvhdp_tuning* t);
diff --git a/mvtopicmodel_amd/_lib.py b/mvtopicmodel_amd/_lib.py
--- a/mvtopicmodel_amd/_lib.py
+++ b/mvtopicmodel_amd/_lib.py
@@ -69,7 +69,7 @@
                 ("live16", C.c_int32), ("single_wave", C.c_int32),
                 ("walk_theta", C.c_double * MAX_M), ("primary_min_share", C.c_double),
                 ("learnt_walk_step", C.c_int32 * 4), ("tree_branch_share", C.c_double * MAX_M),
-                ("live_overlap", C.c_int32), ("live_rows", C.c_int32)]
+                ("live_overlap", C.c_int32), ("live_rows", C.c_int32), ("byte_rows", C.c_int32)]
 
 
 class GroupInfoC(C.Structure):
diff --git a/mvtopicmodel_amd/csrc/mvhdp_api.hip b/mvtopicmodel_amd/csrc/mvhdp_api.hip
--- a/mvtopicmodel_amd/csrc/mvhdp_api.hip
+++ b/mvtopicmodel_amd/csrc/mvhdp_api.hip
@@ -42,6 +42,7 @@
     if (const char* f = getenv("MVHDP_LIVE_ROWS_SEGMENTS")) h->tu.live_rows_segments = std::max(1, std::min(255, atoi(f)));
     if (const char* f = getenv("MVHDP_WIDEST_ON_MAIN")) h->tu.widest_on_main = atoi(f) != 0;
     if (const char* f = getenv("MVHDP_NARROW_WIDE")) h->tu.narrow_wide = atoi(f) != 0;
+    if (const char* f = getenv("MVHDP_BYTE_ROWS")) h->tu.byte_rows = atoi(f) != 0 ? -1 : 0;
     if (const char* f = getenv("MVHDP_LIVE_TREE_EVERY")) h->live_tree_every = std::max(1, atoi(f));
     if (const char* f = getenv("MVHDP_GATE_PCT")) { const int v = atoi(f); if (v >= 5 && v <= 95) h->gate_pct = v; }
     if (const char* f = getenv("MVHDP_FOUR_ROUND_ON_C")) h->tu.four_round_on_c = atoi(f);
@@ -76,7 +77,7 @@
         return MVHDP_ERR_INVALID_ARG;
     }
     for (int m = 0; m < M; m++) if (cfg->num_types[m] < 1) { g_create_error = "num_types[m] must be >= 1"; return MVHDP_ERR_INVALID_ARG; }
-    for (int m = 0; m < M; m++) if (cfg->num_types[m] >= (1 << 29)) { g_create_error = "num_types[m] must be below 2^29"; return MVHDP_ERR_INVALID_ARG; }
+    for (int m = 0; m < M; m++) if (cfg->num_types[m] >= (1 << 28)) { g_create_error = "num_types[m] must be below 2^28"; return MVHDP_ERR_INVALID_ARG; }
     if (cfg->doc_id_base < 0 || cfg->doc_id_base >= (1LL << 29)) { g_create_error = "doc_id_base out of range"; return MVHDP_ERR_INVALID_ARG; }
     int ndev = 0;
     if (hipGetDeviceCount(&ndev) != hipSuccess || ndev <= 0 || cfg->device < 0 || cfg->device >= ndev) {
@@ -115,6 +116,8 @@
     CREATE_HIP(hipMemset(mm.counts, 0, cbytes));
     CREATE_HIP(hipMalloc(&mm.counts16, (size_t)nrows * K * sizeof(uint16_t) + 64));
     CREATE_HIP(hipMemset(mm.counts16, 0, (size_t)nrows * K * sizeof(uint16_t)));
+    CREATE_HIP(hipMalloc(&mm.counts8, (size_t)nrows * K + 64));
+    CREATE_HIP(hipMemset(mm.counts8, 0, (size_t)nrows * K));
     CREATE_HIP(hipMalloc(&mm.delta16, (size_t)(nrows * K + 2) * sizeof(uint16_t)));
     CREATE_HIP(hipMemsetD16(mm.delta16, (unsigned short)0x8000, (size_t)(nrows * K + 2)));
     CREATE_HIP(hipMalloc(&mm.heavy, (size_t)nrows));
@@ -175,7 +178,7 @@
     if (h->stream) hipStreamSynchronize(h->stream);
     auto fr = [](auto*& p) { if (p) { hipFree((void*)p); p = nullptr; } };
     for (int m = 0; m < MVHDP_MAXM; m++) { fr(h->d_doc_off[m]); fr(h->d_tok[m]); fr(h->d_z[m]); fr(h->d_carry[m]); fr(h->d_present[m]); }
-    fr(h->mm.counts); fr(h->mm.delta16); fr(h->mm.counts16); fr(h->mm.heavy); fr(h->mm.delta); fr(h->mm.trees); fr(h->mm.root); fr(h->mm.coef); fr(h->mm.mass0); fr(h->d_births); fr(h->d_birth_keys); fr(h->d_birth_table); fr(h->mm.dtab); fr(h->mm.p);
+    fr(h->mm.counts); fr(h->mm.delta16); fr(h->mm.counts16); fr(h->mm.counts8); fr(h->mm.heavy); fr(h->mm.delta); fr(h->mm.trees); fr(h->mm.root); fr(h->mm.coef); fr(h->mm.mass0); fr(h->d_births); fr(h->d_birth_keys); fr(h->d_birth_table); fr(h->mm.dtab); fr(h->mm.p);
     fr(h->d_alpha); fr(h->d_inactive); fr(h->d_ctl);
     if (h->h_ctl) { hipHostFree(h->h_ctl); h->h_ctl = nullptr; }
     h->d_stats = nullptr; h->d_act_key = nullptr; h->d_doc_counter = nullptr; h->d_ovf_meta = nullptr;
@@ -1088,6 +1091,7 @@
     sl.live_rows = p.live_rows ? 1 : 0;
     sl.coef_lds = p.coef_lds ? 1 : 0;
     sl.delta16 = p.delta16 ? 1 : 0;
+    sl.byte_rows = p.byte_rows ? 1 : 0;
     sl.stats = d_stats;
     sl.act_key = h->d_act_key;
     const bool births = sweep_births(p, flags, mm);
@@ -1515,6 +1519,7 @@
     t->force_primary = h->tu.force_primary; t->narrow = h->tu.narrow; t->walk_fixed = h->tu.walk_fixed;
     t->single_stream = h->tu.single_stream; t->primary_min_share = h->tu.primary_min_share; t->live16 = h->tu.live16;
     t->single_wave = h->tu.single_wave; t->live_overlap = h->tu.live_overlap; t->live_rows = h->tu.live_rows;
+    t->byte_rows = h->tu.byte_rows;
     for (int m = 0; m < MVHDP_MAX_MODALITIES; m++) { t->walk_theta[m] = h->tu.walk_theta[m]; t->tree_branch_share[m] = h->wt.walk_f[m]; }
     for (int g = 0; g < WALK_GROUPS; g++) t->learnt_walk_step[g] = g == h->wt.walk_cls ? h->wt.walk_i : h->wt.walk_i_by[g];
     t->learnt_walk_step[3] = -1;
@@ -1535,6 +1540,7 @@
     h->tu.single_wave = t->single_wave ? 1 : 0;
     h->tu.live_overlap = t->live_overlap < 0 ? -1 : (t->live_overlap ? 1 : 0);
     h->tu.live_rows = t->live_rows < 0 ? -1 : (t->live_rows ? 1 : 0);
+    h->tu.byte_rows = t->byte_rows != 0 ? -1 : 0;
     h->tu.primary_min_share = t->primary_min_share > 0.0 ? t->primary_min_share : 0.10;
     for (int m = 0; m < MVHDP_MAX_MODALITIES; m++) h->tu.walk_theta[m] = t->walk_theta[m];
     if (t->learnt_walk_step[0] >= 0 || t->learnt_walk_step[1] >= 0 || t->learnt_walk_step[2] >= 0) h->wt.restore(t->learnt_walk_step, t->tree_branch_share, h->mm.M);
@@ -1561,6 +1567,7 @@
     if (t) {
         tu.force_primary = t->force_primary; tu.narrow = t->narrow; tu.walk_fixed = t->walk_fixed; tu.single_stream = t->single_stream;
         tu.live16 = t->live16; tu.single_wave = t->single_wave ? 1 : 0; tu.live_overlap = t->live_overlap; tu.live_rows = t->live_rows;
+        tu.byte_rows = t->byte_rows != 0 ? -1 : 0;
         if (t->primary_min_share > 0) tu.primary_min_share = t->primary_min_share;
         for (int m = 0; m < MVHDP_MAX_MODALITIES; m++) tu.walk_theta[m] = t->walk_theta[m];
         if (t->learnt_walk_step[0] >= 0 || t->learnt_walk_step[1] >= 0 || t->learnt_walk_step[2] >= 0) wt.restore(t->learnt_walk_step, t->tree_branch_share, in.M);
diff --git a/mvtopicmodel_amd/csrc/mvhdp_device.h b/mvtopicmodel_amd/csrc/mvhdp_device.h
--- a/mvtopicmodel_amd/csrc/mvhdp_device.h
+++ b/mvtopicmodel_amd/csrc/mvhdp_device.h
@@ -20,6 +20,7 @@
     int32_t* counts;
     uint16_t* delta16;
     uint16_t* counts16;
+    uint8_t* counts8;
     uint8_t* heavy;
     int32_t* delta;
     double* trees;
@@ -40,6 +41,7 @@
 #define MVHDP_SL_STRICT_LIVE 0x8000u
 #define MVHDP_ROW_HEAVY 1
 #define MVHDP_ROW_BIG 2
+#define MVHDP_ROW_BYTE 4
 
 struct SweepLaunch {
     uint32_t sweep_idx;
@@ -63,6 +65,7 @@
     int32_t walk;
     int32_t narrow;
     int32_t delta16;
+    int32_t byte_rows;
     int32_t live16;
     int32_t live_rows;
     int32_t coef_lds;
diff --git a/mvtopicmodel_amd/csrc/mvhdp_group.hip b/mvtopicmodel_amd/csrc/mvhdp_group.hip
--- a/mvtopicmodel_amd/csrc/mvhdp_group.hip
+++ b/mvtopicmodel_amd/csrc/mvhdp_group.hip
@@ -469,6 +469,7 @@
     std::vector<uint8_t> cls((size_t)rows);
     GHIP(g, hipSetDevice(L0->device));
     GHIP(g, hipMemcpy(cls.data(), L0->mm.heavy, (size_t)rows, hipMemcpyDeviceToHost));
+    for (uint8_t& c : cls) c &= (uint8_t)(MVHDP_ROW_HEAVY | MVHDP_ROW_BIG);
     g->woff.assign((size_t)rows + 1, 0);
     for (int64_t r = 0; r < rows; r++) g->woff[(size_t)r + 1] = g->woff[(size_t)r] + (cls[(size_t)r] == 0 ? (K + 1) / 2 : K);
     if (g->d_woff.empty()) { g->d_woff.assign(g->leaders.size(), nullptr); g->d_cls.assign(g->leaders.size(), nullptr); g->xpack.assign(g->leaders.size(), nullptr); }
diff --git a/mvtopicmodel_amd/csrc/mvhdp_kernels.hip b/mvtopicmodel_amd/csrc/mvhdp_kernels.hip
--- a/mvtopicmodel_amd/csrc/mvhdp_kernels.hip
+++ b/mvtopicmodel_amd/csrc/mvhdp_kernels.hip
@@ -98,7 +98,7 @@
     int neg = 0;
     __builtin_amdgcn_s_setprio(3);
     for (int64_t row = row_begin + blockIdx.x; row < row_end; row += gridDim.x) {
-        if (only_heavy && mm.heavy[row] != MVHDP_ROW_HEAVY) continue;
+        if (only_heavy && !(mm.heavy[row] & MVHDP_ROW_HEAVY)) continue;
         int m = 0;
         while (m + 1 < mm.M && row >= mm.rowbase[m + 1]) m++;
         int32_t* cnt = mm.counts + row * K;
@@ -107,10 +107,14 @@
         const double* al = mm.alpha + (int64_t)m * (K + 1);
         const double beta = mm.beta[m], beta_sum = mm.beta_sum[m], gamma = mm.gamma[m];
         uint16_t* c16 = mm.counts16 + row * K;
-        const bool light_src = from_mirror && mm.heavy[row] != MVHDP_ROW_HEAVY;
-        bool hv = false;
+        uint8_t* c8 = mm.counts8 + row * K;
+        const int cls0 = mm.heavy[row];
+        const bool light_src = from_mirror && !(cls0 & MVHDP_ROW_HEAVY);
+        if (from_mirror && lane == 0 && (cls0 & MVHDP_ROW_BYTE)) mm.heavy[row] = (uint8_t)(cls0 & ~MVHDP_ROW_BYTE);
+        bool hv = false, byte_row = false;
         if (!from_mirror) {
             long long sum = 0;
+            int mx = 0;
             for (int k0 = 0; k0 < K; k0 += WAVE * TB) {
                 int cv[TB], dv[TB];
 #pragma unroll
@@ -129,13 +133,15 @@
                             if (d) { c += d; cnt[k] = c; dl[k] = 0; neg += c < 0; }
                         }
                         sum += c < 0 ? 70000 : c;
+                        mx = max(mx, c);
                     }
                 }
             }
 #pragma unroll
-            for (int sft = 32; sft >= 1; sft >>= 1) sum += __shfl_xor(sum, sft, WAVE);
+            for (int sft = 32; sft >= 1; sft >>= 1) { sum += __shfl_xor(sum, sft, WAVE); mx = max(mx, __shfl_xor(mx, sft, WAVE)); }
             hv = sum > 65534;
-            if (lane == 0) mm.heavy[row] = hv ? MVHDP_ROW_HEAVY : (sum > 32767 ? MVHDP_ROW_BIG : 0);
+            byte_row = !hv && mx <= 255;
+            if (lane == 0) mm.heavy[row] = (uint8_t)((hv ? MVHDP_ROW_HEAVY : (sum > 32767 ? MVHDP_ROW_BIG : 0)) | (byte_row ? MVHDP_ROW_BYTE : 0));
         }
         for (int k0 = 0; k0 < K; k0 += WAVE * TB) {
             int cv[TB], nkv[TB];
@@ -156,7 +162,10 @@
                 if (k < K) {
                     const int c = cv[u];
                     if (light_src) cnt[k] = c;
-                    else if (!from_mirror) c16[k] = hv ? (uint16_t)65535 : (uint16_t)c;
+                    else if (!from_mirror) {
+                        c16[k] = hv ? (uint16_t)65535 : (uint16_t)c;
+                        if (byte_row) c8[k] = (uint8_t)c;
+                    }
                     double leaf;
                     if (inference_leaves) {
                         leaf = ((double)c + beta) / ((double)nkv[u] + beta_sum);
@@ -245,7 +254,13 @@
         if (!d) continue;
         const int old = __hip_atomic_fetch_add(&mm.counts[i], d, __ATOMIC_RELAXED, __HIP_MEMORY_SCOPE_AGENT);
         neg += old + d < 0;
-        if (use_mirror && i < n_cells && mm.heavy[i / K] != MVHDP_ROW_HEAVY) __hip_atomic_fetch_add(&m32[i >> 1], (unsigned int)d << ((i & 1) * 16), __ATOMIC_RELAXED, __HIP_MEMORY_SCOPE_AGENT);
+        if (use_mirror && i < n_cells) {
+            const int cls = mm.heavy[i / K];
+            if (!(cls & MVHDP_ROW_HEAVY)) {
+                __hip_atomic_fetch_add(&m32[i >> 1], (unsigned int)d << ((i & 1) * 16), __ATOMIC_RELAXED, __HIP_MEMORY_SCOPE_AGENT);
+                if (cls & MVHDP_ROW_BYTE) mm.heavy[i / K] = (uint8_t)(cls & ~MVHDP_ROW_BYTE);
+            }
+        }
     }
     if (neg && negatives) atomicAdd(negatives, (unsigned long long)neg);
 }
@@ -269,7 +284,13 @@
         if (!dl) continue;
         mm.counts[i] += dl;
         d[i] = 0;
-        if (use_mirror && i < n_cells && mm.heavy[i / K] != MVHDP_ROW_HEAVY) __hip_atomic_fetch_add(&m32[i >> 1], (unsigned int)dl << ((i & 1) * 16), __ATOMIC_RELAXED, __HIP_MEMORY_SCOPE_AGENT);
+        if (use_mirror && i < n_cells) {
+            const int cls = mm.heavy[i / K];
+            if (!(cls & MVHDP_ROW_HEAVY)) {
+                __hip_atomic_fetch_add(&m32[i >> 1], (unsigned int)dl << ((i & 1) * 16), __ATOMIC_RELAXED, __HIP_MEMORY_SCOPE_AGENT);
+                if (cls & MVHDP_ROW_BYTE) mm.heavy[i / K] = (uint8_t)(cls & ~MVHDP_ROW_BYTE);
+            }
+        }
     }
 }
 
@@ -306,7 +327,9 @@
     const int lane = threadIdx.x & 63;
     const int64_t wstride = (int64_t)gridDim.x * (blockDim.x >> 6);
     for (int64_t row = (int64_t)blockIdx.x * (blockDim.x >> 6) + (threadIdx.x >> 6); row < nrows; row += wstride) {
-        if (mm.heavy[row] == MVHDP_ROW_HEAVY) continue;
+        const int cls = mm.heavy[row];
+        if (cls & MVHDP_ROW_HEAVY) continue;
+        if (lane == 0 && (cls & MVHDP_ROW_BYTE)) mm.heavy[row] = (uint8_t)(cls & ~MVHDP_ROW_BYTE);
         const uint16_t* c16 = mm.counts16 + row * K;
         int32_t* cnt = mm.counts + row * K;
         for (int k = lane; k < K; k += WAVE) cnt[k] = (int)c16[k];
@@ -351,7 +374,9 @@
         const int Kp = (K + 7) & ~7;
         const float* cf = mm.coef + (int64_t)m * Kp;
         const float smp_total = mm.coef[(int64_t)mm.M * Kp + (int64_t)m * K + K - 1];
-        const bool light_src = from_mirror && mm.heavy[row] != MVHDP_ROW_HEAVY;
+        const int cls0 = mm.heavy[row];
+        const bool light_src = from_mirror && !(cls0 & MVHDP_ROW_HEAVY);
+        if (from_mirror && lane == 0 && (cls0 & MVHDP_ROW_BYTE)) mm.heavy[row] = (uint8_t)(cls0 & ~MVHDP_ROW_BYTE);
         bool hv = false;
         if (!from_mirror) {
             long long sum = 0;
@@ -392,7 +417,7 @@
 #pragma unroll
         for (int sft = 32; sft >= 1; sft >>= 1) { acc += __shfl_xor(acc, sft, WAVE); acc0 += __shfl_xor(acc0, sft, WAVE); }
         if (lane == 0) { mm.root[row] = (double)smp_total + acc; mm.mass0[row] = (float)acc0; }
-        if (lane == 0 && heavy_list && mm.heavy[row] == MVHDP_ROW_HEAVY) {
+        if (lane == 0 && heavy_list && (mm.heavy[row] & MVHDP_ROW_HEAVY)) {
             const unsigned int i = atomicAdd(heavy_n, 1u);
             if ((int)i < heavy_cap) heavy_list[i] = (int32_t)row;
         }
diff --git a/mvtopicmodel_amd/csrc/mvhdp_plan.h b/mvtopicmodel_amd/csrc/mvhdp_plan.h
--- a/mvtopicmodel_amd/csrc/mvhdp_plan.h
+++ b/mvtopicmodel_amd/csrc/mvhdp_plan.h
@@ -64,6 +64,7 @@
     int nk_global = 0;
     uint32_t block_shared_bytes = 0;
     bool delta16 = false;
+    bool byte_rows = false;
     bool live16 = false;
     bool live_rows = false;
     bool coef_lds = false;
@@ -108,6 +109,7 @@
     int single_stream = 0;
     int four_round_on_c = -1;
     int delta16 = 1;
+    int byte_rows = -1;
     int narrow_wide = 1;
     int fork_delay_us = 0;
     int widest_on_main = 0;
@@ -417,6 +419,7 @@
         for (int c = 1; c < 5; c++) if (p.cls[c].used && p.cls[c].fast && p.cls[c].walk) p.cls[c].narrow = 1;
     p.delta16 = tu.delta16 != 0 && mirror_ok && !p.live && !p.frozen && !p.seg_apply && nseg == 1 && p.only_seg < 0 &&
                 !(flags & MVHDP_SWEEP_NO_APPLY) && !in.unassigned;
+    p.byte_rows = tu.byte_rows != 0 && mirror_ok && !p.live && !p.overlap;
     if (want_live16) {
         bool all_fast = true;
         for (int c = 0; c < MVHDP_N_CLASSES; c++) if (p.cls[c].used && !p.cls[c].fast) all_fast = false;
diff --git a/mvtopicmodel_amd/csrc/mvhdp_sweep_fast.hip b/mvtopicmodel_amd/csrc/mvhdp_sweep_fast.hip
--- a/mvtopicmodel_amd/csrc/mvhdp_sweep_fast.hip
+++ b/mvtopicmodel_amd/csrc/mvhdp_sweep_fast.hip
@@ -56,7 +56,8 @@
 }
 #define W_HEAVY 0x40000000
 #define W_BIG   0x20000000
-#define W_ROW(w) ((w) & 0x1fffffff)
+#define W_BYTE  0x10000000
+#define W_ROW(w) ((w) & 0x0fffffff)
 typedef unsigned int rowq_t __attribute__((ext_vector_type(4), aligned(4)));
 typedef float coefq_t __attribute__((ext_vector_type(4)));
 
@@ -449,6 +450,8 @@
             const int64_t row0 = mm.rowbase[m];
             const char* nwk_v = (const char*)(nwk + row0 * K);
             const char* nwk16_v = (const char*)(nwk16 + row0 * K);
+            const char* nwk8_v = (const char*)(mm.counts8 + row0 * K);
+            const bool byte_ok = NARROW && !LIVEROWS && sl.byte_rows;
             int koffh[RMAX];
 #pragma unroll
             for (int r = 0; r < RMAX; r++) koffh[r] = koff[r] >> 1;
@@ -480,7 +483,8 @@
                 if (w_l >= Vm) w_l = -1;
                 if (NARROW && w_l >= 0) {
                     const int hv = mm.heavy[row0 + w_l];
-                    if (hv) w_l |= (hv == MVHDP_ROW_HEAVY) ? (W_HEAVY | W_BIG) : W_BIG;
+                    if (hv & (MVHDP_ROW_HEAVY | MVHDP_ROW_BIG)) w_l |= (hv & MVHDP_ROW_HEAVY) ? (W_HEAVY | W_BIG) : W_BIG;
+                    if (byte_ok && (hv & MVHDP_ROW_BYTE)) w_l |= W_BYTE;
                 }
                 const float u1f_l = (float)u1_l;
                 int znew_l = z_l;
@@ -558,7 +562,12 @@
                     const int w0 = bcast_i(w_l, ra ? (int)__builtin_ctzll(ra) : t_first);
                     const unsigned int r0 = (unsigned int)W_ROW(max(w0, 0));
                     const bool h0 = w0 >= 0 && (w0 & W_HEAVY);
-                    if (NARROW && !h0) {
+                    const bool b0 = w0 >= 0 && (w0 & W_BYTE);
+                    if (NARROW && !LIVEROWS && b0) {
+                        const gptr_t c0b = scalar_row(nwk8_v, r0, (unsigned int)K);
+#pragma unroll
+                        for (int r = 0; r < RMAX; r++) { const int v = gather_cell<uint8_t>(c0b + ((unsigned int)koff[r] >> 2)); if (a == 0) gn[r] = v; else gn2[r] = v; }
+                    } else if (NARROW && !h0) {
                         const gptr_t c0q = scalar_row(nwk16_v, r0, (unsigned int)K * 2u);
 #pragma unroll
                         for (int r = 0; r < RMAX; r++) { const int v = gather_cell<uint16_t>(c0q + (unsigned int)koffh[r]); if (a == 0) gn[r] = v; else gn2[r] = v; }
diff --git a/mvtopicmodel_amd/csrc/mvhdp_sweep_fast_token.inc b/mvtopicmodel_amd/csrc/mvhdp_sweep_fast_token.inc
--- a/mvtopicmodel_amd/csrc/mvhdp_sweep_fast_token.inc
+++ b/mvtopicmodel_amd/csrc/mvhdp_sweep_fast_token.inc
@@ -17,7 +17,11 @@
                     for (int r = 0; r < RMAX; r++) { touch_lane_off(koff[r]); if (NARROW) touch_lane_off(koffh[r]); }
                     if (NB == 2 || LIVEROWS || rem_n) {
                         const int wn = bcast_i(w_l, rem_n ? (int)__builtin_ctzll(rem_n) : TOK_T);
-                        if (NARROW && !(wn & W_HEAVY)) {
+                        if (NARROW && !LIVEROWS && (wn & W_BYTE)) {
+                            const gptr_t cnb = scalar_row(nwk8_v, (unsigned int)W_ROW(wn), (unsigned int)K);
+#pragma unroll
+                            for (int r = 0; r < RMAX; r++) TOK_G[r] = gather_cell<uint8_t>(cnb + ((unsigned int)koff[r] >> 2));
+                        } else if (NARROW && !(wn & W_HEAVY)) {
                             const gptr_t cnq = scalar_row(nwk16_v, (unsigned int)W_ROW(wn), (unsigned int)K * 2u);
 #pragma unroll
                             for (int r = 0; r < RMAX; r++) TOK_G[r] = gather_cell<uint16_t>(cnq + (unsigned int)koffh[r]);
diff --git a/mvtopicmodel_amd/java/mvhdp_jni.cpp b/mvtopicmodel_amd/java/mvhdp_jni.cpp
--- a/mvtopicmodel_amd/java/mvhdp_jni.cpp
+++ b/mvtopicmodel_amd/java/mvhdp_jni.cpp
@@ -374,6 +374,7 @@
     t.force_primary = iv[0]; t.narrow = iv[1]; t.walk_fixed = iv[2]; t.single_stream = iv[3]; t.live16 = iv[4];
     t.learnt_walk_step[0] = iv[5]; t.learnt_walk_step[1] = iv[6]; t.learnt_walk_step[2] = iv[7]; t.learnt_walk_step[3] = -1;
     t.live_overlap = -1;
+    t.byte_rows = -1;
     t.primary_min_share = dv[0];
     for (int m = 0; m < 8; m++) { t.walk_theta[m] = dv[1 + m]; t.tree_branch_share[m] = dv[9 + m]; }
     int rc = mvhdp_set_tuning(s->h, &t);
```

After: 6.713 billion (median of 6 runs). About the same (-0.8%).
